# Lymphatus/caesium-clt

Measured on AMD Instinct MI355X. Metric: megapixels/sec JPEG q=80 1920x1080 batch, higher is better.
Workload: dtype int32

## Files before the change

### caesium-clt_amd/binding.py

```python
import ctypes as C
import os

_HERE = os.path.dirname(os.path.abspath(__file__))
NPHASES = 8
NKERNELS = 36
PHASE_NAMES = ["decode", "pixel", "masks_flags_runs", "stats_tables", "sizes_scan", "pack", "stuff_assemble", "reserved"]


class CCSParameters(C.Structure):
    _fields_ = [("keep_metadata", C.c_bool), ("jpeg_quality", C.c_uint32), ("jpeg_chroma_subsampling", C.c_uint32),
                ("jpeg_progressive", C.c_bool), ("jpeg_optimize", C.c_bool), ("jpeg_preserve_icc", C.c_bool),
                ("png_quality", C.c_uint32), ("png_optimization_level", C.c_uint32), ("png_force_zopfli", C.c_bool),
                ("png_optimize", C.c_bool), ("gif_quality", C.c_uint32), ("webp_quality", C.c_uint32), ("webp_lossless", C.c_bool),
                ("tiff_compression", C.c_uint32), ("tiff_deflate_level", C.c_uint32), ("width", C.c_uint32), ("height", C.c_uint32)]


class CCSResult(C.Structure):
    _fields_ = [("success", C.c_bool), ("code", C.c_uint32), ("error_message", C.c_char_p)]


class CByteArray(C.Structure):
    _fields_ = [("data", C.POINTER(C.c_uint8)), ("length", C.c_size_t)]


class Timing(C.Structure):
    _fields_ = [("total_ms", C.c_float), ("phase_ms", C.c_float * NPHASES), ("kernel_ms", C.c_float * NKERNELS), ("in_bytes", C.c_uint64), ("out_bytes", C.c_uint64),
                ("pixels", C.c_uint64), ("coef_bytes", C.c_uint64), ("n_images", C.c_uint32), ("n_failed", C.c_uint32), ("n_seq_decoded", C.c_uint32), ("n_par_fallback", C.c_uint32), ("n_par_short", C.c_uint32), ("n_prog_decoded", C.c_uint32), ("n_refine_chains", C.c_uint32), ("n_search_extra", C.c_uint32), ("n_fused_lists", C.c_uint32), ("n_list_refine", C.c_uint32), ("n_ac_in_lists", C.c_uint32), ("n_list_runs", C.c_uint32), ("n_ref_packed", C.c_uint32)]


class PngTiming(C.Structure):
    _fields_ = [("total_ms", C.c_float), ("kernel_ms", C.c_float * 16), ("in_bytes", C.c_uint64), ("out_bytes", C.c_uint64), ("pixels", C.c_uint64),
                ("raw_bytes", C.c_uint64), ("n_images", C.c_uint32), ("n_failed", C.c_uint32), ("n_trials", C.c_uint32)]


class GifTiming(C.Structure):
    _fields_ = [("total_ms", C.c_float), ("kernel_ms", C.c_float * 8), ("in_bytes", C.c_uint64), ("out_bytes", C.c_uint64), ("n_files", C.c_uint32), ("n_frames", C.c_uint32),
                ("n_failed", C.c_uint32), ("n_passed_palette", C.c_uint32), ("n_not_smaller", C.c_uint32), ("chunk_pixels", C.c_uint32), ("lossy_distance", C.c_uint32)]


class CaesiumError(RuntimeError):
    def __init__(self, code, message):
        super().__init__(f"[{code}] {message}")
        self.code = code


def library_path():
    return os.path.join(_HERE, "libcaesium_hip.so")


EXPORTS = ["cs_default_parameters", "cs_compress_in_memory", "cs_compress_to_size_in_memory", "cs_convert_in_memory",
           "cs_batch_compress", "cs_batch_extent", "cs_free_bytes", "cs_free_result", "csh_device_count", "csh_last_error", "csh_kernel_name", "csh_kernel_name_webp", "csh_release_cached_memory", "csh_warmup", "csh_batch_create",
           "csh_batch_run", "csh_batch_fetch", "csh_batch_destroy", "csh_batch_retain_dct", "csh_batch_set_quality", "csh_batch_rerun_encode", "cs_batch_compress_to_size", "csh_batch_geometry", "csh_batch_read_coefs",
           "csp_kernel_name", "csp_batch_create", "csp_batch_create_webp", "csp_batch_create_pixels", "csh_batch_create_pixels", "csh_batch_pixels", "csh_batch_create_from_pixels", "csp_png_to_jpeg", "csp_png_to_lossless_webp", "csp_batch_run", "csp_batch_fetch", "csp_batch_destroy", "csp_batch_geometry", "csp_batch_read_rows", "csp_batch_read_stream",
           "csp_batch_trials", "csp_batch_read_scores", "csp_batch_chunk_bits", "csh_batch_create_webp", "cs_batch_convert",
           "cswd_batch_create", "cswd_batch_run", "cswd_batch_pixels", "cswd_batch_read_pixels", "cswd_batch_alpha", "cswd_batch_read_rgba", "cswd_batch_destroy", "cswd_batch_frames", "cswd_batch_read_canvas", "cswd_batch_encode_anim", "cswd_rgba_join", "cswd_rgba_destroy", "csh_batch_create_webp_from_pixels", "csh_batch_create_from_pixels_rgb", "csl_encode_pixels", "csl_attach_alpha"]
GIF_EXPORTS = ["csg_kernel_name", "csg_batch_create", "csg_batch_run", "csg_batch_fetch", "csg_batch_destroy", "csg_batch_frames", "csg_batch_read_indices", "csg_batch_read_canvas", "csg_batch_create_lossy", "csg_batch_read_near"]


def _declare(L):
    P = C.POINTER
    L.cs_default_parameters.argtypes = [P(CCSParameters)]
    L.cs_default_parameters.restype = None
    L.cs_compress_in_memory.argtypes = [C.c_char_p, C.c_size_t, P(CCSParameters), P(CByteArray)]
    L.cs_compress_in_memory.restype = CCSResult
    L.cs_compress_to_size_in_memory.argtypes = [C.c_char_p, C.c_size_t, P(CCSParameters), C.c_size_t, C.c_bool, P(CByteArray)]
    L.cs_compress_to_size_in_memory.restype = CCSResult
    L.cs_convert_in_memory.argtypes = [C.c_char_p, C.c_size_t, P(CCSParameters), C.c_uint32, P(CByteArray)]
    L.cs_convert_in_memory.restype = CCSResult
    L.cs_batch_compress.argtypes = [P(CByteArray), C.c_size_t, P(CCSParameters), C.c_int, P(CByteArray), P(CCSResult)]
    L.cs_batch_extent.argtypes = [P(CByteArray), C.c_size_t]
    L.cs_batch_extent.restype = C.c_size_t
    L.cs_free_bytes.argtypes = [P(CByteArray)]
    L.cs_free_bytes.restype = None
    L.cs_free_result.argtypes = [P(CCSResult)]
    L.cs_free_result.restype = None
    L.csh_last_error.restype = C.c_char_p
    L.csh_kernel_name.argtypes = [C.c_int]
    L.csh_kernel_name.restype = C.c_char_p
    L.csh_kernel_name_webp.argtypes = [C.c_int]
    L.csh_kernel_name_webp.restype = C.c_char_p
    L.csh_batch_create.argtypes = [P(CByteArray), C.c_size_t, P(CCSParameters), C.c_int, P(C.c_void_p)]
    L.csh_batch_run.argtypes = [C.c_void_p, P(Timing)]
    L.csh_batch_fetch.argtypes = [C.c_void_p, P(CByteArray), P(CCSResult)]
    L.csh_batch_retain_dct.argtypes = [C.c_void_p, C.c_int]
    L.csh_batch_set_quality.argtypes = [C.c_void_p, P(C.c_uint32)]
    L.csh_batch_rerun_encode.argtypes = [C.c_void_p, P(Timing)]
    L.cs_batch_compress_to_size.argtypes = [P(CByteArray), C.c_size_t, P(CCSParameters), C.c_size_t, C.c_bool, C.c_int, P(CByteArray), P(CCSResult)]
    L.csh_batch_destroy.argtypes = [C.c_void_p]
    L.csh_batch_destroy.restype = None
    L.csh_batch_geometry.argtypes = [C.c_void_p, C.c_size_t, C.c_int, C.c_int, P(C.c_int), P(C.c_int), P(C.c_int), P(C.c_int)]
    L.csh_batch_read_coefs.argtypes = [C.c_void_p, C.c_size_t, C.c_int, C.c_int, C.c_void_p]
    L.csh_batch_create_webp.argtypes = [P(CByteArray), C.c_size_t, P(CCSParameters), C.c_int, P(C.c_void_p)]
    L.cs_batch_convert.argtypes = [P(CByteArray), C.c_size_t, P(CCSParameters), C.c_uint32, C.c_int, P(CByteArray), P(CCSResult)]
    L.csp_kernel_name.argtypes = [C.c_int]
    L.csp_kernel_name.restype = C.c_char_p
    L.csp_batch_create.argtypes = [P(CByteArray), C.c_size_t, P(CCSParameters), C.c_int, P(C.c_void_p)]
    L.csp_batch_run.argtypes = [C.c_void_p, P(PngTiming)]
    L.csp_batch_fetch.argtypes = [C.c_void_p, P(CByteArray), P(CCSResult)]
    L.csp_batch_destroy.argtypes = [C.c_void_p]
    L.csp_batch_destroy.restype = None
    L.csp_batch_geometry.argtypes = [C.c_void_p, C.c_size_t, P(C.c_uint32), P(C.c_uint32), P(C.c_uint32)]
    L.csp_batch_read_rows.argtypes = [C.c_void_p, C.c_size_t, C.c_void_p]
    L.csp_batch_read_stream.argtypes = [C.c_void_p, C.c_size_t, C.c_int, C.c_void_p]
    L.csp_batch_read_scores.argtypes = [C.c_void_p, C.c_size_t, C.c_void_p, P(C.c_int)]
    L.csp_batch_chunk_bits.argtypes = [C.c_void_p, C.c_size_t, C.c_int, P(C.c_uint64), C.c_size_t, P(C.c_size_t)]
    L.csp_batch_trials.argtypes = [C.c_void_p, C.c_size_t, P(C.c_int), P(C.c_uint64), P(C.c_int), P(C.c_int)]
    L.cswd_batch_create.argtypes = [P(CByteArray), C.c_size_t, C.c_int, P(C.c_void_p)]
    L.cswd_batch_run.argtypes = [C.c_void_p]
    L.cswd_batch_pixels.argtypes = [C.c_void_p, C.c_size_t, P(C.c_void_p), P(C.c_uint32), P(C.c_uint32), P(C.c_uint32), P(C.c_char_p)]
    L.cswd_batch_read_pixels.argtypes = [C.c_void_p, C.c_size_t, C.c_void_p]
    L.cswd_batch_alpha.argtypes = [C.c_void_p, C.c_size_t, P(C.c_void_p), P(C.c_void_p)]
    L.cswd_batch_read_rgba.argtypes = [C.c_void_p, C.c_size_t, C.c_void_p]
    L.cswd_batch_destroy.argtypes = [C.c_void_p]
    L.cswd_batch_destroy.restype = None
    L.cswd_batch_frames.argtypes = [C.c_void_p, C.c_size_t, P(C.c_uint32), P(C.c_uint32), P(C.c_uint32)]
    L.cswd_batch_read_canvas.argtypes = [C.c_void_p, C.c_size_t, C.c_uint32, C.c_void_p]
    L.cswd_batch_encode_anim.argtypes = [C.c_void_p, P(CByteArray), P(C.c_size_t), C.c_size_t, P(CCSParameters), C.c_int, P(CByteArray), P(CCSResult)]
    L.cswd_rgba_join.argtypes = [C.c_void_p, C.c_void_p, C.c_uint32, C.c_uint32, C.c_int, C.POINTER(C.c_void_p), C.POINTER(C.c_void_p)]
    L.cswd_rgba_join.restype = C.c_int
    L.cswd_rgba_destroy.argtypes = [C.c_void_p]
    L.cswd_rgba_destroy.restype = None
    L.csg_kernel_name.argtypes = [C.c_int]
    L.csg_kernel_name.restype = C.c_char_p
    L.csg_batch_create.argtypes = [P(CByteArray), C.c_size_t, P(CCSParameters), C.c_int, P(C.c_void_p)]
    L.csg_batch_run.argtypes = [C.c_void_p, P(GifTiming)]
    L.csg_batch_fetch.argtypes = [C.c_void_p, P(CByteArray), P(CCSResult)]
    L.csg_batch_destroy.argtypes = [C.c_void_p]
    L.csg_batch_destroy.restype = None
    L.csg_batch_frames.argtypes = [C.c_void_p, C.c_size_t, P(C.c_uint32), P(C.c_uint32), P(C.c_uint32)]
    L.csg_batch_read_indices.argtypes = [C.c_void_p, C.c_size_t, C.c_uint32, C.c_void_p]
    L.csg_batch_read_canvas.argtypes = [C.c_void_p, C.c_size_t, C.c_uint32, C.c_void_p]
    L.csg_batch_create_lossy.argtypes = [P(CByteArray), C.c_size_t, P(CCSParameters), C.c_int, P(C.c_void_p)]
    L.csg_batch_read_near.argtypes = [C.c_void_p, C.c_size_t, C.c_uint32, C.c_void_p, C.c_void_p]
    return L


def default_parameters(lib=None, **kw):
    p = CCSParameters()
    p.jpeg_quality = p.png_quality = p.webp_quality = p.gif_quality = 80
    p.jpeg_progressive = True
    p.jpeg_preserve_icc = True
    p.png_optimization_level = 3
    p.tiff_deflate_level = 6
    for k, v in kw.items():
        if not hasattr(p, k):
            raise AttributeError(k)
        setattr(p, k, v)
    return p


class Batch:

    def __init__(self, api, blobs, params, device=0, webp=False):
        self.api = api
        L = api.L
        self.n = len(blobs)
        self._keep = [C.create_string_buffer(b, len(b)) for b in blobs]
        self._in = (CByteArray * self.n)()
        for i, buf in enumerate(self._keep):
            self._in[i].data = C.cast(buf, C.POINTER(C.c_uint8))
            self._in[i].length = len(blobs[i])
        self.h = C.c_void_p()
        rc = (L.csh_batch_create_webp if webp else L.csh_batch_create)(self._in, self.n, C.byref(params), device, C.byref(self.h))
        if rc:
            raise CaesiumError(rc, L.csh_last_error().decode())

    def run(self):
        t = Timing()
        rc = self.api.L.csh_batch_run(self.h, C.byref(t))
        if rc:
            raise CaesiumError(rc, self.api.L.csh_last_error().decode())
        return t

    def retain_dct(self, on=True):
        if self.api.L.csh_batch_retain_dct(self.h, 1 if on else 0):
            raise CaesiumError(-1, self.api.L.csh_last_error().decode())

    def set_quality(self, qualities):
        arr = (C.c_uint32 * self.n)(*qualities)
        if self.api.L.csh_batch_set_quality(self.h, arr):
# ... 430 lines not shown
```

### caesium-clt_amd/csrc/batch.hpp

```cpp
#pragma once
#include <array>
#include <chrono>
#include <map>
#include <string>
#include <vector>

#include "../../include/caesium_hip.h"
#include "devmem.hpp"
#include "jpeg_host.hpp"
#include "kernels.h"
#include "webp_kernels.h"

namespace csh {

struct Item {
    int code = 0;
    std::string msg;
    JpegInfo in;
    JpegInfo out;
    int image = -1;
    size_t file_size = 0;
    std::vector<uint8_t> meta_out;
};

struct DecodePlan {
    PinnedBytes bits_pool;
    std::vector<DecScan> dscans;
    std::vector<DevHuffSet> hsets;
    std::vector<ParHuffSet> phsets;
    std::vector<char> phset_fits;
    std::vector<ParHuffSet4> phsets4;
    std::vector<std::array<int8_t, 8>> slot4;
    bool use4 = true;
    std::vector<ParScan> pscans;
    std::vector<uint32_t> need_seq_init;
    std::vector<ProgChain> chains;
    std::vector<int> chain_scans;
    std::vector<RefineUnit> refine_units;
    uint32_t refine_hist = 0, refine_pos = 0, refine_max_blocks = 0;
    uint32_t total_sub = 0, max_sub = 0, max_par_blocks = 0, dc_total = 0;

    DevBuf<uint8_t> d_bits, d_clean;
    DevBuf<ParScan> d_pscans;
    DevBuf<uint64_t> d_pstate, d_relax_list[2], d_unstuff_off, d_blk_off, d_dc_off;
    DevBuf<uint32_t> d_unstuff_cnt, d_nblk, d_need_seq, d_need_seq_init, d_relax_cnt, d_scan_pending, d_cut_block, d_claim;
    DevBuf<uint16_t> d_hyp;
    DevBuf<int32_t> d_dcdiff;
    DevBuf<DecScan> d_dscans;
    DevBuf<ProgChain> d_chains;
    DevBuf<int> d_chain_scans;
    DevBuf<uint64_t> d_refine_hist;
    DevBuf<uint32_t> d_refine_pos, d_refine_prog;
    DevBuf<RefineUnit> d_refine_units;
    DevBuf<DevHuffSet> d_hsets;
    DevBuf<ParHuffSet> d_phsets;
    DevBuf<ParHuffSet4> d_phsets4;
};

struct PixelPlan {
    std::vector<PlaneWork> pwork;
    std::vector<ResizeWork> rwork;
    std::vector<ResizeTap> rtaps;
    std::vector<float> rweights;
    uint64_t rgb_bytes = 0, tmp_floats = 0, max_tmp = 0, max_dst = 0;
    uint32_t max_row_in = 0, max_out_w = 0, max_nh = 0;
    uint32_t max_src_px = 0;
    uint64_t plane_bytes = 0, oplane_bytes = 0;
    uint32_t max_quads = 0;
    bool any_layout = false, any_layout_rgb = false;
    bool any_space_rgb = false;

    DevBuf<uint8_t> d_planes, d_oplanes, d_rgb;
    DevBuf<PlaneWork> d_pwork;
    DevBuf<ResizeWork> d_rwork;
    DevBuf<ResizeTap> d_rtaps;
    DevBuf<float> d_rweights, d_rtmp;
    DevBuf<int16_t> d_dct_raw;
};

struct Stage {
    uint32_t work0 = 0, nwork = 0, slot0 = 0, nslots = 0, ech0 = 0, nech = 0, table0 = 0, ntables = 0, plan0 = 0, nplans = 0, nzc0 = 0, nnzc = 0, ls0 = 0, nls = 0, ts0 = 0, nts = 0, rs0 = 0, nrs = 0, lr0 = 0, nlr = 0, rr0 = 0, nrr = 0;
    bool nz_build[2] = {true, true}, nz_filter[2] = {true, true};
};
struct SearchImg {
    int cand_work[64]; int ncand;
    int Al_luma = 0, Al_chroma = 0;
    uint64_t best_luma = 0, best_chroma = 0;
    int split_luma = 0, split_chroma = 0;
    bool luma_on = false, chroma_on = false;
    bool fixed = false;
};

struct EncodePlan {
    std::vector<EncScan> script;
    std::vector<ScanWork> swork;
    uint32_t nslots = 0, nlist_slots = 0, ntok_slots = 0;
    uint32_t nref_slots = 0;
    uint32_t last_run_refine = 0;
    uint32_t last_run_ref_packed = 0;
    bool ref_pack = true;
    uint32_t list_run = CSH_LIST_RUN;
    uint32_t nlist_runs = 0, nref_runs = 0;
    bool ac_runs_slot = false;
    uint32_t last_run_list_runs = 0;
    uint64_t total_corr = 0;
    uint64_t total_units = 0, total_words = 0;
    uint32_t max_units = 0;
    int ntables = 0;
    std::vector<TokPlan> plans;
    std::vector<int> plan_comp, plan_image;
    std::vector<EChunk> echunks;
    uint64_t tok_cap = 0;
    uint32_t tok_scale = 1;
    std::vector<TokRegion> regions;
    std::vector<uint32_t> region_est;
    uint32_t hist_rows = 0;
    std::vector<NzList> nzlists;
    std::vector<NzSet> nzsets;
    std::vector<int> nzset_of;
    std::vector<uint32_t> nzset_built;
    std::vector<int> nzset_comp, nzset_image;
    std::vector<NzChunk> nzchunks;
    std::vector<NzChunk> nzchunks_fused;
    uint32_t n_fused = 0;
    uint32_t last_run_fused = 0;
    uint32_t n_ac_lists = 0;
    uint32_t last_run_ac_lists = 0;
    std::vector<uint8_t> nzset_ac_lists;
    std::vector<uint32_t> nz_est, nz_worst;
    uint32_t nz_nrec = 0;
    uint64_t nz_cap = 0;
    bool search = false;
    enum { ST_1 = 0, ST_1B = 1, ST_2 = 2, ST_2B = 3, ST_2C = 4, ST_N = 5 };
    Stage stage[ST_N];
    void stage_begin(Stage &sg) {
        sg.work0 = uint32_t(swork.size()); sg.slot0 = nslots; sg.ech0 = uint32_t(echunks.size()); sg.table0 = uint32_t(ntables); sg.plan0 = uint32_t(plans.size());
        sg.nzc0 = uint32_t(nzchunks.size()); sg.ls0 = nlist_slots; sg.ts0 = ntok_slots; sg.rs0 = nref_slots; sg.lr0 = nlist_runs; sg.rr0 = nref_runs;
    }
    void stage_end(Stage &sg) {
        sg.nwork = uint32_t(swork.size()) - sg.work0; sg.nslots = nslots - sg.slot0; sg.nech = uint32_t(echunks.size()) - sg.ech0;
        sg.ntables = uint32_t(ntables) - sg.table0; sg.nplans = uint32_t(plans.size()) - sg.plan0;
        sg.nnzc = uint32_t(nzchunks.size()) - sg.nzc0; sg.nls = nlist_slots - sg.ls0; sg.nts = ntok_slots - sg.ts0; sg.nrs = nref_slots - sg.rs0; sg.nlr = nlist_runs - sg.lr0; sg.nrr = nref_runs - sg.rr0;
    }
    std::vector<SearchImg> simg;
    std::vector<uint8_t> work_active;
    uint32_t n_gated_runs = 0;
    std::vector<uint32_t> img_list, img_nlist, h_cost;
    std::map<std::array<int, 5>, int> cand_script;
    std::vector<uint8_t> hdr_pool;
    std::vector<uint32_t> hdr_off;

    DevBuf<uint8_t> d_hdr, d_tail, d_scan_tmp, d_work_active;
    DevBuf<EncScan> d_script;
    DevBuf<ScanWork> d_swork;
    DevBuf<uint32_t> d_slot_work;
    DevBuf<EChunk> d_echunks;
    DevBuf<SlotRec> d_slots;
    DevBuf<TokPlan> d_plans;
    DevBuf<uint64_t> d_corr, d_symbits, d_eobbits, d_tok_off, d_chunk_off, d_scan_raw_off;
    DevBuf<uint32_t> d_tok_cursor;
    DevBuf<TokRegion> d_regions;
    DevBuf<uint16_t> d_eobrun, d_slot_hist, d_lastn;
    DevBuf<uint32_t> d_img_list, d_img_nlist, d_scan_cost, d_slot_raw, d_slot_eobh, d_long_runs, d_long_cnt, d_tokens, d_chunk_ntok, d_chunk_bits, d_raw, d_scan_pad, d_chunk_ff, d_hdr_off;
    DevBuf<DevEncTable> d_tables;
    DevBuf<NzList> d_nzlists;
    DevBuf<NzSet> d_nzsets;
    DevBuf<NzChunk> d_nzchunks, d_nzchunks_fused;
    DevBuf<uint32_t> d_nz_pool, d_nz_cursor, d_nz_chunk_off, d_nz_chunk_cnt, d_list_slots, d_tok_slots, d_ref_slots, d_list_runs, d_ref_runs;
};

struct TrellisPlan {
    bool trellis = false, dering = false;
    Stage tstage;
    std::vector<TrellisWork> twork;
    std::vector<TrellisRun> truns;
    uint32_t t_units = 0, t_max_rows = 0;
    std::vector<uint32_t> trows;
    bool t_sort = false;
    bool nz_once = false;

    DevBuf<TrellisWork> d_twork;
    DevBuf<TrellisRun> d_truns;
    DevBuf<uint32_t> d_tqueue, d_trows, d_tperm, d_tspill;
    DevBuf<uint8_t> d_tblk_cnt;
    DevBuf<uint16_t> d_tblk_off;
    DevBuf<uint64_t> d_tlambda, d_tdcbt;
};

struct WebpTail {
    uint32_t webp_mb_bytes = 768;
    std::vector<csw::WebpImg> wimgs;
    uint64_t wwork_bytes = 0, wlevels = 0;
    uint32_t wmax_luma = 0, wmax_mbh = 0;

    DevBuf<csw::WebpImg> d_wimgs;
    DevBuf<uint8_t> d_wwork, d_wscratch, d_wprobs, d_wupdate;
    DevBuf<uint32_t> d_wpart, d_wstats;
    DevBuf<int16_t> d_wlevels;
};

struct Outputs {
    uint64_t raw_bytes_cap = 0, out_cap = 0;
    DevBuf<uint8_t> d_out;
    DevBuf<uint64_t> d_img_off;
    DevBuf<uint32_t> d_img_size, d_img_size_pad, d_status, d_overflow;
    std::vector<uint32_t> h_img_size;
    std::vector<uint64_t> h_img_off;
    std::vector<uint32_t> h_status;
    bool ran = false;
};

}

struct csh_batch {
    int device = 0;
    hipStream_t stream = 0;
    bool have_stream = false;
    CCSParameters params;
    std::vector<csh::Item> items;
    int nimg = 0;
    bool lossless = false;
    bool rgb_out = false;
    bool webp = false;
    int test_pool_shift = -1;
    bool progressive = true;
    bool retain_dct = false;
    bool have_dct = false;
    int q_base = 0;

    std::vector<csh::ImgDesc> imgs;
    std::vector<csh::DevQuant> quants;
    uint32_t ntiles = 0, ntiles_in = 0, ntiles_out = 0, max_tiles = 0, max_dummy = 0;
    csh::DevBuf<csh::ImgDesc> d_imgs;
    csh::DevBuf<csh::DevQuant> d_quants;
    csh::DevBuf<int16_t> d_coef;

    csh::DecodePlan dec;
    csh::PixelPlan pix;
    csh::EncodePlan enc;
    csh::TrellisPlan tr;
    csh::WebpTail wp;
    csh::Outputs out;

    ~csh_batch() { if (have_stream) { (void)hipStreamSynchronize(stream); (void)hipStreamDestroy(stream); } }
};

namespace csh {

enum KernelSlot {
    KS_MEMSET_COEF, KS_UNSTUFF, KS_DEC_SPEC, KS_DEC_RELAX0, KS_DEC_RELAX, KS_DEC_WRITE, KS_DC_SCATTER, KS_REFINE_CHAINS, KS_DECODE_PROG_SEQ,
    KS_IDCT_PLANE, KS_RESIZE, KS_XFORM_DIRECT, KS_RESAMPLE_FDCT, KS_FIX_DUMMY, KS_MEMSET_ENC, KS_TRELLIS_STATS, KS_TRELLIS_AC, KS_TRELLIS_DC,
    KS_NZLIST, KS_TOKENS, KS_LIST_STATS, KS_AC_RUNS, KS_GEN_TABLES, KS_CHUNK_SIZES, KS_SCAN_CHUNK_BITS, KS_SCAN_LAYOUT, KS_PACK, KS_LIST_PACK,
    KS_FF_COUNT, KS_SCAN_SEARCH, KS_LAYOUT, KS_SCAN_IMAGES, KS_EMIT, KS_SPARE0, KS_SPARE1, KS_SPARE2, KS_COUNT,
    KS_WEBP_YUV = KS_XFORM_DIRECT, KS_WEBP_ENCODE = KS_RESAMPLE_FDCT, KS_WEBP_ASSEMBLE = KS_FIX_DUMMY
};
struct KernelSlotRow { KernelSlot slot; const char *name; int phase; };
constexpr KernelSlotRow kKernelSlots[] = {
    {KS_MEMSET_COEF, "memset_coef", 0},        {KS_UNSTUFF, "unstuff", 0},                 {KS_DEC_SPEC, "k_dec_spec", 0},
    {KS_DEC_RELAX0, "k_dec_relax0", 0},        {KS_DEC_RELAX, "k_dec_relax1_4", 0},        {KS_DEC_WRITE, "k_dec_write", 0},
    {KS_DC_SCATTER, "k_dc_scatter", 0},        {KS_REFINE_CHAINS, "k_refine_chains", 0},   {KS_DECODE_PROG_SEQ, "k_decode_prog+seq", 0},
    {KS_IDCT_PLANE, "k_idct_plane", 1},        {KS_RESIZE, "resize", 1},                   {KS_XFORM_DIRECT, "k_xform_direct", 1},
    {KS_RESAMPLE_FDCT, "k_resample+k_plane_fdct", 1}, {KS_FIX_DUMMY, "k_fix_dummy", 1},    {KS_MEMSET_ENC, "memset_enc", 2},
    {KS_TRELLIS_STATS, "trellis_stats", 1},    {KS_TRELLIS_AC, "k_trellis_ac", 1},         {KS_TRELLIS_DC, "k_trellis_dc", 1},
    {KS_NZLIST, "k_nzlist", 2},                {KS_TOKENS, "k_tokens", 2},                 {KS_LIST_STATS, "k_list_stats", 2},
    {KS_AC_RUNS, "k_ac_runs", 2},              {KS_GEN_TABLES, "k_gen_tables", 3},         {KS_CHUNK_SIZES, "k_chunk_sizes", 4},
    {KS_SCAN_CHUNK_BITS, "scan_chunk_bits", 4}, {KS_SCAN_LAYOUT, "scan_layout", 4},        {KS_PACK, "k_pack", 5},
    {KS_LIST_PACK, "k_list_pack", 5},          {KS_FF_COUNT, "k_ff_count", 6},             {KS_SCAN_SEARCH, "scan_search_stage2", 7},
    {KS_LAYOUT, "k_layout", 6},                {KS_SCAN_IMAGES, "scan_images", 6},         {KS_EMIT, "k_emit", 6},
    {KS_SPARE0, "", 7},                        {KS_SPARE1, "", 7},                         {KS_SPARE2, "", 7}};
constexpr bool kernel_slots_in_order() {
    for (int i = 0; i < int(sizeof kKernelSlots / sizeof kKernelSlots[0]); i++) if (kKernelSlots[i].slot != i) return false;
    return true;
}
static_assert(sizeof kKernelSlots / sizeof kKernelSlots[0] == CSH_NKERNELS && int(KS_COUNT) == int(CSH_NKERNELS), "one row per csh_timing.kernel_ms slot");
static_assert(kernel_slots_in_order(), "row i of kKernelSlots describes slot i");

struct PlanSwitches {
    std::string profile;
    bool nz_once = true;
    bool tr_sort = true;
    int prog_par = -1;
    bool fused_420 = true;
    bool nz_fused = true;
    bool ref_list = true;
    bool ref_pack = true;
    uint32_t list_run = CSH_LIST_RUN;
    bool ac_runs_slot = false;
    bool ac_tiles = false;
    static PlanSwitches read();
};

struct Laps {
    const bool trace;
    std::chrono::steady_clock::time_point at = std::chrono::steady_clock::now();
    std::string text;
    Laps();
    void lap(const char *what);
};

struct BatchPlanner {
    csh_batch *const b;
    const CByteArray *const inputs;
    const size_t count;
    const CCSParameters *const p;
    const csp_pixels *const px;
    const PlanSwitches sw;
    const bool progressive;
    uint16_t qout_nat[64];
    int script_base3 = 0, script_base1 = 0;
    std::map<int, int> other_scripts;
    std::vector<std::pair<std::vector<uint8_t>, int>> hset_keys;
    std::map<std::vector<uint16_t>, int> quant_index;
    uint64_t plane_off = 64, oplane_off = 0;

    BatchPlanner(csh_batch *b, const CByteArray *inputs, size_t count, const CCSParameters *p, const csp_pixels *px);
    void begin();
    void parse();
    int reserve_pinned();
    int plan_image(size_t n);
    int plan_search_stages();
    int plan_trellis();
    void finish_descriptors();
    int upload(Laps &laps);

private:
    void image_geometry(Item &it, ImgDesc &im);
    int decode_scans(Item &it, ImgDesc &im, const uint8_t *d);
    int huff_set(const JScan &js);
    void place_blocks(ParScan &ps, const JpegInfo &in, const JScan &js, uint32_t units, bool dc_rows, bool subseqs);
    int sequential_split(const Item &it, const ImgDesc &im, const uint8_t *d, int img_index, bool &par_ok);
    bool progressive_plan(const Item &it, const ImgDesc &im, int img_index);
    void plane_work(ImgDesc &im, const JpegInfo &in, const JpegInfo &o, int img_index, bool resized);
    void resize_work(const JpegInfo &in, const JpegInfo &o, int img_index);
    void output_scans(Item &it, ImgDesc &im, int img_index, size_t in_len);
    void frame_header(Item &it);
    template <class Fill> int enc_scan(const std::array<int, 5> &key, Fill fill);
    int space_script(int ncomp, int space, int &ns);
    int cand_index(int comp, int Ss, int Se, int Ah, int Al, int cls = -1);
    int dc_scan_index(int ncomp);
    int seq1_index(int comp, int cls = -1);
    uint32_t nz_list(int img_index, int comp, int Al, const ImgDesc &im, size_t in_len);
    void add_works(Item &it, ImgDesc &im, int img_index, const std::vector<int> &list, size_t in_len, const JpegInfo &o, bool stats_only = false);
    template <class Make> void add_stage(int sid, Make make);
    template <class Add> void splits(const ImgDesc &im, Add &add, int i0, int i1, bool whole);
};

void layout_token_pool(csh_batch *b);

int run_once(csh_batch *b, csh_timing *t, bool requant_only);

int search_costs(csh_batch *b, AsmCtx &a, int stage);
uint32_t search_gate(csh_batch *b, int stage, int (*want)(const SearchImg &));
int search_decide(csh_batch *b, int stage);
int search_lists(csh_batch *b);

}
```

### caesium-clt_amd/csrc/batch_plan.cpp

```cpp
#include <algorithm>
#include <atomic>
#include <cmath>
#include <thread>

#include "batch.hpp"
#include "resize_host.h"
#include "result.h"

namespace csh {

static void build_dev_huff(const HuffSpec &h, DevHuff &d) {
    memset(&d, 0, sizeof d);
    for (int l = 0; l < 18; l++) d.maxcode[l] = -1;
    if (!h.present) return;
    int code = 0, p = 0;
    for (int l = 1; l <= 16; l++) {
        if (h.bits[l]) {
            d.valptr[l] = p - code;
            for (int i = 0; i < h.bits[l]; i++, p++, code++)
                if (l <= 9) {
                    int base = code << (9 - l);
                    for (int k = 0; k < (1 << (9 - l)); k++) d.look[(base + k) & 511] = uint16_t((l << 8) | h.vals[p]);
                }
            d.maxcode[l] = code - 1;
// ... 50 lines not shown
            while ((2 << lg) <= q.div[k]) lg++;
            const int P = std::max(25, lg + 18);
            q.mul[k] = uint32_t((1ull << P) / uint64_t(q.div[k])) + 1u;
            q.sh[k] = uint32_t(32 - P);
        }
    }
}

static void fill_geom(const JComp &c, CompGeom &g, uint32_t &ntiles) {
    g.h = c.h; g.v = c.v; g.comp_w = c.comp_w; g.comp_h = c.comp_h;
    g.real_bw = c.real_bw; g.real_bh = c.real_bh; g.bw = c.bw; g.bh = c.bh;
    g.ntiles = (c.bw * c.bh + 63) / 64;
    g.tile_base = ntiles;
    ntiles += g.ntiles;
}

static void add_script(std::vector<EncScan> &v, int ncomp, bool progressive, int space) {
    for (const OutScan &o : output_script(ncomp, progressive, space == CSH_CS_YCC)) {
        EncScan e;
        memset(&e, 0, sizeof e);
        e.ncomp = o.ncomp; e.Ss = o.Ss; e.Se = o.Se; e.Ah = o.Ah; e.Al = o.Al;
        for (int k = 0; k < o.ncomp; k++) e.comp[k] = o.comp[k];
        if (!progressive) {
            e.sequential = 1;
            for (int k = 0; k < o.ncomp; k++) {
                int id = table_class(space, o.comp[k]);
                int di = -1, ai = -1;
                for (int t = 0; t < e.ntables; t++) { if (e.dht_id[t] == id) di = t; if (e.dht_id[t] == (0x10 | id)) ai = t; }
                if (di < 0) { di = e.ntables; e.dht_id[e.ntables++] = id; }
                if (ai < 0) { ai = e.ntables; e.dht_id[e.ntables++] = 0x10 | id; }
                e.dc_tbl[k] = di; e.ac_tbl[k] = ai;
                e.sos_tdta[k] = (id << 4) | id;
            }
        } else if (o.Ss == 0) {
            if (o.Ah == 0) {
                e.ntables = 0;
                for (int k = 0; k < o.ncomp; k++) {
                    int id = table_class(space, o.comp[k]);
                    int idx = -1;
                    for (int t = 0; t < e.ntables; t++) if (e.dht_id[t] == id) idx = t;
                    if (idx < 0) { idx = e.ntables; e.dht_id[e.ntables++] = id; }
                    e.dc_tbl[k] = idx;
                    e.sos_tdta[k] = id << 4;
                }
            }
        } else {
            int id = table_class(space, o.comp[0]);
            e.ntables = 1; e.dht_id[0] = 0x10 | id; e.sos_tdta[0] = id;
        }
        v.push_back(e);
    }
}

static UpDesc up_desc(int hx, int vx, int cw) {
    UpDesc u; u.hx = uint8_t(hx); u.vx = uint8_t(vx); u.pad = 0;
    if (hx == 1 && vx == 1) u.cls = CSH_UP_COPY;
    else if (hx == 2 && vx == 1 && cw > 2) u.cls = CSH_UP_H2V1;
    else if (hx == 1 && vx == 2) u.cls = CSH_UP_H1V2;
    else if (hx == 2 && vx == 2 && cw > 2) u.cls = CSH_UP_H2V2;
    else u.cls = CSH_UP_REP;
    return u;
}
static int dn_kind(int hx, int vx) { return hx == 1 ? CSH_DN_FULL : (hx == 4 ? CSH_DN_H4V1 : (vx == 2 ? CSH_DN_H2V2 : CSH_DN_H2V1)); }

static int plan_item(Item &it, const CCSParameters &p, bool lossless, bool to_rgb) {
    const JpegInfo &in = it.in;
    if (in.ncomp != 1 && in.ncomp != 3 && in.ncomp != 4) { it.msg = "unsupported component count"; return CS_ERR_JPEG_FEATURE; }
    if (uint64_t(in.width) * uint64_t(in.height) > (1ull << 28)) { it.msg = "image dimensions too large for the device path"; return CS_ERR_JPEG_FEATURE; }
    const bool other_space = in.space != CSH_CS_GREY && in.space != CSH_CS_YCC;
    const bool converted = other_space && to_rgb;
    it.out = JpegInfo();
    JpegInfo &o = it.out;
    o.width = in.width; o.height = in.height; o.ncomp = converted ? 3 : in.ncomp;
    o.space = converted ? CSH_CS_YCC : in.space;
    if (other_space && !converted) { o.write_jfif = false; o.write_adobe = in.adobe_transform; }
    if (p.width || p.height) {
        if (lossless) { it.msg = "resize + lossless transcode not on the device path"; return CS_ERR_UNSUPPORTED; }
        csh_compute_dimensions(in.width, in.height, int(p.width), int(p.height), o.width, o.height);
        if (o.width > 65500 || o.height > 65500 || uint64_t(o.width) * uint64_t(o.height) > (1ull << 28)) { it.msg = "resize target too large for JPEG"; return CS_ERR_JPEG_FEATURE; }
    }
    if (in.ncomp >= 3 && (!lossless || in.ncomp == 4)) {
        int blocks = 0;
        for (int c = 0; c < in.ncomp; c++) {
            const JComp &k = in.comp[c];
            blocks += k.h * k.v;
            if (in.hmax % k.h || in.vmax % k.v) { it.msg = "fractional chroma sampling ratio (component factors do not divide the largest ones)"; return CS_ERR_JPEG_FEATURE; }
            if (in.hmax / k.h > 4 || in.vmax / k.v > 4) { it.msg = "chroma sampling ratio above 4"; return CS_ERR_JPEG_FEATURE; }
        }
        if (blocks > 10) { it.msg = "more than 10 blocks per MCU"; return CS_ERR_JPEG_FEATURE; }
    }
    if (lossless) {
        for (int c = 0; c < in.ncomp; c++)
            if (memcmp(in.comp[c].qt, in.qt[in.comp[c].tq], sizeof in.comp[c].qt)) { it.msg = "a component was decoded with a quantisation table that its slot no longer holds"; return CS_ERR_JPEG_FEATURE; }
        for (int c = 0; c < in.ncomp; c++) o.comp[c] = in.comp[c];
        jpeg_geometry(o);
        return 0;
    }
    int ss = int(p.jpeg_chroma_subsampling);
    if (ss == 0) ss = 420;
    static const char kRgbIds[] = "RGB", kCmykIds[] = "CMYK";
    for (int c = 0; c < o.ncomp; c++) {
        o.comp[c].id = o.space == CSH_CS_RGB ? kRgbIds[c] : (o.space == CSH_CS_CMYK ? kCmykIds[c] : c + 1);
        o.comp[c].h = o.comp[c].v = 1; o.comp[c].tq = table_class(o.space, c);
    }
    if (o.space == CSH_CS_YCC || o.space == CSH_CS_YCCK) {
        int h = 1, v = 1;
        if (ss == 420) { h = 2; v = 2; }
        else if (ss == 422) { h = 2; v = 1; }
        else if (ss == 411) { h = 4; v = 1; }
        else if (ss != 444) { it.msg = "unknown output chroma subsampling"; return CS_ERR_JPEG_FEATURE; }
        o.comp[0].h = h; o.comp[0].v = v;
        if (o.space == CSH_CS_YCCK) { o.comp[3].h = h; o.comp[3].v = v; }
    }
    jpeg_geometry(o);
    return 0;
}

void layout_token_pool(csh_batch *b) {
    b->enc.regions.resize(b->enc.region_est.size());
    if (b->test_pool_shift < 0) b->test_pool_shift = getenv("CSH_TEST_POOL_SHIFT") ? std::min(16, std::max(0, atoi(getenv("CSH_TEST_POOL_SHIFT")))) : 0;
    const int shift = b->test_pool_shift;
    uint64_t at = 0;
    for (size_t i = 0; i < b->enc.regions.size(); i++) {
        const uint64_t cap = std::min<uint64_t>(std::max<uint64_t>((uint64_t(b->enc.region_est[i]) * b->enc.tok_scale) >> shift, 64), 0xFFFFFFF0ull);
        b->enc.regions[i].base = at; b->enc.regions[i].cap = uint32_t(cap); b->enc.regions[i].pad = 0;
        at += (cap + 3) & ~uint64_t(3);
    }
    b->enc.tok_cap = at + 64;
    at = 0;
    for (size_t i = 0; i < b->enc.nzlists.size(); i++) {
        const uint64_t cap = std::min<uint64_t>(std::max<uint64_t>((uint64_t(b->enc.nz_est[i]) * b->enc.tok_scale) >> shift, 64), b->enc.nz_worst[i]);
        b->enc.nzlists[i].base = at; b->enc.nzlists[i].cap = uint32_t(cap);
        at += (cap + 3) & ~uint64_t(3);
    }
    b->enc.nz_cap = at + 64;
}

PlanSwitches PlanSwitches::read() {
    auto is = [](const char *name, const char *v) { const char *e = getenv(name); return e && !strcmp(e, v); };
    PlanSwitches s;
    const char *penv = getenv("CSH_PROFILE");
    s.profile = penv && *penv ? penv : "mozjpeg";
    s.nz_once = !is("CSH_NZ_ONCE", "0");
    s.tr_sort = !is("CSH_TR_SORT", "0");
    s.nz_fused = !is("CSH_NZ_FUSED", "0");
    s.ac_tiles = is("CSH_AC_TILES", "1");
    s.ref_list = is("CSH_REF_LIST", "1") || (s.ref_list && !is("CSH_REF_LIST", "0"));
    s.ref_pack = s.ref_list && (is("CSH_REF_PACK", "1") || (s.ref_pack && !is("CSH_REF_PACK", "0")));
    const char *pp = getenv("CSH_PROG_PAR");
    s.prog_par = pp && !strcmp(pp, "0") ? 0 : (pp && !strcmp(pp, "1") ? 1 : -1);
    s.fused_420 = !getenv("CSH_NO_FUSED_420");
    if (const char *lr = getenv("CSH_LIST_RUN")) { if (*lr) s.list_run = uint32_t(std::min(32, std::max(1, atoi(lr)))); }
    s.ac_runs_slot = is("CSH_AC_RUNS", "slot");
    return s;
}

Laps::Laps() : trace(getenv("CSH_TRACE") != nullptr) {}
void Laps::lap(const char *what) {
    if (!trace) return;
    const auto now = std::chrono::steady_clock::now();
    char buf[64];
    snprintf(buf, sizeof buf, " %s %.1f", what, std::chrono::duration<double, std::milli>(now - at).count());
    text += buf; at = now;
}

BatchPlanner::BatchPlanner(csh_batch *b_, const CByteArray *inputs_, size_t count_, const CCSParameters *p_, const csp_pixels *px_)
    : b(b_), inputs(inputs_), count(count_), p(p_), px(px_), sw(PlanSwitches::read()), progressive(p_->jpeg_progressive) {}

void BatchPlanner::begin() {
    b->items.resize(count);
    quality_table(int(p->jpeg_quality), qout_nat);
    DevQuant qo; make_quant(qout_nat, qo);
    b->quants.push_back(qo);
    b->q_base = int(b->quants.size()) - 1;
    for (int q = 1; q <= 100; q++) { uint16_t tq[64]; quality_table(q, tq); DevQuant dq; make_quant(tq, dq); b->quants.push_back(dq); }
    b->progressive = progressive;
    b->enc.list_run = sw.list_run;
    b->enc.ac_runs_slot = sw.ac_runs_slot;
    b->enc.ref_pack = sw.ref_pack;

    add_script(b->enc.script, 3, true, CSH_CS_YCC);
    add_script(b->enc.script, 1, true, CSH_CS_GREY);
    add_script(b->enc.script, 3, false, CSH_CS_YCC);
    add_script(b->enc.script, 1, false, CSH_CS_GREY);
    script_base3 = progressive ? 0 : 16; script_base1 = progressive ? 10 : 17;
    const bool webp = b->webp, rgb_out = b->rgb_out;
    const std::string &profile = sw.profile;
    b->enc.search = progressive && !webp && !rgb_out && profile != "plain";
    const bool lossy_jpeg = !b->lossless && !webp && !rgb_out;
    b->tr.trellis = lossy_jpeg && (profile == "mozjpeg" || profile == "mozjpeg-trellis");
    b->tr.dering = lossy_jpeg && (profile == "mozjpeg" || profile == "mozjpeg-dering");
    b->tr.nz_once = b->tr.trellis && progressive && sw.nz_once && sw.tr_sort;
}

template <class Fill>
int BatchPlanner::enc_scan(const std::array<int, 5> &key, Fill fill) {
    auto f = b->enc.cand_script.find(key);
    if (f != b->enc.cand_script.end()) return f->second;
    EncScan e;
    memset(&e, 0, sizeof e);
    fill(e);
    b->enc.script.push_back(e);
    return b->enc.cand_script[key] = int(b->enc.script.size()) - 1;
}
int BatchPlanner::space_script(int ncomp, int space, int &ns) {
    ns = progressive ? (space == CSH_CS_YCC ? 10 : 2 + 4 * ncomp) : 1;
    if (space == CSH_CS_YCC) return script_base3;
    if (space == CSH_CS_GREY) return script_base1;
    auto f = other_scripts.find(space);
    if (f == other_scripts.end()) {
        f = other_scripts.emplace(space, int(b->enc.script.size())).first;
        add_script(b->enc.script, ncomp, progressive, space);
    }
    return f->second;
}
int BatchPlanner::cand_index(int comp, int Ss, int Se, int Ah, int Al, int cls) {
    const int ycc = comp ? 1 : 0;
    if (cls < 0) cls = ycc;
    return enc_scan({cls == ycc ? comp : comp + 16 * (1 + cls), Ss, Se, Ah, Al}, [&](EncScan &e) {
        const int id = cls;
        e.ncomp = 1; e.comp[0] = comp; e.Ss = Ss; e.Se = Se; e.Ah = Ah; e.Al = Al;
        e.ntables = 1; e.dht_id[0] = 0x10 | id; e.sos_tdta[0] = id;
    });
}
int BatchPlanner::dc_scan_index(int ncomp) {
    return enc_scan({-ncomp, 0, 0, 0, 0}, [&](EncScan &e) {
        e.ncomp = ncomp;
        for (int k = 0; k < ncomp; k++) {
            e.comp[k] = k;
            const int id = k ? 1 : 0;
            int idx = -1;
            for (int t = 0; t < e.ntables; t++) if (e.dht_id[t] == id) idx = t;
            if (idx < 0) { idx = e.ntables; e.dht_id[e.ntables++] = id; }
            e.dc_tbl[k] = idx; e.sos_tdta[k] = id << 4;
        }
    });
}
int BatchPlanner::seq1_index(int comp, int cls) {
    const int ycc = comp ? 1 : 0;
    if (cls < 0) cls = ycc;
    return enc_scan({cls == ycc ? comp : comp + 16 * (1 + cls), 0, 63, -1, -1}, [&](EncScan &e) {
        const int id = cls;
        e.ncomp = 1; e.comp[0] = comp; e.Ss = 0; e.Se = 63; e.sequential = 1;
        e.ntables = 2; e.dht_id[0] = id; e.dht_id[1] = 0x10 | id; e.dc_tbl[0] = 0; e.ac_tbl[0] = 1; e.sos_tdta[0] = (id << 4) | id;
    });
}

static uint64_t blocks_of(const ImgDesc &im) {
    uint64_t n = 0;
    for (int k = 0; k < im.ncomp; k++) n += uint64_t(im.out[k].real_bw) * im.out[k].real_bh;
    return n;
}

uint32_t BatchPlanner::nz_list(int img_index, int comp, int Al, const ImgDesc &im, size_t in_len) {
    if (b->enc.nzset_of.size() < size_t(img_index + 1) * CSH_MAX_COMPS) b->enc.nzset_of.resize(size_t(img_index + 1) * CSH_MAX_COMPS, -1);
    int &si = b->enc.nzset_of[size_t(img_index) * CSH_MAX_COMPS + size_t(comp)];
    const uint32_t nu = uint32_t(im.out[comp].real_bw * im.out[comp].real_bh);
    if (si < 0) {
        NzSet S;
        memset(&S, 0, sizeof S);
        for (int L = 0; L < CSH_NZ_LEVELS; L++) S.list[L] = 0xFFFFFFFFu;
        S.cnt_base = 0xFFFFFFFFu;
        S.nunits = nu; S.real_bw = im.out[comp].real_bw; S.bw = im.out[comp].bw; S.tile_base = im.out[comp].tile_base;
        si = int(b->enc.nzsets.size());
        b->enc.nzsets.push_back(S); b->enc.nzset_built.push_back(0u); b->enc.nzset_comp.push_back(comp); b->enc.nzset_image.push_back(img_index);
    }
    const uint64_t blocks_all = blocks_of(im);
    static const uint32_t kShare[CSH_NZ_LEVELS] = {20, 16, 12, 9};
    for (int L : {0, Al}) {
        if (b->enc.nzsets[size_t(si)].list[L] != 0xFFFFFFFFu) continue;
        const uint32_t nch = (nu + 255) / 256;
        NzList R;
        memset(&R, 0, sizeof R);
        R.chunk0 = b->enc.nz_nrec; b->enc.nz_nrec += nch;
        b->enc.nzsets[size_t(si)].list[L] = uint32_t(b->enc.nzlists.size());
        b->enc.nzlists.push_back(R);
        const uint64_t est = uint64_t(in_len) * kShare[L] / 8 * nu / std::max<uint64_t>(1, blocks_all) + nu + 4ull * nch + 256;
        const uint64_t worst = uint64_t(nu) * 64 + 4ull * nch;
        b->enc.nz_est.push_back(uint32_t(std::min<uint64_t>(est, worst)));
        b->enc.nz_worst.push_back(uint32_t(std::min<uint64_t>(worst, 0xFFFFFFF0ull)));
    }
    return b->enc.nzsets[size_t(si)].list[Al];
}

void BatchPlanner::add_works(Item &it, ImgDesc &im, int img_index, const std::vector<int> &list, size_t in_len, const JpegInfo &o, bool stats_only) {
    const int w_first = int(b->enc.swork.size());
    uint32_t nz_need[CSH_MAX_COMPS] = {0, 0, 0}, nz_gate[CSH_MAX_COMPS] = {0, 0, 0};
    for (int sidx : list) {
        const EncScan &e = b->enc.script[sidx];
        ScanWork w;
        memset(&w, 0, sizeof w);
        w.image = img_index; w.scan = sidx;
        w.out_off = 0xFFFFFFFFu;
        const bool from_list = e.Ss > 0 && !e.sequential && e.Ah == 0;
        const bool ref_list = sw.ref_list && e.Ss > 0 && !e.sequential && e.Ah != 0;
        w.list = 0xFFFFFFFFu; w.rs_base = 0xFFFFFFFFu; w.lr_base = 0xFFFFFFFFu; w.rr_base = 0xFFFFFFFFu;
        if (from_list || ref_list) {
            if (e.Al >= CSH_NZ_LEVELS) { it.code = CS_ERR_JPEG_FEATURE; it.msg = "internal: output scan script outside what the list coder carries"; }
            else {
                w.list = nz_list(img_index, e.comp[0], e.Al, im, in_len);
                if (!nz_need[e.comp[0]]) nz_gate[e.comp[0]] = uint32_t(b->enc.swork.size());
                nz_need[e.comp[0]] |= 1u << e.Al;
            }
        }
        if (e.Ss == 0 && e.ncomp > 1) w.nunits = uint32_t(im.omcus_x * im.omcus_y);
        else w.nunits = uint32_t(im.out[e.comp[0]].real_bw * im.out[e.comp[0]].real_bh);
// ... 585 lines not shown
    }
}
int BatchPlanner::plan_search_stages() {
    b->enc.hdr_off.push_back(uint32_t(b->enc.hdr_pool.size()));
    b->nimg = int(b->imgs.size());
    b->enc.stage_end(b->enc.stage[0]);
    if (!b->enc.search) return 0;
    add_stage(EncodePlan::ST_1B, [&](const ImgDesc &, auto &add) { add(9, cand_index(0, 1, 63, 3, 2)); add(10, cand_index(0, 1, 8, 0, 3)); add(11, cand_index(0, 9, 63, 0, 3)); });
    add_stage(EncodePlan::ST_2, [&](const ImgDesc &im, auto &add) { splits(im, add, 0, 2, true); });
    add_stage(EncodePlan::ST_2B, [&](const ImgDesc &im, auto &add) { splits(im, add, 3, 3, false); });
    add_stage(EncodePlan::ST_2C, [&](const ImgDesc &im, auto &add) { splits(im, add, 4, 4, false); });
    for (int c = 0; c < 3; c++) for (int i = -1; i < 5; i++) for (int Al = 1; Al <= (c ? 2 : 3); Al++) {
        if (i < 0) cand_index(c, 1, 63, 0, Al); else { cand_index(c, 1, kSplit[i], 0, Al); cand_index(c, kSplit[i] + 1, 63, 0, Al); }
    }
    b->enc.work_active.assign(b->enc.swork.size(), 0);
    if (b->enc.total_units > 0xFFFFFFF0ull) { csh_set_error("csh_batch_create: batch too large for the scan search's candidate lists (fewer files per batch)"); return CS_ERR_POOL_OVERFLOW; }
    return 0;
}

int BatchPlanner::plan_trellis() {
    if (!b->tr.trellis) return 0;
    b->enc.nslots++;
    Stage &tg = b->tr.tstage;
    b->enc.stage_begin(tg);
    for (size_t n = 0; n < count; n++) {
        Item &it = b->items[n];
        if (it.image < 0) continue;
        ImgDesc &im = b->imgs[size_t(it.image)];
        std::vector<int> list;
        const int space = it.out.space;
        for (int c = 0; c < im.ncomp; c++) list.push_back(progressive ? cand_index(c, 1, 63, 0, 0, table_class(space, c)) : seq1_index(c, table_class(space, c)));
        const size_t first = b->enc.swork.size();
        add_works(it, im, it.image, list, inputs[n].length, it.out, true);
        for (int c = 0; c < im.ncomp; c++) {
            const ScanWork &w = b->enc.swork[first + size_t(c)];
            TrellisWork tw;
            memset(&tw, 0, sizeof tw);
            tw.image = it.image; tw.comp = c; tw.dc_cls = uint32_t(table_class(space, c));
            tw.table_ac = w.table_base + (progressive ? 0u : 1u);
            tw.table_dc = progressive ? -1 : int32_t(w.table_base);
            tw.nunits = w.nunits; tw.unit_base = b->tr.t_units;
            b->tr.t_units += w.nunits;
            b->tr.t_max_rows = std::max<uint32_t>(b->tr.t_max_rows, uint32_t((im.out[c].real_bh + im.out[c].v - 1) / im.out[c].v));
            tw.nzset = 0xFFFFFFFFu;
            if (progressive) {
                const int si = b->enc.nzset_of[size_t(it.image) * CSH_MAX_COMPS + size_t(c)];
                b->enc.nzsets[size_t(si)].cnt_base = tw.unit_base;
                if (b->tr.nz_once) tw.nzset = uint32_t(si);
            }
            b->tr.twork.push_back(tw);
        }
    }
    b->enc.stage_end(tg);
    {
        std::vector<uint32_t> nch(b->tr.twork.size());
        uint32_t most = 0;
        for (size_t wi = 0; wi < b->tr.twork.size(); wi++) { nch[wi] = (b->tr.twork[wi].nunits + CSH_TR_WG - 1) / CSH_TR_WG; most = std::max(most, nch[wi]); }
        for (uint32_t j = 0; j < most; j += CSH_TR_RUN)
            for (size_t wi = 0; wi < b->tr.twork.size(); wi++)
                if (j < nch[wi]) b->tr.truns.push_back(TrellisRun{uint32_t(wi), j, std::min<uint32_t>(CSH_TR_RUN, nch[wi] - j)});
    }
    {
        b->tr.t_sort = progressive && sw.tr_sort;
        std::vector<std::pair<uint32_t, uint32_t>> rows;
        for (size_t wi = 0; wi < b->tr.twork.size(); wi++) {
            const CompGeom &g = b->imgs[size_t(b->tr.twork[wi].image)].out[b->tr.twork[wi].comp];
            for (int r = 0; r < (g.real_bh + g.v - 1) / g.v; r++) rows.push_back({uint32_t(g.real_bw * g.v), uint32_t(wi << 16) | uint32_t(r)});
        }
        std::stable_sort(rows.begin(), rows.end(), [](const auto &a, const auto &b2) { return a.first > b2.first; });
        for (const auto &r : rows) b->tr.trows.push_back(r.second);
    }
    if (b->enc.total_units > 0xFFFFFFF0ull) { csh_set_error("csh_batch_create: batch too large (fewer files per batch)"); return CS_ERR_POOL_OVERFLOW; }
    return 0;
}

void BatchPlanner::finish_descriptors() {
    if (!b->lossless)
        for (ImgDesc &im : b->imgs) for (int c = 0; c < im.ncomp; c++) im.out[c].tile_base += b->ntiles_in;
    for (size_t i = 0; i < b->enc.plans.size(); i++) b->enc.plans[i].tile_base = b->imgs[size_t(b->enc.plan_image[i])].out[b->enc.plan_comp[i]].tile_base;
    for (size_t i = 0; i < b->enc.nzsets.size(); i++) b->enc.nzsets[i].tile_base = b->imgs[size_t(b->enc.nzset_image[i])].out[b->enc.nzset_comp[i]].tile_base;
    {
        b->enc.nzchunks_fused = b->enc.nzchunks;
        const bool allowed = sw.nz_fused && !b->lossless && !b->webp && !b->rgb_out && !(b->tr.trellis && progressive && !b->tr.nz_once);
        std::vector<uint8_t> fused(b->enc.nzsets.size(), 0);
        const bool lists_only = progressive && !sw.ac_tiles && sw.ref_list && sw.nz_once && sw.tr_sort && (!b->tr.trellis || (b->tr.t_sort && b->tr.nz_once));
        std::vector<uint8_t> planned(b->enc.nzsets.size(), 0);
        for (size_t i = 0; i < b->enc.plans.size(); i++) {
            const size_t at = size_t(b->enc.plan_image[i]) * CSH_MAX_COMPS + size_t(b->enc.plan_comp[i]);
            if (at < b->enc.nzset_of.size() && b->enc.nzset_of[at] >= 0) planned[size_t(b->enc.nzset_of[at])] = 1;
        }
        b->enc.nzset_ac_lists.assign(b->enc.nzsets.size(), 0);
        for (PlaneWork &w : b->pix.pwork) {
            w.ac_lists = 0u;
            const size_t at = size_t(w.image) * CSH_MAX_COMPS + size_t(w.comp);
            const int si = allowed && at < b->enc.nzset_of.size() ? b->enc.nzset_of[at] : -1;
            if (si < 0) continue;
            const NzSet &S = b->enc.nzsets[size_t(si)];
            if (S.real_bw != S.bw || S.list[0] == 0xFFFFFFFFu) continue;
            w.nzset = uint32_t(si); fused[size_t(si)] = 1; b->enc.n_fused++;
            if (lists_only && !planned[size_t(si)]) { w.ac_lists = 1u; b->enc.nzset_ac_lists[size_t(si)] = 1; b->enc.n_ac_lists++; }
        }
        for (TrellisWork &tw : b->tr.twork) tw.ac_lists = (tw.nzset != 0xFFFFFFFFu && b->enc.nzset_ac_lists[tw.nzset]) ? 1u : 0u;
        for (NzChunk &ch : b->enc.nzchunks_fused) if (fused[ch.set]) ch.levels &= ~1u;
        auto flags = [&](Stage &sg) {
            for (int f = 0; f < 2; f++) {
                const std::vector<NzChunk> &v = f ? b->enc.nzchunks_fused : b->enc.nzchunks;
                sg.nz_build[f] = sg.nz_filter[f] = false;
                for (uint32_t i = sg.nzc0; i < sg.nzc0 + sg.nnzc; i++) { sg.nz_build[f] |= (v[i].levels & 1u) != 0u; sg.nz_filter[f] |= (v[i].levels & ~1u) != 0u; }
            }
        };
        for (Stage &sg : b->enc.stage) flags(sg);
        flags(b->tr.tstage);
    }
    for (ParScan &ps : b->dec.pscans)
        for (int m = 0; m < ps.nb_mcu && m < 10; m++) {
            int dcs = ps.dct[m] & 3, acs = 4 + (ps.act[m] & 3);
            if (b->dec.use4) { dcs = std::max<int>(0, b->dec.slot4[ps.huff_set][dcs]); acs = std::max<int>(0, b->dec.slot4[ps.huff_set][acs]); }
            ps.sel |= uint64_t(dcs | (acs << 3)) << (6 * m);
        }
    {
        std::vector<int> last(b->dec.chains.size(), -1);
        for (int s = 0;; s++) {
            bool any = false;
            for (size_t c = 0; c < b->dec.chains.size(); c++)
                if (b->dec.chains[c].refine && b->dec.chains[c].count > s) {
                    RefineUnit u; u.chain = int(c); u.s = s; u.prev = last[c];
                    last[c] = int(b->dec.refine_units.size());
                    b->dec.refine_units.push_back(u);
                    any = true;
                }
            if (!any) break;
        }
    }
    b->ntiles = b->ntiles_in + b->ntiles_out;
    b->pix.plane_bytes = plane_off;
    b->pix.oplane_bytes = oplane_off;
    b->out.out_cap = b->out.raw_bytes_cap;
    layout_token_pool(b);
}

int BatchPlanner::upload(Laps &laps) {
    hipStream_t st = b->stream;
    if (!b->nimg) return 0;
    b->dec.bits_pool.flush_copies();
    laps.lap("copy_in");
    if (b->dec.d_bits.alloc(b->dec.bits_pool.size()) || (b->dec.bits_pool.size() && hipMemcpyAsync(b->dec.d_bits.p, b->dec.bits_pool.p, b->dec.bits_pool.size(), hipMemcpyHostToDevice, st) != hipSuccess) ||
        b->d_imgs.upload(b->imgs, st) || b->dec.d_dscans.upload(b->dec.dscans, st) || b->dec.d_chains.upload(b->dec.chains, st) || b->dec.d_chain_scans.upload(b->dec.chain_scans, st) ||
        b->dec.d_hsets.upload(b->dec.hsets, st) || b->dec.d_phsets.upload(b->dec.phsets, st) || (b->dec.use4 && b->dec.d_phsets4.upload(b->dec.phsets4, st)) || b->d_quants.upload(b->quants, st) || b->pix.d_pwork.upload(b->pix.pwork, st) ||
        b->enc.d_script.upload(b->enc.script, st) || b->enc.d_swork.upload(b->enc.swork, st) || b->enc.d_slot_work.alloc(size_t(b->enc.nslots) + 1) || b->enc.d_slots.alloc(size_t(b->enc.nslots) + 1) || b->enc.d_plans.upload(b->enc.plans, st) || b->enc.d_echunks.upload(b->enc.echunks, st) || b->enc.d_hdr.upload(b->enc.hdr_pool, st) ||
        b->enc.d_hdr_off.upload(b->enc.hdr_off, st) || b->dec.d_pscans.upload(b->dec.pscans, st) || b->pix.d_rwork.upload(b->pix.rwork, st) || b->pix.d_rtaps.upload(b->pix.rtaps, st) ||
        b->pix.d_rweights.upload(b->pix.rweights, st) || b->pix.d_rgb.alloc(b->pix.rgb_bytes + 64) || b->pix.d_rtmp.alloc((resize_is_fused(b->pix.max_row_in) ? 0 : b->pix.tmp_floats) + 16) || b->dec.d_need_seq_init.upload(b->dec.need_seq_init, st))
        return CS_ERR_NO_DEVICE;
    size_t nchunks = b->dec.bits_pool.size() / 64 + 1, nst = size_t(b->dec.total_sub) + b->dec.pscans.size() + 1;
    if (b->dec.d_clean.alloc(b->dec.bits_pool.size() + 64) || b->dec.d_unstuff_cnt.alloc(nchunks + 1) || b->dec.d_unstuff_off.alloc(nchunks + 2) ||
        b->dec.d_pstate.alloc(nst) || b->dec.d_relax_list[0].alloc(nst) || b->dec.d_relax_list[1].alloc(nst) || b->dec.d_relax_cnt.alloc(512) || b->dec.d_scan_pending.alloc(b->dec.pscans.size() + 1) || b->dec.d_cut_block.alloc(b->dec.pscans.size() + 1) || b->dec.d_claim.alloc(size_t(b->dec.total_sub) + 1) || b->dec.d_hyp.alloc((size_t(b->dec.total_sub) + 1) * 10) ||
        b->dec.d_nblk.alloc(size_t(b->dec.total_sub) + 1) || b->dec.d_blk_off.alloc(size_t(b->dec.total_sub) + 2) || b->dec.d_need_seq.alloc(b->nimg + 1) ||
        b->dec.d_dcdiff.alloc(size_t(b->dec.dc_total) + 1) || b->dec.d_dc_off.alloc(size_t(b->dec.dc_total) + 2) ||
        b->dec.d_refine_hist.alloc(size_t(b->dec.refine_hist) + 1) || b->dec.d_refine_pos.alloc(size_t(b->dec.refine_pos) + 1) || b->dec.d_refine_units.upload(b->dec.refine_units, st) ||
        b->dec.d_refine_prog.alloc(b->dec.refine_units.size() + 1))
        return CS_ERR_NO_DEVICE;
    if (b->d_coef.alloc(size_t(b->ntiles) * CSH_TILE_I16) || b->pix.d_planes.alloc(b->pix.plane_bytes + 64) || b->pix.d_oplanes.alloc(b->pix.oplane_bytes + 64) ||
        b->enc.d_symbits.alloc(b->enc.total_words + 1) || b->enc.d_eobbits.alloc(b->enc.total_words + 1) ||
        b->enc.d_long_runs.alloc(2 * (b->enc.total_units / 512 + b->enc.swork.size() + 16)) || b->enc.d_long_cnt.alloc(4) || b->enc.d_tail.alloc(b->enc.total_units + 1) || b->enc.d_eobrun.alloc(b->enc.total_units + 1) || b->enc.d_corr.alloc(b->enc.total_corr + 1) || b->enc.d_lastn.alloc((b->enc.ref_pack ? b->enc.total_corr : 0) + 1) ||
        b->enc.d_tok_off.alloc(4 * size_t(b->enc.nslots) + 4) || b->enc.d_chunk_ntok.alloc(4 * size_t(b->enc.nslots) + 4) || b->enc.d_slot_hist.alloc(size_t(b->enc.hist_rows) * 256 + 256) ||
        b->enc.d_slot_raw.alloc(size_t(b->enc.nslots) + 1) || b->enc.d_img_list.upload(b->enc.img_list, st) || b->enc.d_img_nlist.upload(b->enc.img_nlist, st) || b->enc.d_scan_cost.alloc(b->enc.swork.size() + 1) || b->enc.d_slot_eobh.alloc(16 * size_t(b->enc.nslots) + 16) || b->enc.d_chunk_bits.alloc(size_t(b->enc.nslots) + 1) || b->enc.d_chunk_off.alloc(size_t(b->enc.nslots) + 2) || b->enc.d_tok_cursor.alloc(b->enc.region_est.size() + 1) || b->enc.d_regions.upload(b->enc.regions, st) ||
        b->enc.d_tables.alloc(b->enc.ntables) || b->enc.d_scan_pad.alloc(b->enc.swork.size() + 1) ||
        b->enc.d_nzlists.upload(b->enc.nzlists, st) || b->enc.d_nzsets.upload(b->enc.nzsets, st) || b->enc.d_nzchunks.upload(b->enc.nzchunks, st) || (b->enc.n_fused && b->enc.d_nzchunks_fused.upload(b->enc.nzchunks_fused, st)) || b->enc.d_list_slots.alloc(size_t(b->enc.nlist_slots) + 1) || b->enc.d_tok_slots.alloc(size_t(b->enc.ntok_slots) + 1) || b->enc.d_ref_slots.alloc(size_t(b->enc.nref_slots) + 1) || b->enc.d_list_runs.alloc(size_t(b->enc.nlist_runs) + 1) || b->enc.d_ref_runs.alloc(size_t(b->enc.nref_runs) + 1) ||
        b->enc.d_nz_cursor.alloc(b->enc.nzlists.size() + 1) || b->enc.d_nz_chunk_off.alloc(size_t(b->enc.nz_nrec) + 1) || b->enc.d_nz_chunk_cnt.alloc(size_t(b->enc.nz_nrec) + 1) ||
        b->enc.d_scan_raw_off.alloc(b->enc.swork.size() + 2) || b->out.d_img_size.alloc(b->nimg + 1) || b->out.d_img_size_pad.alloc(b->nimg + 1) ||
        b->out.d_img_off.alloc(b->nimg + 2) || b->out.d_status.alloc(b->nimg) || b->out.d_overflow.alloc(4))
        return CS_ERR_NO_DEVICE;
    if (hipMemsetAsync(b->enc.d_slots.p, 0, (size_t(b->enc.nslots) + 1) * sizeof(SlotRec), st) != hipSuccess ||
        hipMemsetAsync(b->enc.d_slot_work.p, 0, (size_t(b->enc.nslots) + 1) * sizeof(uint32_t), st) != hipSuccess) { csh_set_error("hipMemsetAsync failed"); return CS_ERR_NO_DEVICE; }
    launch_make_slots(st, b->enc.d_swork.p, uint32_t(b->enc.swork.size()), b->enc.d_script.p, b->enc.d_nzlists.p, b->enc.d_slots.p, b->enc.d_slot_work.p, b->enc.d_list_slots.p, b->enc.d_tok_slots.p, b->enc.d_ref_slots.p, b->enc.d_list_runs.p, b->enc.d_ref_runs.p, b->enc.list_run);
    if (b->tr.trellis && (b->tr.d_trows.upload(b->tr.trows, st) || (b->tr.t_sort && (b->tr.d_tperm.alloc(size_t(b->tr.t_units) + 1) || b->tr.d_tblk_cnt.alloc(size_t(b->tr.t_units) + 1) || (b->tr.nz_once && b->tr.d_tblk_off.alloc(size_t(b->tr.t_units) + 1)))))) return CS_ERR_NO_DEVICE;
    if (b->tr.trellis && (b->tr.d_twork.upload(b->tr.twork, st) || b->tr.d_truns.upload(b->tr.truns, st) || b->tr.d_tqueue.alloc(1) || b->tr.d_tlambda.alloc(size_t(b->tr.t_units) + 1) || b->tr.d_tdcbt.alloc(size_t(b->tr.t_units) + 1) ||
                       b->tr.d_tspill.alloc(trellis_spill_words(trellis_ac_slots())) || b->pix.d_dct_raw.alloc(size_t(b->ntiles_out) * CSH_TILE_I16)))
        return CS_ERR_NO_DEVICE;
    for (size_t n = 0; px && n < count; n++) {
        const Item &it = b->items[n];
        if (it.image < 0) continue;
        const ResizeWork &rw = b->pix.rwork[size_t(it.image)];
        if (rw.image != it.image) { csh_set_error("internal: resize work out of order"); return CS_ERR_NO_DEVICE; }
        if (hipMemcpyAsync(b->pix.d_rgb.p + rw.rgb_src_off, px[n].device_pixels, size_t(px[n].width) * px[n].height * px[n].channels, hipMemcpyDeviceToDevice, st) != hipSuccess) { csh_set_error("pixel copy failed"); return CS_ERR_NO_DEVICE; }
    }
    laps.lap("alloc+enqueue");
    if (hipStreamSynchronize(st) != hipSuccess) { csh_set_error("upload failed"); return CS_ERR_NO_DEVICE; }
    laps.lap("upload_wait");
    return 0;
}

}
```

### caesium-clt_amd/csrc/batch_run.cpp

```cpp
#include <algorithm>

#include "batch.hpp"

namespace csh {
namespace {

class KernelMarks {
    hipEvent_t ev[CSH_NKERNELS + 1];
    int created = 0, next = 0;
    const hipStream_t st;

public:
    explicit KernelMarks(hipStream_t s) : st(s) {}
    KernelMarks(const KernelMarks &) = delete;
    KernelMarks &operator=(const KernelMarks &) = delete;
    ~KernelMarks() { for (int i = 0; i < created; i++) (void)hipEventDestroy(ev[i]); }
    int start() {
        for (; created <= CSH_NKERNELS; created++) CSH_CHECK(hipEventCreate(&ev[created]));
        CSH_CHECK(hipEventRecord(ev[0], st));
        return 0;
    }
    int claim(KernelSlot slot, hipEvent_t *e) {
        if (int(slot) != next || next >= CSH_NKERNELS) {
            csh_set_error("internal: timing mark '%s' out of order (slot %d is next)", slot < KS_COUNT ? kKernelSlots[slot].name : "?", next);
            return -1;
        }
        *e = ev[++next];
        return 0;
    }
    int mark(KernelSlot slot) {
        hipEvent_t e;
        if (claim(slot, &e)) return -1;
        CSH_CHECK(hipEventRecord(e, st));
        return 0;
    }
    int skip_to(KernelSlot slot) {
        while (next < int(slot)) if (mark(KernelSlot(next))) return -1;
        return int(slot) == next ? 0 : mark(slot);
    }
    int read(csh_timing *t, bool phases) const {
        if (phases) {
            for (int i = 0; i < CSH_NPHASES; i++) t->phase_ms[i] = 0;
            for (int i = 0; i < CSH_NKERNELS; i++) t->kernel_ms[i] = 0;
        }
        for (int i = 0; i < next; i++) {
            CSH_CHECK(hipEventElapsedTime(&t->kernel_ms[i], ev[i], ev[i + 1]));
            if (phases) t->phase_ms[kKernelSlots[i].phase] += t->kernel_ms[i];
        }
        CSH_CHECK(hipEventElapsedTime(&t->total_ms, ev[0], ev[next]));
        return 0;
    }
};
#define MARK(slot) do { if (marks.mark(slot)) return -1; } while (0)

struct Run {
    csh_batch *const b;
    csh_timing *const t;
    const hipStream_t st;
    const int nimg;
    KernelMarks marks;
    uint64_t raw_chunks = 0;
    bool eobrun_cleared = false;
    bool fused = false;
    EncCtx c;
    AsmCtx a;

    Run(csh_batch *b_, csh_timing *t_) : b(b_), t(t_), st(b_->stream), nimg(b_->nimg), marks(b_->stream) {}

    int pools() {
        raw_chunks = (b->out.raw_bytes_cap + 63) / 64;
        if (b->enc.d_raw.n != raw_chunks * 16) {
            if (b->enc.d_raw.alloc(raw_chunks * 16) || b->enc.d_chunk_ff.alloc(raw_chunks + 1) || b->out.d_out.alloc(b->out.out_cap + 64))
                return -1;
            const uint64_t longest = std::max({uint64_t(size_t(b->enc.nslots)), uint64_t(b->enc.swork.size()), uint64_t(b->dec.dc_total), uint64_t(b->dec.total_sub), uint64_t(b->dec.bits_pool.size() / 64), uint64_t(nimg)});
            size_t tmp = exclusive_scan_tmp_bytes(longest + 1);
            if (b->enc.d_scan_tmp.alloc(tmp)) return -1;
        }
        if (b->enc.d_tokens.n < b->enc.tok_cap && b->enc.d_tokens.alloc(b->enc.tok_cap)) return -1;
        if (b->enc.d_nz_pool.n < b->enc.nz_cap && b->enc.d_nz_pool.alloc(b->enc.nz_cap)) return -1;
        return 0;
    }

    int requant() {
        if (b->out.d_status.zero(st) || b->out.d_overflow.zero(st)) return -1;
        launch_requant(st, b->d_imgs.p, b->pix.d_pwork.p, int(b->pix.pwork.size()), b->max_tiles, b->d_quants.p, b->pix.d_dct_raw.p, b->ntiles_in, b->d_coef.p);
        launch_fix_dummy(st, b->d_imgs.p, nimg, b->max_dummy, b->d_coef.p);
        return marks.skip_to(KS_MEMSET_ENC);
    }
    int skip_decode() {
        if (b->out.d_status.zero(st) || b->out.d_overflow.zero(st)) return -1;
        return marks.skip_to(KS_IDCT_PLANE);
    }

    int decode() {
        const bool zero_in_spec = !b->dec.pscans.empty() && b->dec.max_sub != 0;
        if (!zero_in_spec) CSH_CHECK(hipMemsetAsync(b->d_coef.p, 0, size_t(b->ntiles_in) * CSH_TILE_I16 * sizeof(int16_t), st));
        if (b->out.d_status.zero(st) || b->out.d_overflow.zero(st)) return -1;
        CSH_CHECK(hipMemcpyAsync(b->dec.d_need_seq.p, b->dec.d_need_seq_init.p, size_t(nimg) * sizeof(uint32_t), hipMemcpyDeviceToDevice, st));
        MARK(KS_MEMSET_COEF);
        {
            int nps = int(b->dec.pscans.size());
            uint32_t nchunks = uint32_t(b->dec.bits_pool.size() / 64);
            if (nps) {
                launch_unstuff_count(st, b->dec.d_bits.p, b->dec.d_pscans.p, nps, nchunks, b->dec.d_unstuff_cnt.p);
                launch_exclusive_scan(st, b->dec.d_unstuff_cnt.p, b->dec.d_unstuff_off.p, nchunks, b->enc.d_scan_tmp.p, b->enc.d_scan_tmp.n);
                launch_unstuff_copy(st, b->dec.d_bits.p, b->dec.d_clean.p, b->dec.d_pscans.p, nps, nchunks, b->dec.d_unstuff_off.p);
            }
            MARK(KS_UNSTUFF);
            DenseArgs da;
            memset(&da, 0, sizeof da);
            da.clean = b->dec.d_clean.p; da.pss = b->dec.d_pscans.p; da.huffs = b->dec.use4 ? static_cast<const void *>(b->dec.d_phsets4.p) : static_cast<const void *>(b->dec.d_phsets.p); da.compact = b->dec.use4 ? 1 : 0; da.state = b->dec.d_pstate.p; da.nblk = b->dec.d_nblk.p;
            da.list_out = b->dec.d_relax_list[0].p; da.cnt_out = b->dec.d_relax_cnt.p; da.blk_off = b->dec.d_blk_off.p; da.imgs = b->d_imgs.p;
            da.coef = b->d_coef.p; da.dcdiff = b->dec.d_dcdiff.p; da.need_seq = b->dec.d_need_seq.p; da.cut_block = b->dec.d_cut_block.p;
            CSH_CHECK(hipMemsetAsync(b->dec.d_cut_block.p, 0xFF, b->dec.d_cut_block.n * sizeof(uint32_t), st));
            const uint64_t zero_all = uint64_t(b->ntiles_in) * CSH_TILE_I16 * sizeof(int16_t), zero_half = (zero_all / 2) & ~uint64_t(15);
            const uint64_t eob_all = (uint64_t(b->enc.d_eobrun.n) * sizeof(uint16_t)) & ~uint64_t(15), eob_half = (eob_all / 2) & ~uint64_t(15);
            if (zero_in_spec) { da.zero_ptr = reinterpret_cast<uint8_t *>(b->d_coef.p); da.zero_bytes = zero_half; da.zero2_ptr = reinterpret_cast<uint8_t *>(b->enc.d_eobrun.p); da.zero2_bytes = eob_half; }
            launch_dec_dense(st, 0, nps, b->dec.max_sub, da);
            da.zero_bytes = 0; da.zero2_bytes = 0;
            MARK(KS_DEC_SPEC);
            if (nps) CSH_CHECK(hipMemsetAsync(b->dec.d_relax_cnt.p, 0, b->dec.d_relax_cnt.n * sizeof(uint32_t), st));
            if (nps && b->dec.d_claim.zero(st)) return -1;
            if (zero_in_spec) {
                da.zero_ptr = reinterpret_cast<uint8_t *>(b->d_coef.p) + zero_half; da.zero_bytes = zero_all - zero_half;
                da.zero2_ptr = reinterpret_cast<uint8_t *>(b->enc.d_eobrun.p) + eob_half; da.zero2_bytes = eob_all - eob_half;
                if (uint64_t(b->enc.d_eobrun.n) * sizeof(uint16_t) > eob_all) CSH_CHECK(hipMemsetAsync(reinterpret_cast<uint8_t *>(b->enc.d_eobrun.p) + eob_all, 0, uint64_t(b->enc.d_eobrun.n) * sizeof(uint16_t) - eob_all, st));
                eobrun_cleared = b->enc.d_eobrun.n != 0;
            }
            launch_dec_dense(st, 1, nps, b->dec.max_sub, da);
            da.zero_bytes = 0; da.zero2_bytes = 0;
            MARK(KS_DEC_RELAX0);
            const int kMaxRounds = int(b->dec.d_relax_cnt.n) - 2;
            int R = 0;
            for (int group = 12; nps && R < kMaxRounds; group = 8) {
                for (int g = 0; g < group && R < kMaxRounds; g++, R++)
                    launch_dec_relax_list(st, b->dec.d_clean.p, b->dec.d_pscans.p, b->dec.total_sub, da.huffs, da.compact, b->dec.d_pstate.p, b->dec.d_nblk.p, b->dec.d_relax_list[R & 1].p,
                                          b->dec.d_relax_cnt.p + R, b->dec.d_relax_list[(R & 1) ^ 1].p, b->dec.d_relax_cnt.p + R + 1, b->dec.d_pstate.n, b->dec.d_claim.p, uint32_t(R + 1));
                uint32_t left = 0;
                CSH_CHECK(hipMemcpyAsync(&left, b->dec.d_relax_cnt.p + R, sizeof left, hipMemcpyDeviceToHost, st));
                CSH_CHECK(hipStreamSynchronize(st));
                if (!left) break;
            }
            if (nps) {
                if (b->dec.d_scan_pending.zero(st)) return -1;
                launch_dec_mark_pending(st, b->dec.d_pscans.p, b->dec.total_sub, b->dec.d_relax_list[R & 1].p, b->dec.d_relax_cnt.p + R, b->dec.d_scan_pending.p);
                da.hyp = b->dec.d_hyp.p; da.scan_pending = b->dec.d_scan_pending.p;
                launch_dec_dense(st, 3, nps, b->dec.max_sub, da);
                launch_dec_chain(st, b->dec.d_pscans.p, nps, b->dec.d_pstate.p, b->dec.d_nblk.p, b->dec.d_hyp.p, b->dec.d_scan_pending.p, b->dec.d_need_seq.p);
            }
            MARK(KS_DEC_RELAX);
            if (nps) launch_exclusive_scan(st, b->dec.d_nblk.p, b->dec.d_blk_off.p, b->dec.total_sub, b->enc.d_scan_tmp.p, b->enc.d_scan_tmp.n);
            launch_dec_dense(st, 2, nps, b->dec.max_sub, da);
            MARK(KS_DEC_WRITE);
            if (nps) launch_exclusive_scan(st, reinterpret_cast<uint32_t *>(b->dec.d_dcdiff.p), b->dec.d_dc_off.p, b->dec.dc_total, b->enc.d_scan_tmp.p, b->enc.d_scan_tmp.n);
            launch_dc_scatter(st, b->dec.d_pscans.p, nps, b->dec.max_par_blocks, b->d_imgs.p, b->dec.d_dc_off.p, b->d_coef.p, b->dec.d_need_seq.p, b->dec.d_cut_block.p);
            launch_dc_refine(st, b->dec.d_clean.p, b->dec.d_pscans.p, nps, b->dec.max_par_blocks, b->d_imgs.p, b->d_coef.p, b->dec.d_need_seq.p);
            MARK(KS_DC_SCATTER);
        }
        launch_refine_chains(st, b->dec.d_clean.p, b->dec.d_pscans.p, b->dec.d_phsets.p, b->dec.d_dscans.p, b->dec.d_chains.p, b->dec.d_chain_scans.p, int(b->dec.chains.size()), b->dec.d_refine_units.p,
                             int(b->dec.refine_units.size()), b->dec.refine_max_blocks, b->d_imgs.p, b->d_coef.p, b->dec.d_need_seq.p, b->dec.d_refine_hist.p, b->dec.d_refine_pos.p, b->dec.d_refine_prog.p);
        MARK(KS_REFINE_CHAINS);
        launch_decode_prog(st, b->dec.d_clean.p, b->dec.d_pscans.p, b->dec.d_phsets.p, b->dec.d_dscans.p, b->dec.d_chains.p, b->dec.d_chain_scans.p, int(b->dec.chains.size()), b->d_imgs.p,
                           b->d_coef.p, b->dec.d_need_seq.p);
        launch_decode_seq(st, b->dec.d_bits.p, b->d_imgs.p, b->dec.d_dscans.p, b->dec.d_hsets.p, b->d_coef.p, nimg, b->dec.d_need_seq.p);
        MARK(KS_DECODE_PROG_SEQ);
        return 0;
    }

    int planes() {
        int nw = b->lossless ? 0 : int(b->pix.pwork.size());
        launch_idct_plane(st, b->d_imgs.p, b->pix.d_pwork.p, nw, b->max_tiles, b->d_quants.p, b->d_coef.p, b->pix.d_planes.p);
        MARK(KS_IDCT_PLANE);
        launch_resize(st, b->d_imgs.p, b->pix.d_rwork.p, int(b->pix.rwork.size()), b->pix.d_rtaps.p, b->pix.d_rweights.p, b->pix.d_planes.p, b->pix.d_rgb.p, b->pix.d_rtmp.p,
                      b->pix.max_src_px, b->pix.max_tmp, b->pix.max_dst, b->pix.max_row_in, b->pix.max_out_w, b->pix.max_nh, !(b->webp || b->rgb_out), b->pix.any_layout_rgb, b->pix.any_space_rgb);
        MARK(KS_RESIZE);
        return 0;
    }
    int pixels() {
        const int nw = b->lossless ? 0 : int(b->pix.pwork.size());
        int16_t *rawp = ((b->retain_dct || b->tr.trellis) && !b->lossless) ? b->pix.d_dct_raw.p : nullptr;
        NzFuse nzf;
        memset(&nzf, 0, sizeof nzf);
        fused = nw && b->enc.n_fused;
        if (fused) {
            if (b->enc.d_nz_cursor.zero(st) || b->enc.d_nz_chunk_cnt.zero(st)) return -1;
            nzf.nzsets = b->enc.d_nzsets.p; nzf.nzlists = b->enc.d_nzlists.p; nzf.nz_pool = b->enc.d_nz_pool.p; nzf.nz_cursor = b->enc.d_nz_cursor.p;
            nzf.nz_chunk_off = b->enc.d_nz_chunk_off.p; nzf.nz_chunk_cnt = b->enc.d_nz_chunk_cnt.p; nzf.overflow = b->out.d_overflow.p;
            nzf.blk_cnt = (b->tr.trellis && b->tr.t_sort) ? b->tr.d_tblk_cnt.p : nullptr;
            nzf.blk_off = (nzf.blk_cnt && b->tr.nz_once) ? b->tr.d_tblk_off.p : nullptr;
        }
        if (nw && getenv("CSH_DEBUG") && (uint32_t(atoi(getenv("CSH_DEBUG"))) & 32768u))
            CSH_CHECK(hipMemsetAsync(b->d_coef.p + size_t(b->ntiles_in) * CSH_TILE_I16, 0x5A, size_t(b->ntiles - b->ntiles_in) * CSH_TILE_I16 * sizeof(int16_t), st));
        launch_xform_direct(st, b->d_imgs.p, b->pix.d_pwork.p, nw, b->max_tiles, b->d_quants.p, b->d_coef.p, b->d_coef.p, rawp, b->ntiles_in, b->tr.dering, nzf);
        MARK(KS_XFORM_DIRECT);
        launch_resample_plane(st, b->d_imgs.p, b->pix.d_pwork.p, nw, b->pix.max_quads, b->pix.d_planes.p, b->pix.d_oplanes.p);
        if (b->pix.any_layout) launch_resample_any(st, b->d_imgs.p, b->pix.d_pwork.p, nw, b->pix.max_quads, b->pix.d_planes.p, b->pix.d_oplanes.p);
        launch_plane_fdct(st, b->d_imgs.p, b->pix.d_pwork.p, nw, b->max_tiles, b->d_quants.p, b->pix.d_oplanes.p, b->d_coef.p, rawp, b->ntiles_in, b->tr.dering, nzf);
        launch_resample_fdct_420(st, b->d_imgs.p, b->pix.d_pwork.p, nw, b->max_tiles, b->d_quants.p, b->pix.d_planes.p, b->d_coef.p, rawp, b->ntiles_in, b->tr.dering, nzf);
        MARK(KS_RESAMPLE_FDCT);
        if (!b->lossless) launch_fix_dummy(st, b->d_imgs.p, nimg, b->max_dummy, b->d_coef.p);
        MARK(KS_FIX_DUMMY);
        return 0;
    }

    void fill_enc_ctx() {
        memset(&c, 0, sizeof c);
        c.imgs = b->d_imgs.p; c.script = b->enc.d_script.p; c.work = b->enc.d_swork.p; c.nwork = int(b->enc.swork.size());
        c.echunks = b->enc.d_echunks.p; c.plans = b->enc.d_plans.p; c.nechunks = uint32_t(b->enc.echunks.size()); c.slot_work = b->enc.d_slot_work.p; c.slots = b->enc.d_slots.p; c.nslots = b->enc.nslots;
        c.coef = b->d_coef.p; c.sym_bits = b->enc.d_symbits.p; c.eob_bits = b->enc.d_eobbits.p; c.tail = b->enc.d_tail.p;
        c.eobrun = b->enc.d_eobrun.p; c.long_runs = b->enc.d_long_runs.p; c.long_cnt = b->enc.d_long_cnt.p; c.corr = b->enc.d_corr.p; c.lastn = b->enc.d_lastn.p; c.ref_pack = b->enc.ref_pack ? 1u : 0u;
        c.tokens = b->enc.d_tokens.p; c.regions = b->enc.d_regions.p; c.tok_cursor = b->enc.d_tok_cursor.p; c.tok_off = b->enc.d_tok_off.p; c.chunk_ntok = b->enc.d_chunk_ntok.p; c.slot_hist = b->enc.d_slot_hist.p; c.slot_raw = b->enc.d_slot_raw.p; c.slot_eobh = b->enc.d_slot_eobh.p;
        c.chunk_bits = b->enc.d_chunk_bits.p; c.chunk_off = b->enc.d_chunk_off.p; c.tables = b->enc.d_tables.p;
        c.raw = b->enc.d_raw.p; c.raw_words = raw_chunks * 16; c.status = b->out.d_status.p; c.overflow = b->out.d_overflow.p;
        c.nzlists = b->enc.d_nzlists.p; c.nzsets = b->enc.d_nzsets.p; c.nz_pool = b->enc.d_nz_pool.p; c.nz_cursor = b->enc.d_nz_cursor.p; c.nz_chunk_off = b->enc.d_nz_chunk_off.p; c.nz_chunk_cnt = b->enc.d_nz_chunk_cnt.p;
        c.debug = getenv("CSH_DEBUG") ? uint32_t(atoi(getenv("CSH_DEBUG"))) : 0u;
    }
    void fill_asm_ctx() {
        memset(&a, 0, sizeof a);
        a.imgs = b->d_imgs.p; a.script = b->enc.d_script.p; a.work = b->enc.d_swork.p; a.nimg = nimg;
        a.nwork = b->tr.trellis ? int(b->tr.tstage.work0) : c.nwork;
        a.tables = b->enc.d_tables.p; a.chunk_off = b->enc.d_chunk_off.p; a.scan_pad_bytes = b->enc.d_scan_pad.p; a.scan_raw_off = b->enc.d_scan_raw_off.p;
        a.raw = b->enc.d_raw.p; a.raw_chunks = raw_chunks; a.chunk_ff = b->enc.d_chunk_ff.p;
        a.hdr_pool = b->enc.d_hdr.p; a.hdr_off = b->enc.d_hdr_off.p; a.img_size = b->out.d_img_size.p; a.img_size_pad = b->out.d_img_size_pad.p;
        a.img_off = b->out.d_img_off.p; a.out = b->out.d_out.p; a.out_cap = b->out.out_cap; a.status = b->out.d_status.p; a.overflow = b->out.d_overflow.p;
        a.img_list = b->enc.d_img_list.p; a.img_nlist = b->enc.d_img_nlist.p; a.scan_cost = b->enc.d_scan_cost.p;
    }
    void fill_trellis_ctx(TrellisCtx &tc) {
        memset(&tc, 0, sizeof tc);
        tc.imgs = b->d_imgs.p; tc.quant = b->d_quants.p; tc.work = b->tr.d_twork.p; tc.nwork = int(b->tr.twork.size()); tc.runs = b->tr.d_truns.p; tc.nruns = uint32_t(b->tr.truns.size());
        tc.tables = b->enc.d_tables.p; tc.raw = b->pix.d_dct_raw.p; tc.raw_tile0 = b->ntiles_in; tc.coef = b->d_coef.p; tc.dcrec = b->tr.d_tlambda.p; tc.dcbt = b->tr.d_tdcbt.p;
        tc.spill = b->tr.d_tspill.p; tc.nslots = uint32_t(b->tr.d_tspill.n / trellis_spill_words(1)); tc.max_rows = b->tr.t_max_rows;
        tc.queue = b->tr.d_tqueue.p;
        tc.rows = b->tr.d_trows.p; tc.nrows = uint32_t(b->tr.trows.size());
        if (b->tr.t_sort) { tc.blk_cnt = b->tr.d_tblk_cnt.p; tc.perm = b->tr.d_tperm.p; }
        if (b->tr.t_sort && b->tr.nz_once) {
            tc.nz_pool = b->enc.d_nz_pool.p; tc.nzlists = b->enc.d_nzlists.p; tc.nzsets = b->enc.d_nzsets.p; tc.nz_chunk_off = b->enc.d_nz_chunk_off.p; tc.nz_chunk_cnt = b->enc.d_nz_chunk_cnt.p;
            tc.blk_off = b->tr.d_tblk_off.p;
        }
        tc.ac_lists = fused ? 1u : 0u;
        tc.debug = getenv("CSH_TR_DEBUG") ? uint32_t(atoi(getenv("CSH_TR_DEBUG"))) : 0u;
    }

    int encode_begin() {
        fill_enc_ctx();
        launch_reset_works(st, b->enc.d_swork.p, c.nwork);
        if (!fused && (b->enc.d_nz_cursor.zero(st) || b->enc.d_nz_chunk_cnt.zero(st))) return -1;
        if (b->enc.d_symbits.zero(st) || b->enc.d_eobbits.zero(st) || (!eobrun_cleared && b->enc.d_eobrun.zero(st)) || b->enc.d_tables.zero(st) || b->enc.d_tok_cursor.zero(st) || b->enc.d_slot_eobh.zero(st) || b->enc.d_scan_pad.zero(st)) return -1;
#ifdef CSH_EMUL
        if (b->enc.d_raw.zero(st)) return -1;
#else
        if ((c.debug & 8192u) && b->enc.d_raw.zero(st)) return -1;
#endif
        MARK(KS_MEMSET_ENC);
        return 0;
    }

    void count_list_runs(const Stage &sg, bool gate) {
        for (uint32_t wi = sg.work0; (sg.nlr || sg.nrr) && wi < sg.work0 + sg.nwork; wi++) {
            const ScanWork &w = b->enc.swork[wi];
            if ((w.lr_base != 0xFFFFFFFFu || w.rr_base != 0xFFFFFFFFu) && (!gate || b->enc.work_active[wi])) b->enc.last_run_list_runs += ((w.nunits + 255u) / 256u + b->enc.list_run - 1u) / b->enc.list_run;
        }
    }

    void set_stage(const Stage &sg) {
        c.echunks = b->enc.d_echunks.p + sg.ech0; c.nechunks = sg.nech; c.slot0 = sg.slot0; c.nslots = sg.nslots;
        c.nzchunks = (fused ? b->enc.d_nzchunks_fused.p : b->enc.d_nzchunks.p) + sg.nzc0; c.nnzchunks = sg.nnzc;
        c.nz_build = sg.nz_build[fused ? 1 : 0]; c.nz_filter = sg.nz_filter[fused ? 1 : 0];
        c.list_slots = b->enc.d_list_slots.p + sg.ls0; c.nlist_slots = sg.nls; c.tok_slots = b->enc.d_tok_slots.p + sg.ts0; c.ntok_slots = sg.nts;
        c.ref_slots = b->enc.d_ref_slots.p + sg.rs0; c.nref_slots = sg.nrs;
        c.list_runs = b->enc.d_list_runs.p + sg.lr0; c.nlist_runs = sg.nlr; c.ref_runs = b->enc.d_ref_runs.p + sg.rr0; c.nref_runs = sg.nrr; c.list_run = b->enc.list_run;
        c.ac_runs_slot = b->enc.ac_runs_slot ? 1u : 0u;
    }

    int trellis() {
        const Stage &tg = b->tr.tstage;
        set_stage(tg);
        c.stats_only = 1;
        if (b->enc.d_long_cnt.zero(st)) return -1;
        c.nz_blk_cnt = b->tr.t_sort ? b->tr.d_tblk_cnt.p : nullptr;
        c.nz_blk_off = (b->tr.t_sort && b->tr.nz_once) ? b->tr.d_tblk_off.p : nullptr;
        launch_nzlist(st, c);
        c.nz_blk_cnt = nullptr; c.nz_blk_off = nullptr;
        if (b->tr.t_sort) {
            TrellisCtx ts;
            memset(&ts, 0, sizeof ts);
            ts.work = b->tr.d_twork.p; ts.nwork = int(b->tr.twork.size()); ts.blk_cnt = b->tr.d_tblk_cnt.p; ts.perm = b->tr.d_tperm.p;
            launch_trellis_sort(st, ts);
        }
        launch_tokens(st, c);
        launch_list_stats(st, c);
        count_list_runs(tg, false);
        launch_ac_runs(st, c);
        launch_gen_tables(st, b->enc.d_tables.p + tg.table0, int(tg.ntables));
        c.stats_only = 0;
        if (b->enc.d_nz_cursor.zero(st)) return -1;
        MARK(KS_TRELLIS_STATS);
        TrellisCtx tc;
        fill_trellis_ctx(tc);
        if (b->tr.d_tqueue.zero(st)) return -1;
        launch_trellis_ac(st, tc);
        MARK(KS_TRELLIS_AC);
        launch_trellis_dc(st, tc);
        launch_fix_dummy(st, b->d_imgs.p, nimg, b->max_dummy, b->d_coef.p);
        MARK(KS_TRELLIS_DC);
        return 0;
    }

    int stage(const Stage &sg, bool mark, bool gate) {
#define SMARK(slot) do { if (mark) MARK(slot); } while (0)
        set_stage(sg);
        c.work_active = gate ? b->enc.d_work_active.p : nullptr;
        a.work0 = int(sg.work0); a.nwork_run = int(sg.nwork);
        if (b->enc.d_long_cnt.zero(st)) return -1;
        launch_nzlist(st, c);
        SMARK(KS_NZLIST);
        launch_list_refine(st, c);
        for (uint32_t wi = sg.work0; sg.nrs && wi < sg.work0 + sg.nwork; wi++)
            if (b->enc.swork[wi].rs_base != 0xFFFFFFFFu && (!gate || b->enc.work_active[wi])) { b->enc.last_run_refine++; if (b->enc.ref_pack) b->enc.last_run_ref_packed++; }
        count_list_runs(sg, gate);
        launch_tokens(st, c);
        SMARK(KS_TOKENS);
        launch_list_stats(st, c);
        SMARK(KS_LIST_STATS);
        launch_ac_runs(st, c);
        SMARK(KS_AC_RUNS);
        launch_gen_tables(st, b->enc.d_tables.p + sg.table0, int(sg.ntables));
        SMARK(KS_GEN_TABLES);
        launch_chunk_sizes(st, c);
        SMARK(KS_CHUNK_SIZES);
        launch_exclusive_scan(st, b->enc.d_chunk_bits.p + sg.slot0, b->enc.d_chunk_off.p + sg.slot0, sg.nslots, b->enc.d_scan_tmp.p, b->enc.d_scan_tmp.n);
        SMARK(KS_SCAN_CHUNK_BITS);
        launch_scan_sizes(st, a);
        launch_exclusive_scan(st, b->enc.d_scan_pad.p, b->enc.d_scan_raw_off.p, uint64_t(a.nwork), b->enc.d_scan_tmp.p, b->enc.d_scan_tmp.n);
        launch_scan_place(st, a);
        launch_zero_edges(st, c);
        SMARK(KS_SCAN_LAYOUT);
        launch_pack(st, c);
        launch_list_refine_pack(st, c);
        SMARK(KS_PACK);
        launch_list_pack(st, c);
        SMARK(KS_LIST_PACK);
        launch_ff_count(st, a);
        SMARK(KS_FF_COUNT);
#undef SMARK
        return 0;
    }

    int gated_stage(int sid, int (*want)(const SearchImg &)) {
        if (!search_gate(b, sid, want)) return 0;
        b->enc.n_gated_runs++;
        if (b->enc.d_work_active.upload(b->enc.work_active, st)) return -1;
        if (stage(b->enc.stage[sid], false, true) || search_costs(b, a, sid)) return -1;
        return search_decide(b, sid);
    }
    int search() {
        b->enc.n_gated_runs = 0;
        if (search_costs(b, a, EncodePlan::ST_1) || search_decide(b, EncodePlan::ST_1)) return -1;
        if (gated_stage(EncodePlan::ST_1B, [](const SearchImg &si) { return si.luma_on ? 1 : 0; })) return -1;
        if (stage(b->enc.stage[EncodePlan::ST_2], false, false)) return -1;
        if (search_costs(b, a, EncodePlan::ST_2) || search_decide(b, EncodePlan::ST_2)) return -1;
        for (int sid : {int(EncodePlan::ST_2B), int(EncodePlan::ST_2C)})
            if (gated_stage(sid, [](const SearchImg &si) { return (si.luma_on ? 1 : 0) | (si.chroma_on ? 2 : 0); })) return -1;
        if (search_lists(b)) return -1;
        return 0;
    }

    int emit() {
        MARK(KS_SCAN_SEARCH);
        launch_layout(st, a);
        MARK(KS_LAYOUT);
        launch_exclusive_scan(st, b->out.d_img_size_pad.p, b->out.d_img_off.p, uint64_t(nimg), b->enc.d_scan_tmp.p, b->enc.d_scan_tmp.n);
        MARK(KS_SCAN_IMAGES);
        launch_emit(st, a);
        MARK(KS_EMIT);
        return 0;
    }

    int finish(bool phases) {
        CSH_CHECK(hipStreamSynchronize(st));
        CSH_CHECK(hipGetLastError());
        if (t && marks.read(t, phases)) return -1;
        if (t && !phases) t->n_images = uint32_t(nimg);
        return 0;
    }

    int webp() {
        const int nwimg = int(b->wp.wimgs.size());
        uint64_t out_bytes = 0;
        std::vector<uint64_t> off(size_t(b->nimg) + 1, 0);
        for (auto &wi : b->wp.wimgs) {
            const uint64_t cap = 4096 + uint64_t(wi.mbw) * wi.mbh * (b->wp.webp_mb_bytes + 2);
            wi.out_cap = uint32_t(std::min<uint64_t>(cap, 0xFFFFFF00u)); wi.out_off = out_bytes;
            off[wi.image] = out_bytes;
            out_bytes += (wi.out_cap + 63) & ~uint64_t(63);
            const int q = int(b->params.webp_quality);
            wi.quality = q < 0 ? 0 : q > 100 ? 100 : q;
        }
        off[b->nimg] = out_bytes;
        if (b->out.d_out.n < out_bytes + 64 && b->out.d_out.alloc(out_bytes + 64)) return -1;
        if ((b->wp.d_wscratch.n < out_bytes + 64 && b->wp.d_wscratch.alloc(out_bytes + 64)) || (b->wp.d_wpart.n < size_t(b->nimg) * 9 + 9 && b->wp.d_wpart.alloc(size_t(b->nimg) * 9 + 9)) ||
            (b->wp.d_wstats.n < size_t(b->nimg) * 2112 + 8 && (b->wp.d_wstats.alloc(size_t(b->nimg) * 2112 + 8) || b->wp.d_wprobs.alloc(size_t(b->nimg) * 1056 + 8) || b->wp.d_wupdate.alloc(size_t(b->nimg) * 1056 + 8))))
            return -1;
        if (b->wp.d_wstats.zero(st)) return -1;
        if (b->wp.d_wimgs.upload(b->wp.wimgs, st) || (b->wp.d_wwork.n < b->wp.wwork_bytes + 64 && b->wp.d_wwork.alloc(b->wp.wwork_bytes + 64)) ||
            (b->wp.d_wlevels.n < b->wp.wlevels + 64 && b->wp.d_wlevels.alloc(b->wp.wlevels + 64)))
            return -1;
        CSH_CHECK(hipMemcpyAsync(b->out.d_img_off.p, off.data(), off.size() * sizeof(uint64_t), hipMemcpyHostToDevice, st));
        if (b->out.d_img_size.zero(st)) return -1;
        csw::launch_webp_yuv(st, b->wp.d_wimgs.p, nwimg, b->wp.wmax_luma, b->pix.d_rgb.p, b->wp.d_wwork.p);
        MARK(KS_WEBP_YUV);
        hipEvent_t mid;
        if (marks.claim(KS_WEBP_ENCODE, &mid)) return -1;
        if (csw::launch_webp_encode(st, b->wp.wimgs.data(), nwimg, b->wp.d_wimgs.p, b->wp.d_wwork.p, b->wp.d_wlevels.p, b->wp.d_wscratch.p, b->wp.d_wpart.p, b->out.d_out.p, b->out.d_img_size.p, b->out.d_status.p, mid)) return -1;
        MARK(KS_WEBP_ASSEMBLE);
        return finish(false);
    }
};

}

int run_once(csh_batch *b, csh_timing *t, bool requant_only) {
    Run r(b, t);
    b->enc.last_run_list_runs = 0;
    b->enc.last_run_fused = 0; b->enc.last_run_refine = 0; b->enc.last_run_ref_packed = 0; b->enc.last_run_ac_lists = 0;
    if (r.pools() || r.marks.start()) return -1;
    const bool from_pixels = requant_only && b->tr.dering;
    if (requant_only && !from_pixels) {
        if (r.requant()) return -1;
    } else {
        if (from_pixels ? r.skip_decode() : r.decode()) return -1;
        if (r.planes()) return -1;
        if (b->webp) return r.webp();
        if (b->rgb_out) return (r.marks.mark(KS_XFORM_DIRECT) || r.finish(false)) ? -1 : 0;
        if (r.pixels()) return -1;
    }
    if (r.encode_begin()) return -1;
    b->enc.last_run_fused = r.fused ? b->enc.n_fused : 0u;
    b->enc.last_run_ac_lists = r.fused ? b->enc.n_ac_lists : 0u;
    if (b->tr.trellis ? r.trellis() : r.marks.skip_to(KS_NZLIST)) return -1;
    r.fill_asm_ctx();
    if (r.stage(b->enc.stage[0], true, false)) return -1;
    if (b->enc.search && r.search()) return -1;
    return (r.emit() || r.finish(true)) ? -1 : 0;
}

}
```

### caesium-clt_amd/csrc/k_decode_par.hip

```cpp
#include "kernels.h"

namespace csh {

__device__ static int scan_of_byte(const ParScan *ps, int nps, uint32_t byte) {
    int lo = 0, hi = nps;
    while (hi - lo > 1) { int mid = (lo + hi) >> 1; if (ps[mid].bits_off <= byte) lo = mid; else hi = mid; }
    return lo;
}

#define CSH_US_STRIDE 17
__device__ __forceinline__ static uint32_t zero_bytes(uint32_t w) { return ~(((w & 0x7F7F7F7Fu) + 0x7F7F7F7Fu) | w | 0x7F7F7F7Fu); }
__device__ __forceinline__ static void unstuff_stage(const uint8_t *raw, uint32_t c0, uint32_t nchunks, uint32_t *lw, uint32_t tid) {
    const uint32_t *g = reinterpret_cast<const uint32_t *>(raw);
    for (uint32_t i = 0; i < 16; i++) {
        uint32_t d = i * 256 + tid, chunk = c0 + d / 16;
        lw[(d / 16) * CSH_US_STRIDE + d % 16] = chunk < nchunks ? g[size_t(c0) * 16 + d] : 0u;
    }
    if (tid == 0) lw[256 * CSH_US_STRIDE] = c0 ? g[size_t(c0) * 16 - 1] : 0u;
}
__device__ __forceinline__ static uint32_t unstuff_masks(const uint32_t *lw, uint32_t tid, uint32_t b0, uint32_t lo, uint32_t end, uint32_t del[16]) {
    uint32_t prev = tid ? lw[(tid - 1) * CSH_US_STRIDE + 15] : lw[256 * CSH_US_STRIDE];
    uint32_t carry = (b0 > lo) ? (zero_bytes(~prev) >> 24) : 0u;
    uint32_t n = 0;
    for (int j = 0; j < 16; j++) {
// ... 115 lines not shown
};
#define CSH_LROW_WORDS 35
#define CSH_LROW_STRIDE 35
struct RowReader {
    const uint32_t *row;
    __device__ __forceinline__ uint32_t word(uint32_t r) const {
#ifdef CSH_EMUL
        if (r >= CSH_LROW_WORDS) { fprintf(stderr, "decode_span: stream window exceeded (%u)\n", r); abort(); }
#endif
        return row[r];
    }
};
#define CSH_SWZ_WORDS (257 * 32)
struct SwzReader {
    const uint32_t *lds;
    uint32_t tl;
    __device__ __forceinline__ static uint32_t index(uint32_t row, uint32_t r) { return (row << 5) + ((r + row) & 31u); }
    __device__ __forceinline__ uint32_t word(uint32_t r) const {
#ifdef CSH_EMUL
        if (r >= CSH_LROW_WORDS) { fprintf(stderr, "decode_span: stream window exceeded (%u)\n", r); abort(); }
#endif
        return lds[index(tl + (r >> 5), r & 31u)];
    }
};

__device__ __forceinline__ static int extend_p(int r, int n) { return r < (1 << (n - 1)) ? r - (1 << n) + 1 : r; }

struct ParCtx {
    uint64_t sel;
    int nb_mcu;
    uint32_t total_blocks;
    int mcus_x;
    uint32_t first_mcu;
    uint32_t real_bits;
    int Ss, Se, Al;
};
__device__ __forceinline__ static ParCtx make_ctx(const ParScan &ps, const ImgDesc *im) {
    ParCtx c; c.sel = ps.sel; c.nb_mcu = ps.nb_mcu; c.total_blocks = ps.total_blocks;
    c.mcus_x = im ? (ps.ncomp > 1 ? im->mcus_x : im->in[ps.comp_of[0]].real_bw) : 1;
    c.first_mcu = ps.first_mcu;
    c.real_bits = ps.clean_len * 8u;
    c.Ss = ps.Ss; c.Se = ps.Se; c.Al = ps.Al;
    return c;
}
__device__ __forceinline__ static void make_block_info(const ParScan &ps, const ImgDesc &im, int m, ParBlockInfo &o) {
    const CompGeom &g = im.in[ps.comp_of[m]];
    o.tile_base = g.tile_base;
    if (ps.ncomp > 1) { o.row_step = g.v * g.bw; o.col_step = g.h; o.first = ps.by_of[m] * g.bw + ps.bx_of[m]; }
    else { o.row_step = g.bw; o.col_step = 1; o.first = 0; }
    o.dc_first = ps.dc_base[m] + ps.dc_idx[m]; o.dc_per_mcu = ps.dc_per_mcu[m];
}

template <bool WRITE, int KIND, class R>
__device__ __forceinline__ static uint32_t decode_span(const R &rd, uint32_t w0, const uint8_t *hb, uint32_t sub_off, const ParCtx &cx, PState &st, uint32_t stop_bit,
                                                        uint32_t ordinal, const ParBlockInfo *bi, int16_t *coef, int32_t *dcdiff, uint32_t *hand_over = nullptr) {
    uint32_t nblk = 0;
    int16_t *blk = nullptr;
    int32_t *dcp = nullptr;
    const uint16_t *sub = reinterpret_cast<const uint16_t *>(hb + sub_off);
    uint32_t mcu = 0; int mx = 0, my = 0;
    bool in_range = false;
    auto word = [&](uint32_t wi) -> uint32_t { const uint32_t r = wi - w0; return (WRITE && r >= CSH_LROW_WORDS) ? 0u : rd.word(r); };
    uint32_t cut_mcu = 0xFFFFFFFFu;
    const bool dead = WRITE && st.pos > cx.real_bits;
    auto locate = [&](int m) {
        in_range = __umul24(mcu, uint32_t(cx.nb_mcu)) + uint32_t(m) < cx.total_blocks && mcu <= cut_mcu && !dead;
        const ParBlockInfo g = bi[m];
        blk = coef + coef_index(g.tile_base, __mul24(my, g.row_step) + __mul24(mx, g.col_step) + g.first, 0);
        dcp = dcdiff + (__umul24(mcu, g.dc_per_mcu) + g.dc_first);
    };
    uint32_t pos = st.pos, wi = (pos >> 5) + 2;
    int k = st.k, m = st.m;
    const int k_first = KIND == CSH_PS_AC_FIRST ? cx.Ss : 0;
    int cur_oct = -1, shared_oct = k > 0 ? (k >> 3) : -1;
    uint64_t olo = 0, ohi = 0;
    auto flush = [&](bool piecewise) {
        int16_t *dst = blk + cur_oct * CSH_OCT_STRIDE;
        if (!piecewise) *reinterpret_cast<uint4 *>(dst) = uint4{uint32_t(olo), uint32_t(olo >> 32), uint32_t(ohi), uint32_t(ohi >> 32)};
        else {
            CSH_UNROLL
            for (int i = 0; i < 8; i++) { const uint32_t c = uint32_t(((i & 4) ? ohi : olo) >> (16 * (i & 3))) & 0xFFFFu; if (c) dst[i] = int16_t(c); }
        }
        cur_oct = -1; olo = 0; ohi = 0;
    };
    if (WRITE) {
        mcu = ordinal / uint32_t(cx.nb_mcu);
        my = int(mcu + cx.first_mcu) / cx.mcus_x; mx = int(mcu + cx.first_mcu) - my * cx.mcus_x;
        locate(m);
    }
    uint32_t dco, aco;
    auto tables = [&](int mm) { uint32_t x = uint32_t(cx.sel >> __umul24(uint32_t(mm), 6u)); dco = (x & 7u) << 10; aco = (x & 56u) << 7; };
    tables(m);
    uint64_t acc = ((uint64_t(word(wi - 2)) << 32) | word(wi - 1)) << (pos & 31);
    int nb = 64 - int(pos & 31);
    uint32_t nxt = word(wi);
    auto step = [&]() {
        const uint32_t w = uint32_t(acc >> 32), top16 = w >> 16;
        const bool isdc = KIND == CSH_PS_DC_FIRST ? true : (KIND == CSH_PS_AC_FIRST ? false : k == 0);
        uint32_t e = *reinterpret_cast<const uint16_t *>(hb + (isdc ? dco : aco) + ((top16 >> 7) << 1));
        if (e & 0x8000u) e = sub[(e & 0xFFFu) + ((top16 & 127u) >> (7u - ((e >> 12) & 7u)))];
        const int len = e ? int(e >> 8) : 16;
        const int sym = int(e & 255u);
        const int n = sym & 15, r = isdc ? 0 : (sym >> 4);
        const int kn = k + r;
        const bool val = n != 0 && kn <= 63;
        const bool eobrun = KIND == CSH_PS_AC_FIRST && n == 0 && r != 15;
        const int nx = eobrun ? r : n;
        int v = int((w << len) >> ((32 - nx) & 31));
        uint32_t run = 1;
        if (eobrun) { run = (1u << r) + (r ? uint32_t(v) : 0u); v = 0; }
        else { v = v < int(1u << ((n - 1) & 31)) ? v - (1 << n) + 1 : v; v = val ? v : 0; }
        if (WRITE && in_range) {
            if (KIND == CSH_PS_AC_FIRST) {
                if (val) blk[coef_off(kn)] = int16_t(v * (1 << cx.Al));
                if (val && kn > cx.Se) *hand_over = 2u;
            }
            else if (isdc) *dcp = v;
            else if (val) {
                const int oct = kn >> 3;
                if (oct != cur_oct) { if (cur_oct >= 0) flush(cur_oct == shared_oct); cur_oct = oct; }
                const uint64_t piece = uint64_t(uint32_t(v) & 0xFFFFu) << (16 * (kn & 3));
                if (kn & 4) ohi |= piece; else olo |= piece;
            }
        }
        const int used = len + (eobrun ? r : (val ? n : 0));
        const bool eob = KIND == CSH_PS_AC_FIRST ? eobrun : (!isdc && n == 0 && r != 15);
        const int kc = kn > 63 ? 63 : kn;
        if (KIND == CSH_PS_DC_FIRST) k = 64;
        else if (KIND == CSH_PS_AC_FIRST) k = (eob || kn > 63 || kc + 1 > cx.Se) ? 64 : kc + 1;
        else k = eob ? 64 : kc + 1;
        pos += uint32_t(used);
        acc <<= used;
        nb -= used;
        if (nb < 32) { acc |= uint64_t(nxt) << (32 - nb); nb += 32; wi++; nxt = word(wi); }
        if (k >= 64) {
            if (WRITE && KIND == CSH_PS_SEQ) { if (cur_oct >= 0) flush(cur_oct == shared_oct); shared_oct = -1; }
            k = k_first;
            nblk += run;
            if (WRITE) cut_mcu = (pos > cx.real_bits && mcu < cut_mcu) ? mcu : cut_mcu;
            const bool wrap = m + 1 == cx.nb_mcu;
            m = wrap ? 0 : m + 1;
            tables(m);
            if (WRITE) {
                if (KIND == CSH_PS_AC_FIRST) {
                    mcu += run;
                    if (run == 1) { if (++mx == cx.mcus_x) { mx = 0; my++; } }
                    else { my = int(mcu + cx.first_mcu) / cx.mcus_x; mx = int(mcu + cx.first_mcu) - my * cx.mcus_x; }
                } else if (wrap) { mcu++; if (++mx == cx.mcus_x) { mx = 0; my++; } }
                locate(m);
            }
        }
    };
    while (pos < stop_bit) step();
    if (WRITE && !dead)
        while (pos > cx.real_bits && (k != k_first || m != 0) && __umul24(mcu, uint32_t(cx.nb_mcu)) < cx.total_blocks) step();
    if (WRITE && KIND == CSH_PS_SEQ && cur_oct >= 0) flush(true);
    st.pos = pos; st.k = k; st.m = m;
    return WRITE ? ((cut_mcu == 0xFFFFFFFFu || dead) ? 0xFFFFFFFFu : (cut_mcu + 1u) * uint32_t(cx.nb_mcu)) : nblk;
}

#define CSH_SPAN(WR, KINDV, ...)                                                                        \
    ((KINDV) == CSH_PS_AC_FIRST ? decode_span<WR, CSH_PS_AC_FIRST>(__VA_ARGS__)                          \
                                : (KINDV) == CSH_PS_DC_FIRST ? decode_span<WR, CSH_PS_DC_FIRST>(__VA_ARGS__) : decode_span<WR, CSH_PS_SEQ>(__VA_ARGS__))
__device__ __forceinline__ static bool par_decoded(int kind) { return kind == CSH_PS_SEQ || kind == CSH_PS_DC_FIRST || kind == CSH_PS_AC_FIRST; }

#define CSH_LIST_LANES 512
#define CSH_LIST_WALK 8
template <class SET>
__global__ void __launch_bounds__(CSH_LIST_LANES) k_dec_relax_list(const uint8_t *clean, const ParScan *pss, const SET *huffs, uint64_t *state, const uint64_t *state_rd,
                                                         uint32_t *nblk, const uint64_t *list_in, const uint32_t *cnt_in, uint64_t *list_out, uint32_t *cnt_out,
                                                         uint32_t *claim, uint32_t epoch, uint32_t walk_below) {
    CSH_SHARED uint32_t lbits[CSH_LIST_LANES * CSH_LROW_STRIDE];
    CSH_SHARED SET lhs;
    CSH_SHARED uint32_t d_scan[CSH_LIST_LANES], d_t[CSH_LIST_LANES];
    const uint32_t tid = threadIdx.x, j = blockIdx.x * blockDim.x + tid, count = *cnt_in;
    const uint32_t j0 = blockIdx.x * blockDim.x;
    CSH_PHASE_LOOP(3) {
        if (j0 >= count) continue;
        if (phase == 0) {
            uint32_t si = 0xFFFFFFFFu, t = 0;
            if (j < count) {
                uint64_t e = list_in[j]; si = uint32_t(e >> 32); t = uint32_t(e);
                if (atomicExch(&claim[pss[si].sub_base + t], epoch) == epoch) si = 0xFFFFFFFFu;
            }
            d_scan[tid] = si; d_t[tid] = t;
            const uint32_t *src = reinterpret_cast<const uint32_t *>(&huffs[pss[uint32_t(list_in[j0] >> 32)].huff_set]);
            uint32_t *dst = reinterpret_cast<uint32_t *>(&lhs);
            for (uint32_t i = tid; i < sizeof(SET) / 4; i += CSH_LIST_LANES) dst[i] = src[i];
            continue;
        }
        if (phase == 1) {
            const uint32_t wave0 = tid & ~63u, lane = tid & 63u;
            for (uint32_t r = 0; r < 64; r++) {
                uint32_t si = d_scan[wave0 + r];
                if (si == 0xFFFFFFFFu || lane >= CSH_LROW_WORDS) continue;
                const ParScan &ps = pss[si];
                PReader g; g.base = clean + ps.bits_off; g.len = ps.clean_len;
                lbits[(wave0 + r) * CSH_LROW_STRIDE + lane] = g.word(d_t[wave0 + r] * (CSH_SUBSEQ_BYTES / 4) + lane);
            }
            continue;
        }
        if (j >= count || d_scan[tid] == 0xFFFFFFFFu) continue;
        const ParScan &ps = pss[d_scan[tid]];
        uint32_t t = d_t[tid];
        const size_t base = ps.sub_base + ps.par_index;
        PState st = unpack_state(state_rd[base + t]);
        uint32_t *row = lbits + tid * CSH_LROW_STRIDE;
        RowReader rd; rd.row = row;
        const ParCtx cx = make_ctx(ps, nullptr);
        const int staged_set = pss[uint32_t(list_in[j0] >> 32)].huff_set;
        const uint8_t *hb = ps.huff_set == staged_set ? reinterpret_cast<const uint8_t *>(&lhs) : reinterpret_cast<const uint8_t *>(&huffs[ps.huff_set]);
        PReader g; g.base = clean + ps.bits_off; g.len = ps.clean_len;
        for (int step = 0;; step++) {
            const uint32_t w0 = t * (CSH_SUBSEQ_BYTES / 4), stop = (t + 1) * CSH_SUBSEQ_BYTES * 8;
            const uint32_t n = CSH_SPAN(false, ps.kind, rd, w0, hb, uint32_t(sizeof(SET::root)), cx, st, stop, 0, nullptr, nullptr, nullptr);
            nblk[ps.sub_base + t] = n;
            const uint64_t e = pack_state(st);
            if (e == state[base + t + 1]) break;
            state[base + t + 1] = e;
            if ((t + 1) * CSH_SUBSEQ_BYTES >= ps.clean_len) break;
            if (count < walk_below && step + 1 < CSH_LIST_WALK && atomicExch(&claim[ps.sub_base + t + 1], epoch) != epoch) {
                t++;
                for (uint32_t i = 0; i < CSH_LROW_WORDS; i++) row[i] = g.word(t * (CSH_SUBSEQ_BYTES / 4) + i);
                continue;
            }
            list_out[atomicAdd(cnt_out, 1u)] = (uint64_t(ps.par_index) << 32) | (t + 1);
            break;
        }
    }
}

__global__ void __launch_bounds__(256) k_dec_mark_pending(const ParScan *pss, const uint64_t *list_in, const uint32_t *cnt_in, uint32_t *scan_pending) {
    uint32_t j = blockIdx.x * blockDim.x + threadIdx.x;
    if (j >= *cnt_in) return;
    scan_pending[uint32_t(list_in[j] >> 32)] = 1;
}
__global__ void k_dec_chain(const ParScan *pss, int nps, uint64_t *state, uint32_t *nblk, const uint16_t *hyp, const uint32_t *scan_pending, uint32_t *need_seq) {
    int si = blockIdx.x * blockDim.x + threadIdx.x;
    if (si >= nps || !scan_pending[si] || !par_decoded(pss[si].kind)) return;
    const ParScan &ps = pss[si];
    if (ps.kind == CSH_PS_AC_FIRST) { need_seq[ps.image] = 2; return; }
    uint32_t nsub = (ps.bits_len + CSH_SUBSEQ_BYTES - 1) / CSH_SUBSEQ_BYTES;
    size_t base = ps.sub_base + ps.par_index;
    int m = 0;
    for (uint32_t t = 0; t < nsub && t * CSH_SUBSEQ_BYTES < ps.clean_len; t++) {
        PState st = unpack_state(state[base + t]);
        st.m = m;
        state[base + t] = pack_state(st);
        uint16_t h = hyp[(size_t(ps.sub_base) + t) * 10 + m];
        if (h == 0xFFFF) { need_seq[ps.image] = 2; return; }
        nblk[ps.sub_base + t] = h & 4095u;
        m = h >> 12;
    }
}

template <int MODE, class SET>
__global__ void __launch_bounds__(256) k_dec_dense(DenseArgs a) {
    CSH_SHARED uint32_t lbits[CSH_SWZ_WORDS];
    CSH_SHARED SET lhs;
    CSH_SHARED ParBlockInfo lbi[10];
    auto clear_region = [&](uint8_t *ptr, uint64_t bytes) __attribute__((always_inline)) {
        if (!bytes) return;
        const uint64_t nwg = uint64_t(gridDim.x) * gridDim.y, wg = uint64_t(blockIdx.y) * gridDim.x + blockIdx.x;
        const uint64_t share = ((bytes / 16 + nwg - 1) / nwg) * 16, z0 = wg * share, z1 = z0 + share < bytes ? z0 + share : bytes;
        for (uint64_t off = z0 + uint64_t(threadIdx.x) * 16; off < z1; off += 256 * 16) {
#ifdef CSH_EMUL
            memset(ptr + off, 0, 16);
#else
            __builtin_nontemporal_store(0ull, reinterpret_cast<unsigned long long *>(ptr + off));
            __builtin_nontemporal_store(0ull, reinterpret_cast<unsigned long long *>(ptr + off + 8));
#endif
        }
    };
    auto clear_share = [&]() __attribute__((always_inline)) {
        if (MODE != 0 && MODE != 1) return;
        clear_region(a.zero_ptr, a.zero_bytes);
        clear_region(a.zero2_ptr, a.zero2_bytes);
    };
    const ParScan &ps = a.pss[blockIdx.y];
    if (!par_decoded(ps.kind)) { clear_share(); return; }
    const uint32_t nsub = (ps.bits_len + CSH_SUBSEQ_BYTES - 1) / CSH_SUBSEQ_BYTES;
    const uint32_t t0 = blockIdx.x * 256, tid = threadIdx.x, t = t0 + tid;
    const bool wg_live = t0 < nsub && t0 * CSH_SUBSEQ_BYTES < ps.clean_len && !(MODE == 2 && a.need_seq[ps.image] == 1) &&
                         !(MODE == 3 && a.scan_pending[ps.par_index] == 0);
    PReader g; g.base = a.clean + ps.bits_off; g.len = ps.clean_len;
    CSH_PHASE_LOOP(2) {
        if (phase == 0) {
            if (MODE == 1 && t < nsub && t * CSH_SUBSEQ_BYTES >= ps.clean_len) a.nblk[ps.sub_base + t] = 0;
            if (!wg_live) continue;
            const uint32_t *src = reinterpret_cast<const uint32_t *>(&static_cast<const SET *>(a.huffs)[ps.huff_set]);
            uint32_t *dst = reinterpret_cast<uint32_t *>(&lhs);
            for (uint32_t i = tid; i < sizeof(SET) / 4; i += 256) dst[i] = src[i];
            if (MODE == 2 && int(tid) < ps.nb_mcu && tid < 10) make_block_info(ps, a.imgs[ps.image], int(tid), lbi[tid]);
            const uint32_t w_first = t0 * (CSH_SUBSEQ_BYTES / 4);
            for (uint32_t i = 0; i < CSH_SUBSEQ_BYTES / 4 + 1; i++) {
                uint32_t d = i * 256 + tid;
                if (d >= 256 * (CSH_SUBSEQ_BYTES / 4) + (CSH_LROW_WORDS - CSH_SUBSEQ_BYTES / 4)) break;
                lbits[SwzReader::index(d >> 5, d & 31u)] = g.word(w_first + d);
            }
            continue;
        }
        if (!wg_live || t >= nsub) continue;
        size_t base = ps.sub_base + ps.par_index;
        const bool live = t * CSH_SUBSEQ_BYTES < ps.clean_len;
        SwzReader rd; rd.lds = lbits; rd.tl = tid;
        const uint32_t w0 = t * (CSH_SUBSEQ_BYTES / 4), stop = (t + 1) * CSH_SUBSEQ_BYTES * 8;
        const uint8_t *hb = reinterpret_cast<const uint8_t *>(&lhs);
        const uint32_t sub_off = uint32_t(sizeof(SET::root));
        const ParCtx cx = make_ctx(ps, MODE == 2 ? &a.imgs[ps.image] : nullptr);
        if (MODE == 0) {
            PState st; st.pos = t * CSH_SUBSEQ_BYTES * 8; st.m = 0; st.k = ps.kind == CSH_PS_AC_FIRST ? ps.Ss : 0;
            if (t == 0) a.state[base] = pack_state(st);
            if (!live) { a.state[base + t + 1] = 0; continue; }
            CSH_SPAN(false, ps.kind, rd, w0, hb, sub_off, cx, st, stop, 0, nullptr, nullptr, nullptr);
            a.state[base + t + 1] = pack_state(st);
        } else if (MODE == 1) {
            if (!live) continue;
            PState st = unpack_state(a.state[base + t]);
            uint32_t n = CSH_SPAN(false, ps.kind, rd, w0, hb, sub_off, cx, st, stop, 0, nullptr, nullptr, nullptr);
            a.nblk[ps.sub_base + t] = n;
            uint64_t e = pack_state(st);
            if (e != a.state[base + t + 1]) {
                a.state[base + t + 1] = e;
                if ((t + 1) * CSH_SUBSEQ_BYTES < ps.clean_len) a.list_out[atomicAdd(a.cnt_out, 1u)] = (uint64_t(ps.par_index) << 32) | (t + 1);
            }
        } else if (MODE == 3) {
            if (!live) continue;
            const PState s0 = unpack_state(a.state[base + t]);
            const PState nx = unpack_state(a.state[base + t + 1]);
            const bool last = (t + 1) * CSH_SUBSEQ_BYTES >= ps.clean_len;
            for (int m0 = 0; m0 < ps.nb_mcu && m0 < 10; m0++) {
                PState st = s0; st.m = m0;
                uint32_t n = CSH_SPAN(false, ps.kind, rd, w0, hb, sub_off, cx, st, stop, 0, nullptr, nullptr, nullptr);
                const bool same = last || (st.pos == nx.pos && st.k == nx.k);
                a.hyp[(size_t(ps.sub_base) + t) * 10 + m0] = same ? uint16_t((st.m << 12) | (n > 4095 ? 4095 : n)) : uint16_t(0xFFFF);
            }
        } else {
            { const uint32_t ns = a.need_seq[ps.image]; if (ns && ns != 4u) continue; }
            uint32_t ordinal = uint32_t(a.blk_off[ps.sub_base + t] - a.blk_off[ps.sub_base]);
            if (!live || ordinal >= ps.total_blocks) continue;
            PState st = unpack_state(a.state[base + t]);
            const uint32_t cut = CSH_SPAN(true, ps.kind, rd, w0, hb, sub_off, cx, st, stop, ordinal, lbi, a.coef, a.dcdiff, a.need_seq + ps.image);
            if (cut != 0xFFFFFFFFu) atomicMin(&a.cut_block[ps.par_index], cut);
        }
    }
    clear_share();
}

__global__ void __launch_bounds__(256) k_dc_scatter(const ParScan *pss, const ImgDesc *imgs, const uint64_t *dc_off, int16_t *coef, const uint32_t *need_seq,
                                                     const uint32_t *cut_block) {
    const ParScan &ps = pss[blockIdx.y];
    if (ps.kind != CSH_PS_SEQ && ps.kind != CSH_PS_DC_FIRST) return;
    { const uint32_t ns = need_seq[ps.image]; if (ns && ns != 4u) return; }
    uint32_t j = blockIdx.x * blockDim.x + threadIdx.x;
    if (j >= ps.total_blocks) return;
    const ImgDesc &im = imgs[ps.image];
    uint32_t mcu = j / uint32_t(ps.nb_mcu);
    int m = int(j - mcu * uint32_t(ps.nb_mcu));
    const CompGeom &g = im.in[ps.comp_of[m]];
    int by, bx;
    const int amcu = int(mcu + ps.first_mcu);
    if (ps.ncomp > 1) { int my = amcu / im.mcus_x, mx = amcu - my * im.mcus_x; by = my * g.v + ps.by_of[m]; bx = mx * g.h + ps.bx_of[m]; }
    else { by = amcu / g.real_bw; bx = amcu - by * g.real_bw; }
    uint32_t idx = ps.dc_base[m] + mcu * ps.dc_per_mcu[m] + ps.dc_idx[m];
    uint32_t v = uint32_t(dc_off[idx + 1] - dc_off[ps.dc_base[m]]);
    if (j >= cut_block[blockIdx.y]) v = 0;
    coef[coef_index(g.tile_base, by * g.bw + bx, 0)] = int16_t(int32_t(v) * (1 << (ps.kind == CSH_PS_DC_FIRST ? ps.Al : 0)));
}
__global__ void __launch_bounds__(256) k_dc_refine(const uint8_t *clean, const ParScan *pss, const ImgDesc *imgs, int16_t *coef, const uint32_t *need_seq) {
    const ParScan &ps = pss[blockIdx.y];
    if (ps.kind != CSH_PS_DC_REFINE || need_seq[ps.image] != 4u) return;
    const uint32_t j = blockIdx.x * blockDim.x + threadIdx.x;
    if (j >= ps.total_blocks || (j >> 3) >= ps.clean_len) return;
    if (!((clean[ps.bits_off + (j >> 3)] >> (7u - (j & 7u))) & 1u)) return;
    const ImgDesc &im = imgs[ps.image];
    const uint32_t mcu = j / uint32_t(ps.nb_mcu);
    const int m = int(j - mcu * uint32_t(ps.nb_mcu));
    const CompGeom &g = im.in[ps.comp_of[m]];
    int by, bx;
    if (ps.ncomp > 1) { const int my = int(mcu) / im.mcus_x, mx = int(mcu) - my * im.mcus_x; by = my * g.v + ps.by_of[m]; bx = mx * g.h + ps.bx_of[m]; }
    else { by = int(mcu) / g.real_bw; bx = int(mcu) - by * g.real_bw; }
    int16_t *p = coef + coef_index(g.tile_base, by * g.bw + bx, 0);
    const uintptr_t a = reinterpret_cast<uintptr_t>(p);
    atomicOr(reinterpret_cast<uint32_t *>(a & ~uintptr_t(3)), (1u << ps.Al) << ((a & 2u) ? 16 : 0));
}

void launch_unstuff_count(hipStream_t st, const uint8_t *raw, const ParScan *ps, int nps, uint32_t nchunks, uint32_t *cnt) {
    if (nchunks) CSH_LAUNCH_PHASED(k_unstuff_count, 2, dim3((nchunks + 255) / 256), dim3(256), st, raw, ps, nps, nchunks, cnt);
}
void launch_unstuff_copy(hipStream_t st, const uint8_t *raw, uint8_t *clean, ParScan *ps, int nps, uint32_t nchunks, const uint64_t *off) {
    if (nchunks) CSH_LAUNCH_PHASED(k_unstuff_copy, 2, dim3((nchunks + 255) / 256), dim3(256), st, raw, clean, ps, nps, nchunks, off);
}
void launch_dec_dense(hipStream_t st, int mode, int nps, uint32_t max_sub, const DenseArgs &a) {
    if (!nps || !max_sub) return;
    dim3 grid((max_sub + 255) / 256, nps);
#define CSH_DENSE(M) do { if (a.compact) CSH_LAUNCH_PHASED((k_dec_dense<M, ParHuffSet4>), 2, grid, dim3(256), st, a); \
                          else CSH_LAUNCH_PHASED((k_dec_dense<M, ParHuffSet>), 2, grid, dim3(256), st, a); } while (0)
    if (mode == 0) CSH_DENSE(0);
    else if (mode == 1) CSH_DENSE(1);
    else if (mode == 2) CSH_DENSE(2);
    else CSH_DENSE(3);
#undef CSH_DENSE
}
#ifdef CSH_EMUL
int csh_emul_jacobi = 0;
#endif
void launch_dec_relax_list(hipStream_t st, const uint8_t *clean, const ParScan *ps, uint32_t total_sub, const void *huffs, int compact, uint64_t *state, uint32_t *nblk,
                           const uint64_t *list_in, const uint32_t *cnt_in, uint64_t *list_out, uint32_t *cnt_out, size_t nstate, uint32_t *claim, uint32_t epoch) {
    const uint32_t walk_below = epoch > 10 ? 0xFFFFFFFFu : total_sub / 1024 + 1;
    if (!total_sub) return;
    const uint64_t *state_rd = state;
#ifdef CSH_EMUL
    uint64_t *snap = nullptr;
    if (csh_emul_jacobi) { snap = (uint64_t *)malloc(nstate * 8); memcpy(snap, state, nstate * 8); state_rd = snap; }
#else
    (void)nstate;
#endif
    if (compact) CSH_LAUNCH_PHASED(k_dec_relax_list<ParHuffSet4>, 3, dim3((total_sub + CSH_LIST_LANES - 1) / CSH_LIST_LANES), dim3(CSH_LIST_LANES), st, clean, ps, static_cast<const ParHuffSet4 *>(huffs), state, state_rd, nblk, list_in, cnt_in, list_out, cnt_out, claim, epoch, walk_below);
    else CSH_LAUNCH_PHASED(k_dec_relax_list<ParHuffSet>, 3, dim3((total_sub + CSH_LIST_LANES - 1) / CSH_LIST_LANES), dim3(CSH_LIST_LANES), st, clean, ps, static_cast<const ParHuffSet *>(huffs), state, state_rd, nblk, list_in, cnt_in, list_out, cnt_out, claim, epoch, walk_below);
#ifdef CSH_EMUL
    free(snap);
#endif
}
void launch_dec_mark_pending(hipStream_t st, const ParScan *ps, uint32_t total_sub, const uint64_t *list_in, const uint32_t *cnt_in, uint32_t *scan_pending) {
    if (total_sub) CSH_LAUNCH(k_dec_mark_pending, dim3((total_sub + 255) / 256), dim3(256), st, ps, list_in, cnt_in, scan_pending);
}
void launch_dec_chain(hipStream_t st, const ParScan *ps, int nps, uint64_t *state, uint32_t *nblk, const uint16_t *hyp, const uint32_t *scan_pending, uint32_t *need_seq) {
    if (nps) CSH_LAUNCH(k_dec_chain, dim3((nps + 63) / 64), dim3(64), st, ps, nps, state, nblk, hyp, scan_pending, need_seq);
}
void launch_dc_refine(hipStream_t st, const uint8_t *clean, const ParScan *ps, int nps, uint32_t max_blocks, const ImgDesc *imgs, int16_t *coef, const uint32_t *need_seq) {
    if (nps && max_blocks) CSH_LAUNCH(k_dc_refine, dim3((max_blocks + 255) / 256, nps), dim3(256), st, clean, ps, imgs, coef, need_seq);
}
void launch_dc_scatter(hipStream_t st, const ParScan *ps, int nps, uint32_t max_blocks, const ImgDesc *imgs, const uint64_t *dc_off, int16_t *coef,
                       const uint32_t *need_seq, const uint32_t *cut_block) {
    if (nps && max_blocks) CSH_LAUNCH(k_dc_scatter, dim3((max_blocks + 255) / 256, nps), dim3(256), st, ps, imgs, dc_off, coef, need_seq, cut_block);
}

}
```

### caesium-clt_amd/csrc/kernels.h

```cpp
#pragma once
#include "gpu_rt.h"
#include "types.h"

namespace csh {

__host__ __device__ static inline int coef_off(int k) { return (k >> 3) * CSH_OCT_STRIDE + (k & 7); }
__host__ __device__ static inline size_t coef_index(uint32_t tile_base, int b, int k) {
    return (size_t(tile_base) + size_t(b >> 6)) * CSH_TILE_I16 + size_t((b & 63) * CSH_BLK_STRIDE) + size_t(coef_off(k));
}

#define CSH_RAW_OCT 8
__host__ __device__ static inline size_t raw_index(uint32_t tile_base, int b) { return size_t(tile_base) * CSH_TILE_I16 + size_t(b) * 64; }

__device__ __forceinline__ static int csh_plane_at(const uint8_t *p, int pitch, int cw, int ch, int y, int x) {
    y = y < 0 ? 0 : (y > ch - 1 ? ch - 1 : y);
    x = x < 0 ? 0 : (x > cw - 1 ? cw - 1 : x);
    return p[size_t(y) * pitch + x];
}
__device__ __forceinline__ static int csh_upsample_at(const uint8_t *p, int pitch, int cw, int ch, UpDesc u, int r, int xx) {
    switch (u.cls) {
    case CSH_UP_COPY: return csh_plane_at(p, pitch, cw, ch, r, xx);
    case CSH_UP_H2V1: {
        const int cx = xx >> 1, nb = (xx & 1) ? cx + 1 : cx - 1;
        return (3 * csh_plane_at(p, pitch, cw, ch, r, cx) + csh_plane_at(p, pitch, cw, ch, r, nb) + ((xx & 1) ? 2 : 1)) >> 2;
    }
    case CSH_UP_H1V2: {
        const int cy = r >> 1, fy = (r & 1) ? cy + 1 : cy - 1;
        return (3 * csh_plane_at(p, pitch, cw, ch, cy, xx) + csh_plane_at(p, pitch, cw, ch, fy, xx) + ((r & 1) ? 2 : 1)) >> 2;
    }
    case CSH_UP_H2V2: {
        const int cy = r >> 1, cx = xx >> 1, fy = (r & 1) ? cy + 1 : cy - 1, nb = (xx & 1) ? cx + 1 : cx - 1;
        const int cs = 3 * csh_plane_at(p, pitch, cw, ch, cy, cx) + csh_plane_at(p, pitch, cw, ch, fy, cx);
        const int cn = 3 * csh_plane_at(p, pitch, cw, ch, cy, nb) + csh_plane_at(p, pitch, cw, ch, fy, nb);
        return (3 * cs + cn + ((xx & 1) ? 7 : 8)) >> 4;
    }
    default: return csh_plane_at(p, pitch, cw, ch, r / int(u.vx), xx / int(u.hx));
    }
}

void launch_decode_seq(hipStream_t st, const uint8_t *bits, ImgDesc *imgs, const DecScan *scans, const DevHuffSet *huffs,
                       int16_t *coef, int nimg, const uint32_t *need_seq);

void launch_unstuff_count(hipStream_t st, const uint8_t *raw, const ParScan *ps, int nps, uint32_t nchunks, uint32_t *cnt);
void launch_unstuff_copy(hipStream_t st, const uint8_t *raw, uint8_t *clean, ParScan *ps, int nps, uint32_t nchunks, const uint64_t *off);
struct DenseArgs {
    const uint8_t *clean; const ParScan *pss; const void *huffs; int compact;
    uint64_t *state; uint32_t *nblk; uint64_t *list_out; uint32_t *cnt_out;
    uint16_t *hyp; const uint32_t *scan_pending;
    const uint64_t *blk_off; const ImgDesc *imgs; int16_t *coef; int32_t *dcdiff; uint32_t *need_seq;
    uint32_t *cut_block;
    uint8_t *zero_ptr; uint64_t zero_bytes;
    uint8_t *zero2_ptr; uint64_t zero2_bytes;
};
void launch_dec_dense(hipStream_t st, int mode , int nps, uint32_t max_sub, const DenseArgs &a);
void launch_dec_relax_list(hipStream_t st, const uint8_t *clean, const ParScan *ps, uint32_t total_sub, const void *huffs, int compact, uint64_t *state, uint32_t *nblk,
                           const uint64_t *list_in, const uint32_t *cnt_in, uint64_t *list_out, uint32_t *cnt_out, size_t nstate, uint32_t *claim, uint32_t epoch);
void launch_refine_chains(hipStream_t st, const uint8_t *clean, const ParScan *pss, const ParHuffSet *huffs, const DecScan *scans, const ProgChain *chains,
                          const int *chain_scans, int nchains, const RefineUnit *units, int nunits, uint32_t max_blocks, const ImgDesc *imgs, int16_t *coef,
                          uint32_t *need_seq, uint64_t *hist, uint32_t *posv, uint32_t *prog);
void launch_rebind_slots(hipStream_t st, const ScanWork *works, uint32_t nworks, const NzList *nzlists, SlotRec *slots);
void launch_make_slots(hipStream_t st, const ScanWork *works, uint32_t nworks, const EncScan *script, const NzList *nzlists, SlotRec *slots, uint32_t *slot_work, uint32_t *list_slots,
                       uint32_t *tok_slots, uint32_t *ref_slots, uint32_t *list_runs, uint32_t *ref_runs, uint32_t list_run);
void launch_decode_prog(hipStream_t st, const uint8_t *clean, const ParScan *pss, const ParHuffSet *huffs, const DecScan *scans, const ProgChain *chains,
                        const int *chain_scans, int nchains, const ImgDesc *imgs, int16_t *coef, uint32_t *need_seq);
void launch_dec_mark_pending(hipStream_t st, const ParScan *ps, uint32_t total_sub, const uint64_t *list_in, const uint32_t *cnt_in, uint32_t *scan_pending);
void launch_dec_chain(hipStream_t st, const ParScan *ps, int nps, uint64_t *state, uint32_t *nblk, const uint16_t *hyp, const uint32_t *scan_pending, uint32_t *need_seq);
void launch_dc_refine(hipStream_t st, const uint8_t *clean, const ParScan *ps, int nps, uint32_t max_blocks, const ImgDesc *imgs, int16_t *coef, const uint32_t *need_seq);
void launch_dc_scatter(hipStream_t st, const ParScan *ps, int nps, uint32_t max_blocks, const ImgDesc *imgs, const uint64_t *dc_off, int16_t *coef,
                       const uint32_t *need_seq, const uint32_t *cut_block);

struct NzFuse {
    const NzSet *nzsets; const NzList *nzlists;
    uint32_t *nz_pool, *nz_cursor, *nz_chunk_off, *nz_chunk_cnt;
    uint8_t *blk_cnt; uint16_t *blk_off;
    uint32_t *overflow;
};
void launch_xform_direct(hipStream_t st, const ImgDesc *imgs, const PlaneWork *work, int nwork, int max_tiles, const DevQuant *quant,
                         const int16_t *coef_in, int16_t *coef_out, int16_t *dct_raw, uint32_t raw_tile0, bool dering, const NzFuse &nzf);
void launch_requant(hipStream_t st, const ImgDesc *imgs, const PlaneWork *work, int nwork, int max_tiles, const DevQuant *quant, const int16_t *dct_raw,
                    uint32_t raw_tile0, int16_t *coef_out);
void launch_idct_plane(hipStream_t st, const ImgDesc *imgs, const PlaneWork *work, int nwork, int max_tiles, const DevQuant *quant,
                       const int16_t *coef_in, uint8_t *planes);
void launch_resample_plane(hipStream_t st, const ImgDesc *imgs, const PlaneWork *work, int nwork, uint32_t max_quads, const uint8_t *planes, uint8_t *oplanes);
void launch_plane_fdct(hipStream_t st, const ImgDesc *imgs, const PlaneWork *work, int nwork, int max_tiles, const DevQuant *quant,
                       const uint8_t *oplanes, int16_t *coef_out, int16_t *dct_raw, uint32_t raw_tile0, bool dering, const NzFuse &nzf);
void launch_resample_fdct_420(hipStream_t st, const ImgDesc *imgs, const PlaneWork *work, int nwork, int max_tiles, const DevQuant *quant,
                              const uint8_t *planes, int16_t *coef_out, int16_t *dct_raw, uint32_t raw_tile0, bool dering, const NzFuse &nzf);
void launch_resample_any(hipStream_t st, const ImgDesc *imgs, const PlaneWork *work, int nwork, uint32_t max_quads, const uint8_t *planes, uint8_t *oplanes);
void launch_fix_dummy(hipStream_t st, const ImgDesc *imgs, int nimg, int max_blocks, int16_t *coef_out);

bool resize_is_fused(uint32_t max_row_in);
void launch_resize(hipStream_t st, const ImgDesc *imgs, const ResizeWork *work, int nwork, const ResizeTap *taps, const float *weights,
                   uint8_t *planes, uint8_t *rgb, float *tmp, uint32_t max_src_px, uint64_t max_tmp, uint64_t max_dst, uint32_t max_row_in, uint32_t max_out_w, uint32_t max_nh, bool to_planes,
                   bool any_layout = false, bool any_space = false);

struct EncCtx {
    const ImgDesc *imgs;
    const EncScan *script;
    const ScanWork *work;
    int nwork;
    const EChunk *echunks;
    uint32_t nechunks;
    const TokPlan *plans;
    const uint32_t *slot_work;
    const SlotRec *slots;
    uint32_t slot0, nslots;
    const int16_t *coef;
    uint64_t *sym_bits;
    uint64_t *eob_bits;
    uint8_t *tail;
    uint16_t *eobrun;
    uint32_t *long_runs, *long_cnt;
    uint64_t *corr;
    uint32_t *tokens;
    const TokRegion *regions;
    uint32_t *tok_cursor;
    uint64_t *tok_off;
    uint32_t *chunk_ntok;
    uint16_t *slot_hist;
    uint32_t *slot_raw;
    uint32_t *slot_eobh;
    uint32_t *chunk_bits;
    const uint64_t *chunk_off;
    DevEncTable *tables;
    uint32_t *raw;
    uint64_t raw_words;
    uint32_t *status;
    uint32_t *overflow;
    uint32_t debug;
    uint32_t stats_only;
    const uint8_t *work_active;
    const NzList *nzlists;
    const NzSet *nzsets;
    const NzChunk *nzchunks;
    uint32_t nnzchunks;
    uint32_t *nz_pool;
    uint32_t *nz_cursor;
    uint32_t *nz_chunk_off;
    uint32_t *nz_chunk_cnt;
    uint8_t *nz_blk_cnt;
    uint16_t *nz_blk_off;
    const uint32_t *list_slots;
    uint32_t nlist_slots;
    const uint32_t *tok_slots;
    uint32_t ntok_slots;
    const uint32_t *ref_slots;
    uint32_t nref_slots;
    const uint32_t *list_runs;
    uint32_t nlist_runs;
    const uint32_t *ref_runs;
    uint32_t nref_runs;
    uint32_t list_run;
    uint16_t *lastn;
    uint32_t ref_pack;
    uint32_t ac_runs_slot;
    uint32_t nz_build, nz_filter;
};
enum : uint32_t { TK_SYM = 0u, TK_RAW = 1u, TK_ACF = 2u, TK_REF = 3u, TK_EOB = 4u };
void launch_tokens(hipStream_t st, const EncCtx &c);
void launch_ac_runs(hipStream_t st, const EncCtx &c);
void launch_gen_tables(hipStream_t st, DevEncTable *tables, int ntables);
void launch_chunk_sizes(hipStream_t st, const EncCtx &c);
void launch_zero_edges(hipStream_t st, const EncCtx &c);
void launch_pack(hipStream_t st, const EncCtx &c);
void launch_nzlist(hipStream_t st, const EncCtx &c);
void launch_list_stats(hipStream_t st, const EncCtx &c);
void launch_list_refine(hipStream_t st, const EncCtx &c);
void launch_list_pack(hipStream_t st, const EncCtx &c);
void launch_list_refine_pack(hipStream_t st, const EncCtx &c);
void launch_nz_to_tiles(hipStream_t st, const NzSet *nzsets, const NzList *nzlists, const uint32_t *nz_pool, const uint32_t *nz_chunk_off, const uint32_t *nz_chunk_cnt,
                        uint32_t set, uint32_t nchunks, int16_t *coef);
void launch_reset_works(hipStream_t st, ScanWork *work, int nwork);

#ifndef CSH_LIST_RUN
#define CSH_LIST_RUN 8
#endif
#ifndef CSH_TR_WG
#define CSH_TR_WG 256
#endif
#ifndef CSH_TR_RUN
#define CSH_TR_RUN 8
#endif
struct TrellisCtx {
    const ImgDesc *imgs;
    const DevQuant *quant;
    const TrellisWork *work;
    int nwork;
    const TrellisRun *runs;
    uint32_t nruns;
    uint32_t *queue;
    uint32_t nslots;
    const DevEncTable *tables;
    const int16_t *raw;
    uint32_t raw_tile0;
    int16_t *coef;
    uint64_t *dcrec;
    uint64_t *dcbt;
    uint32_t *spill;
    uint32_t max_rows;
    const uint8_t *blk_cnt;
    uint32_t *perm;
    const uint32_t *rows;
    uint32_t nrows;
    uint32_t debug;
    uint32_t *nz_pool;
    const NzList *nzlists;
    const NzSet *nzsets;
    const uint32_t *nz_chunk_off, *nz_chunk_cnt;
    const uint16_t *blk_off;
// ... 46 lines not shown
```

### caesium-clt_amd/csrc/pipeline.cpp

```cpp
#include <algorithm>
#include <atomic>
#include <cmath>
#include <cstdarg>
#include <memory>
#include <thread>

#include "batch.hpp"
#include "../../include/vp8_tables.h"
#include "resize_host.h"

static thread_local char g_err[512];
void csh_set_error(const char *fmt, ...) {
    va_list ap;
    va_start(ap, fmt);
    vsnprintf(g_err, sizeof g_err, fmt, ap);
    va_end(ap);
}
extern "C" const char *csh_last_error(void) { return g_err; }

#ifdef CSH_EMUL
thread_local dim3 threadIdx, blockIdx, blockDim, gridDim;
int csh_emul_reverse = 0;
thread_local int csh_emul_phase = 0;
extern "C" void csh_emul_set_reverse(int r) { csh_emul_reverse = r; }
// ... 76 lines not shown
    plan.begin();
    plan.parse();
    laps.lap("stream+parse");
    if (int rc = plan.reserve_pinned()) return rc;
    laps.lap("pinned");
    for (size_t n = 0; n < count; n++)
        if (int rc = plan.plan_image(n)) return rc;
    if (int rc = plan.plan_search_stages()) return rc;
    if (int rc = plan.plan_trellis()) return rc;
    plan.finish_descriptors();
    laps.lap("descriptors");
    if (int rc = plan.upload(laps)) return rc;
    if (laps.trace) fprintf(stderr, "[csh] create %zu files:%s\n", count, laps.text.c_str());
    *out = b.release();
    return 0;
}
extern "C" int csh_batch_create(const CByteArray *inputs, size_t count, const CCSParameters *p, int device, csh_batch **out) { return batch_create(inputs, count, p, device, false, out); }
extern "C" int csh_batch_create_pixels(const CByteArray *inputs, size_t count, const CCSParameters *p, int device, csh_batch **out) { return batch_create(inputs, count, p, device, false, out, true); }
extern "C" int csh_batch_create_webp(const CByteArray *inputs, size_t count, const CCSParameters *p, int device, csh_batch **out) { return batch_create(inputs, count, p, device, true, out); }

static std::vector<uint8_t> standin_jpeg(uint32_t w, uint32_t h, uint32_t nc) {
    std::vector<uint8_t> f = {0xFF, 0xD8, 0xFF, 0xDB, 0x00, 0x43, 0x00};
    f.insert(f.end(), 64, 1);
    const uint8_t sof[] = {0xFF, 0xC0, 0x00, uint8_t(8 + 3 * nc), 8, uint8_t(h >> 8), uint8_t(h), uint8_t(w >> 8), uint8_t(w), uint8_t(nc)};
    f.insert(f.end(), sof, sof + sizeof sof);
    for (uint32_t c = 0; c < nc; c++) { f.push_back(uint8_t(c + 1)); f.push_back(0x11); f.push_back(0); }
    for (int cls = 0; cls < 2; cls++) {
        const uint8_t dht[] = {0xFF, 0xC4, 0x00, 0x14, uint8_t(cls << 4), 1, 0, 0, 0, 0, 0, 0, 0, 0, 0, 0, 0, 0, 0, 0, 0, 0x00};
        f.insert(f.end(), dht, dht + sizeof dht);
    }
    const uint8_t sos[] = {0xFF, 0xDA, 0x00, uint8_t(6 + 2 * nc), uint8_t(nc)};
    f.insert(f.end(), sos, sos + sizeof sos);
    for (uint32_t c = 0; c < nc; c++) { f.push_back(uint8_t(c + 1)); f.push_back(0x00); }
    f.push_back(0); f.push_back(63); f.push_back(0);
    const uint64_t bits = uint64_t((w + 7) / 8) * ((h + 7) / 8) * nc * 2;
    f.insert(f.end(), size_t(bits / 8), 0x00);
    if (bits % 8) f.push_back(uint8_t(0xFF >> (bits % 8)));
    f.push_back(0xFF); f.push_back(0xD9);
    return f;
}
static int create_from_pixels(const csp_pixels *sources, size_t count, const CCSParameters *p, int device, csh_batch **out, bool webp, bool rgb_out) {
    *out = nullptr;
    const uint32_t max_side = webp ? 16383 : 65535;
    std::vector<std::vector<uint8_t>> files(count);
    std::vector<CByteArray> in(count);
    for (size_t i = 0; i < count; i++) {
        const csp_pixels &s = sources[i];
        if (!s.device_pixels || !s.width || !s.height || s.width > max_side || s.height > max_side || (s.channels != 1 && s.channels != 3)) files[i] = {'?'};
        else files[i] = standin_jpeg(s.width, s.height, s.channels);
        in[i].data = files[i].data(); in[i].length = files[i].size();
    }
    return batch_create(in.data(), count, p, device, webp, out, rgb_out, sources);
}
extern "C" int csh_batch_create_from_pixels(const csp_pixels *sources, size_t count, const CCSParameters *p, int device, csh_batch **out) { return create_from_pixels(sources, count, p, device, out, false, false); }
extern "C" int csh_batch_create_from_pixels_rgb(const csp_pixels *sources, size_t count, const CCSParameters *p, int device, csh_batch **out) { return create_from_pixels(sources, count, p, device, out, false, true); }
extern "C" int csh_batch_create_webp_from_pixels(const csp_pixels *sources, size_t count, const CCSParameters *p, int device, csh_batch **out) { return create_from_pixels(sources, count, p, device, out, true, false); }

extern "C" void csh_batch_destroy(csh_batch *b) { delete b; }

extern "C" const char *csh_kernel_name(int i) { return (i >= 0 && i < CSH_NKERNELS) ? kKernelSlots[i].name : ""; }
extern "C" const char *csh_kernel_name_webp(int i) {
    return i == KS_WEBP_YUV ? "k_webp_yuv" : i == KS_WEBP_ENCODE ? "k_vp8_analyse+segments+loop" : i == KS_WEBP_ASSEMBLE ? "k_webp_hdr+decisions+bool+assemble" : csh_kernel_name(i);
}

static int batch_run(csh_batch *b, csh_timing *t, bool requant_only);
extern "C" int csh_batch_run(csh_batch *b, csh_timing *t) { return batch_run(b, t, false); }

extern "C" int csh_batch_retain_dct(csh_batch *b, int on) {
    if (b->lossless) { csh_set_error("retain_dct: a coefficient transcode has no quality to re-target"); return -1; }
    b->retain_dct = on != 0;
    if (b->retain_dct && b->nimg && b->pix.d_dct_raw.n == 0 && b->pix.d_dct_raw.alloc(size_t(b->ntiles_out) * CSH_TILE_I16)) return -1;
    return 0;
}
extern "C" int csh_batch_set_quality(csh_batch *b, const uint32_t *quality) {
    if (b->lossless) { csh_set_error("set_quality on a lossless batch"); return -1; }
    b->enc.hdr_pool.clear(); b->enc.hdr_off.clear();
    for (size_t n = 0; n < b->items.size(); n++) {
        Item &it = b->items[n];
        if (it.image < 0) continue;
        ImgDesc &im = b->imgs[it.image];
        if (quality[n]) {
            int q = int(quality[n]) < 1 ? 1 : (quality[n] > 100 ? 100 : int(quality[n]));
            for (int c = 0; c < im.ncomp; c++) im.qt_out[c] = b->q_base + q;
        }
        JpegInfo hdr = it.out;
        int qidx = im.qt_out[0];
        uint16_t nat[64];
        for (int k = 0; k < 64; k++) nat[kZigZag[k]] = b->quants[qidx].q[k];
        memcpy(hdr.qt[0], nat, 128); memcpy(hdr.qt[1], nat, 128);
        std::vector<uint8_t> fh = build_frame_header(hdr, b->progressive, it.meta_out.empty() ? nullptr : &it.meta_out);
        b->enc.hdr_off.push_back(uint32_t(b->enc.hdr_pool.size()));
        b->enc.hdr_pool.insert(b->enc.hdr_pool.end(), fh.begin(), fh.end());
    }
    b->enc.hdr_off.push_back(uint32_t(b->enc.hdr_pool.size()));
    if (!b->nimg) return 0;
    if (hipSetDevice(b->device) != hipSuccess) return -1;
    if (b->d_imgs.upload(b->imgs, b->stream) || b->enc.d_hdr.upload(b->enc.hdr_pool, b->stream) || b->enc.d_hdr_off.upload(b->enc.hdr_off, b->stream)) return -1;
    CSH_CHECK(hipStreamSynchronize(b->stream));
    return 0;
}
extern "C" int csh_batch_rerun_encode(csh_batch *b, csh_timing *t) {
    if (!b->have_dct) { csh_set_error("rerun_encode needs a completed csh_batch_run after csh_batch_retain_dct(1)"); return -1; }
    return batch_run(b, t, true);
}

static int batch_run(csh_batch *b, csh_timing *t, bool requant_only) {
    if (t) memset(t, 0, sizeof *t);
    if (!b->nimg) { b->out.ran = true; return 0; }
    if (hipSetDevice(b->device) != hipSuccess) { csh_set_error("hipSetDevice failed"); return CS_ERR_NO_DEVICE; }
    for (int attempt = 0; attempt < 4; attempt++) {
        if (run_once(b, t, requant_only)) return CS_ERR_NO_DEVICE;
        uint32_t ovf[4] = {0, 0, 0, 0};
        if (csh_copy_wait(ovf, b->out.d_overflow.p, sizeof ovf, hipMemcpyDeviceToHost, b->stream) != hipSuccess) { csh_set_error("D2H failed"); return CS_ERR_NO_DEVICE; }
        b->out.h_status.resize(b->nimg);
        if (csh_copy_wait(b->out.h_status.data(), b->out.d_status.p, b->nimg * sizeof(uint32_t), hipMemcpyDeviceToHost, b->stream) != hipSuccess) return CS_ERR_NO_DEVICE;
        bool pool = ovf[0] != 0;
        if (ovf[1]) {
            pool = true; b->enc.tok_scale *= 4;
            layout_token_pool(b);
            if (b->enc.d_regions.upload(b->enc.regions, b->stream) || b->enc.d_nzlists.upload(b->enc.nzlists, b->stream) || hipStreamSynchronize(b->stream) != hipSuccess) return CS_ERR_NO_DEVICE;
        }
        for (uint32_t s : b->out.h_status) if (s == CS_ERR_POOL_OVERFLOW) pool = true;
        if (!pool) break;
        if (attempt == 3) { csh_set_error("device pools overflowed after 3 retries"); return CS_ERR_POOL_OVERFLOW; }
        b->out.raw_bytes_cap *= 4; b->out.out_cap = b->out.raw_bytes_cap;
        b->wp.webp_mb_bytes *= 4;
    }
    b->out.h_img_size.resize(b->nimg);
    b->out.h_img_off.resize(b->nimg + 1);
    if (csh_copy_wait(b->out.h_img_size.data(), b->out.d_img_size.p, b->nimg * sizeof(uint32_t), hipMemcpyDeviceToHost, b->stream) != hipSuccess ||
        csh_copy_wait(b->out.h_img_off.data(), b->out.d_img_off.p, (b->nimg + 1) * sizeof(uint64_t), hipMemcpyDeviceToHost, b->stream) != hipSuccess) {
        csh_set_error("D2H of sizes failed"); return CS_ERR_NO_DEVICE;
    }
    if (t) {
        std::vector<uint32_t> ns(b->nimg);
        if (csh_copy_wait(ns.data(), b->dec.d_need_seq.p, b->nimg * sizeof(uint32_t), hipMemcpyDeviceToHost, b->stream) != hipSuccess) return CS_ERR_NO_DEVICE;
        if (getenv("CSH_TRACE") && b->dec.d_relax_cnt.n) {
            std::vector<uint32_t> rc(b->dec.d_relax_cnt.n);
            if (csh_copy_wait(rc.data(), b->dec.d_relax_cnt.p, rc.size() * sizeof(uint32_t), hipMemcpyDeviceToHost, b->stream) == hipSuccess) {
                fprintf(stderr, "[csh] relax list sizes (of %u sub-sequences):", b->dec.total_sub);
                for (size_t i = 0; i < rc.size() && (i < 16 || rc[i]); i++) fprintf(stderr, " %u", rc[i]);
                fprintf(stderr, "\n");
            }
        }
        for (const ProgChain &pc : b->dec.chains) if (pc.refine && ns[size_t(pc.image)] == 4) t->n_refine_chains++;
        for (uint32_t v : ns) { if (v == 4) { t->n_prog_decoded++; continue; } if (v) t->n_seq_decoded++; if (v == 2 || v == 3) t->n_par_fallback++; if (v == 3) t->n_par_short++; }
        t->n_images = uint32_t(b->nimg);
        t->n_search_extra = b->enc.search ? b->enc.n_gated_runs : 0u;
        t->n_fused_lists = b->enc.last_run_fused;
        t->n_list_refine = b->enc.last_run_refine;
        t->n_ac_in_lists = b->enc.last_run_ac_lists;
        t->n_list_runs = b->enc.last_run_list_runs;
        t->n_ref_packed = b->enc.last_run_ref_packed;
        for (const Item &it : b->items) if (it.image < 0) t->n_failed++;
        for (int i = 0; i < b->nimg; i++) { t->out_bytes += b->out.h_img_size[i]; t->pixels += uint64_t(b->imgs[i].width) * b->imgs[i].height; }
        t->in_bytes = b->dec.bits_pool.size();
        uint64_t in_tiles = 0;
        for (const ImgDesc &im : b->imgs) for (int c = 0; c < im.ncomp_in; c++) in_tiles += im.in[c].ntiles;
        t->coef_bytes = in_tiles * CSH_TILE_I16 * 2;
    }
    b->out.ran = true;
    if (!requant_only) b->have_dct = (b->retain_dct || b->tr.trellis) && !b->lossless;
    return 0;
}

static void set_result(CCSResult *r, int code, const std::string &msg) {
    r->success = code == 0;
    r->code = uint32_t(code);
    r->error_message = nullptr;
    if (code) { char *m = (char *)malloc(msg.size() + 1); memcpy(m, msg.c_str(), msg.size() + 1); r->error_message = m; }
}

extern "C" int csh_batch_pixels(csh_batch *b, size_t image, const uint8_t **device_pixels, uint32_t *width, uint32_t *height, uint32_t *channels, const char **message) {
    *device_pixels = nullptr; *width = *height = *channels = 0;
    if (message) *message = "";
    if (!b || !b->out.ran || !b->rgb_out || image >= b->items.size()) { csh_set_error("csh_batch_pixels: not a pixel batch that has run"); if (message) *message = "not a pixel batch that has run"; return CS_ERR_NO_DEVICE; }
    const Item &it = b->items[image];
    if (it.code) { if (message) *message = it.msg.c_str(); return it.code; }
    if (b->out.h_status[it.image]) { if (message) *message = "device reported a malformed stream"; return int(b->out.h_status[it.image]); }
    if (size_t(it.image) < b->pix.rwork.size() && b->pix.rwork[size_t(it.image)].image == it.image) {
        const ResizeWork &rw = b->pix.rwork[size_t(it.image)];
        *device_pixels = b->pix.d_rgb.p + rw.rgb_dst_off; *width = uint32_t(rw.nw); *height = uint32_t(rw.nh); *channels = uint32_t(b->imgs[it.image].ncomp);
        return 0;
    }
    if (message) *message = "image has no pixel output";
    return CS_ERR_NO_DEVICE;
}

extern "C" int csh_batch_fetch(csh_batch *b, CByteArray *outputs, CCSResult *results) {
    if (!b->out.ran) { csh_set_error("csh_batch_fetch before csh_batch_run"); return -1; }
    if (b->rgb_out) { csh_set_error("csh_batch_fetch: a pixel batch has no files (csh_batch_pixels)"); return -1; }
    struct PinnedOut { uint8_t *p = nullptr; size_t cap = 0; ~PinnedOut() { if (p) pinned_cache().put(p, cap); } uint8_t *data() const { return p; } } host;
    if (b->nimg && b->out.h_img_off[b->nimg]) {
        host.p = static_cast<uint8_t *>(pinned_cache().get(b->out.h_img_off[b->nimg], host.cap));
        if (!host.p) { csh_set_error("out of pinned host memory"); return -1; }
        if (csh_copy_wait(host.p, b->out.d_out.p, b->out.h_img_off[b->nimg], hipMemcpyDeviceToHost, b->stream) != hipSuccess) { csh_set_error("D2H of output failed"); return -1; }
    }
    std::atomic<int> failed{0};
    std::atomic<size_t> next{0};
    auto worker = [&]() {
        for (size_t n; (n = next++) < b->items.size();) {
            Item &it = b->items[n];
            outputs[n].data = nullptr; outputs[n].length = 0;
            int code = it.code;
            std::string msg = it.msg;
            if (!code && it.image >= 0 && b->out.h_status[it.image]) { code = int(b->out.h_status[it.image]); msg = "device reported a malformed stream"; }
            if (!code) {
                size_t len = b->out.h_img_size[it.image];
                outputs[n].data = (uint8_t *)malloc(len ? len : 1);
                memcpy(outputs[n].data, host.data() + b->out.h_img_off[it.image], len);
                outputs[n].length = len;
            } else failed++;
            if (results) set_result(&results[n], code, msg);
        }
    };
    size_t nthreads = std::min<size_t>(std::min<size_t>(8, std::max(1u, std::thread::hardware_concurrency())), b->items.size() / 64 + 1);
    std::vector<std::thread> pool;
    for (size_t t = 1; t < nthreads; t++) pool.emplace_back(worker);
    worker();
    for (auto &t : pool) t.join();
    return failed.load();
}

extern "C" int csh_batch_geometry(csh_batch *b, size_t image, int comp, int which, int *bw, int *bh, int *real_bw, int *real_bh) {
    if (image >= b->items.size() || b->items[image].image < 0) { csh_set_error("image not on the device"); return -1; }
    const ImgDesc &im = b->imgs[b->items[image].image];
    if (comp < 0 || comp >= (which ? im.ncomp : im.ncomp_in)) { csh_set_error("bad component"); return -1; }
    const CompGeom &g = which ? im.out[comp] : im.in[comp];
    *bw = g.bw; *bh = g.bh; *real_bw = g.real_bw; *real_bh = g.real_bh;
    return 0;
}

extern "C" int csh_batch_read_coefs(csh_batch *b, size_t image, int comp, int which, int16_t *dst) {
    int bw, bh, rbw, rbh;
    if (csh_batch_geometry(b, image, comp, which, &bw, &bh, &rbw, &rbh)) return -1;
    const ImgDesc &im = b->imgs[b->items[image].image];
    const CompGeom &g = which ? im.out[comp] : im.in[comp];
    {
        const size_t at = size_t(b->items[image].image) * CSH_MAX_COMPS + size_t(comp);
        const int si = (which && b->enc.last_run_ac_lists && at < b->enc.nzset_of.size()) ? b->enc.nzset_of[at] : -1;
        if (si >= 0 && size_t(si) < b->enc.nzset_ac_lists.size() && b->enc.nzset_ac_lists[size_t(si)]) {
            if (hipSetDevice(b->device) != hipSuccess) { csh_set_error("hipSetDevice failed"); return -1; }
            launch_nz_to_tiles(b->stream, b->enc.d_nzsets.p, b->enc.d_nzlists.p, b->enc.d_nz_pool.p, b->enc.d_nz_chunk_off.p, b->enc.d_nz_chunk_cnt.p, uint32_t(si),
                               (b->enc.nzsets[size_t(si)].nunits + 255u) / 256u, b->d_coef.p);
        }
    }
    std::vector<int16_t> tiles(size_t(g.ntiles) * CSH_TILE_I16);
    if (csh_copy_wait(tiles.data(), b->d_coef.p + size_t(g.tile_base) * CSH_TILE_I16, tiles.size() * 2, hipMemcpyDeviceToHost, b->stream) != hipSuccess) { csh_set_error("D2H failed"); return -1; }
    for (int blk = 0; blk < bw * bh; blk++)
        for (int k = 0; k < 64; k++) dst[size_t(blk) * 64 + k] = tiles[size_t(blk >> 6) * CSH_TILE_I16 + (blk & 63) * CSH_BLK_STRIDE + coef_off(k)];
    return 0;
}
```

### include/caesium_hip.h

```cpp
#ifndef CAESIUM_HIP_H
#define CAESIUM_HIP_H
#include <stdbool.h>
#include <stddef.h>
#include <stdint.h>
#ifdef __cplusplus
extern "C" {
#endif

enum { CS_TYPE_JPEG = 0, CS_TYPE_PNG = 1, CS_TYPE_GIF = 2, CS_TYPE_WEBP = 3, CS_TYPE_TIFF = 4, CS_TYPE_UNKN = 5 };

enum {
    CS_OK = 0,
    CS_ERR_NO_DEVICE = 10001,
    CS_ERR_UNKNOWN_TYPE = 10200,
    CS_ERR_UNSUPPORTED = 10201,
    CS_ERR_BAD_JPEG = 20100,
    CS_ERR_JPEG_FEATURE = 20101,
    CS_ERR_POOL_OVERFLOW = 20200,
    CS_ERR_BAD_PNG = 30100,
    CS_ERR_BAD_WEBP = 40100,
    CS_ERR_BAD_GIF = 50100,
    CS_ERR_SAME_FORMAT = 10407,
    CS_ERR_TOO_BIG = 10500
};

typedef struct {
    bool keep_metadata;
    uint32_t jpeg_quality;
    uint32_t jpeg_chroma_subsampling;
    bool jpeg_progressive;
    bool jpeg_optimize;
    bool jpeg_preserve_icc;
    uint32_t png_quality;
    uint32_t png_optimization_level;
    bool png_force_zopfli;
    bool png_optimize;
    uint32_t gif_quality;
    uint32_t webp_quality;
    bool webp_lossless;
    uint32_t tiff_compression;
    uint32_t tiff_deflate_level;
    uint32_t width;
    uint32_t height;
} CCSParameters;

typedef struct {
    bool success;
    uint32_t code;
    const char *error_message;
} CCSResult;

typedef struct {
    uint8_t *data;
    size_t length;
} CByteArray;

void cs_default_parameters(CCSParameters *p);

CCSResult cs_compress_in_memory(const uint8_t *in, size_t n, const CCSParameters *p, CByteArray *out);
CCSResult cs_compress_to_size_in_memory(const uint8_t *in, size_t n, CCSParameters *p, size_t max_output_size,
                                        bool return_smallest, CByteArray *out);
CCSResult cs_convert_in_memory(const uint8_t *in, size_t n, const CCSParameters *p, uint32_t format, CByteArray *out);
int cs_batch_convert(const CByteArray *inputs, size_t count, const CCSParameters *p, uint32_t format, int device, CByteArray *outputs, CCSResult *results);

int cs_batch_compress(const CByteArray *inputs, size_t count, const CCSParameters *p, int device,
                      CByteArray *outputs, CCSResult *results);
int cs_batch_compress_to_size(const CByteArray *inputs, size_t count, CCSParameters *p, size_t max_output_size, bool return_smallest,
                              int device, CByteArray *outputs, CCSResult *results);

size_t cs_batch_extent(const CByteArray *inputs, size_t count);

void cs_free_bytes(CByteArray *b);
void cs_free_result(CCSResult *r);

typedef struct csh_batch csh_batch;

enum { CSH_NPHASES = 8, CSH_NKERNELS = 36 };
typedef struct {
    float total_ms;
    float phase_ms[CSH_NPHASES];
    float kernel_ms[CSH_NKERNELS];
    uint64_t in_bytes, out_bytes;
    uint64_t pixels;
    uint64_t coef_bytes;
    uint32_t n_images, n_failed;
    uint32_t n_seq_decoded;
    uint32_t n_par_fallback;
    uint32_t n_par_short;
    uint32_t n_prog_decoded;
    uint32_t n_refine_chains;
    uint32_t n_search_extra;
    uint32_t n_fused_lists;
    uint32_t n_list_refine;
    uint32_t n_ac_in_lists;
    uint32_t n_list_runs;
    uint32_t n_ref_packed;
} csh_timing;

int csh_device_count(void);
const char *csh_last_error(void);
void csh_warmup(int device);
void csh_release_cached_memory(void);
const char *csh_kernel_name(int slot);
const char *csh_kernel_name_webp(int slot);
int csh_batch_create(const CByteArray *inputs, size_t count, const CCSParameters *p, int device, csh_batch **out);
int csh_batch_create_webp(const CByteArray *inputs, size_t count, const CCSParameters *p, int device, csh_batch **out);
int csh_batch_create_pixels(const CByteArray *inputs, size_t count, const CCSParameters *p, int device, csh_batch **out);
int csh_batch_pixels(csh_batch *b, size_t image, const uint8_t **device_pixels, uint32_t *width, uint32_t *height, uint32_t *channels, const char **message);
struct csp_pixels_s;
int csh_batch_create_from_pixels(const struct csp_pixels_s *sources, size_t count, const CCSParameters *p, int device, csh_batch **out);
int csh_batch_run(csh_batch *b, csh_timing *t);
int csh_batch_fetch(csh_batch *b, CByteArray *outputs, CCSResult *results);
void csh_batch_destroy(csh_batch *b);

int csh_batch_retain_dct(csh_batch *b, int on);
int csh_batch_set_quality(csh_batch *b, const uint32_t *quality);
int csh_batch_rerun_encode(csh_batch *b, csh_timing *t);

int csh_batch_geometry(csh_batch *b, size_t image, int comp, int which, int *bw, int *bh, int *real_bw, int *real_bh);
int csh_batch_read_coefs(csh_batch *b, size_t image, int comp, int which, int16_t *dst);

typedef struct csp_batch csp_batch;
enum { CSP_NKERNELS = 16 };
typedef struct {
    float total_ms;
    float kernel_ms[CSP_NKERNELS];
    uint64_t in_bytes, out_bytes;
    uint64_t pixels, raw_bytes;
    uint32_t n_images, n_failed, n_trials;
} csp_timing;
const char *csp_kernel_name(int slot);
int csp_batch_create(const CByteArray *inputs, size_t count, const CCSParameters *p, int device, csp_batch **out);
int csp_batch_create_webp(const CByteArray *inputs, size_t count, const CCSParameters *p, int device, csp_batch **out);
typedef struct csp_pixels_s { const uint8_t *device_pixels; uint32_t width, height, channels; } csp_pixels;
int csp_batch_create_pixels(const csp_pixels *sources, size_t count, const CCSParameters *p, int device, csp_batch **out);
int csp_png_to_jpeg(const CByteArray *inputs, size_t count, const CCSParameters *p, int device, CByteArray *outputs, CCSResult *results);
int csp_png_to_lossless_webp(const CByteArray *inputs, size_t count, const CCSParameters *p, int device, CByteArray *outputs, CCSResult *results);
int csp_batch_run(csp_batch *b, csp_timing *t);
int csp_batch_fetch(csp_batch *b, CByteArray *outputs, CCSResult *results);
void csp_batch_destroy(csp_batch *b);
int csp_batch_geometry(csp_batch *b, size_t image, uint32_t *width, uint32_t *height, uint32_t *rowbytes);
int csp_batch_read_rows(csp_batch *b, size_t image, uint8_t *dst);
int csp_batch_read_stream(csp_batch *b, size_t image, int strategy, uint8_t *dst);
int csp_batch_read_scores(csp_batch *b, size_t image, uint64_t *dst, int *have);
int csp_batch_trials(csp_batch *b, size_t image, int *strategies, uint64_t *zlib_bytes, int *ntrials, int *winner);
int csp_batch_chunk_bits(csp_batch *b, size_t image, int trial, uint64_t *dst, size_t cap, size_t *nchunks);

int csl_encode_pixels(const struct csp_pixels_s *sources, size_t count, int device, CByteArray *outputs, CCSResult *results);
int csl_attach_alpha(CByteArray *lossy, const CByteArray *alpha_vp8l, uint32_t width, uint32_t height);

typedef struct cswd_batch cswd_batch;
int cswd_batch_create(const CByteArray *inputs, size_t count, int device, cswd_batch **out);
int cswd_batch_run(cswd_batch *b);
int cswd_batch_pixels(cswd_batch *b, size_t image, const uint8_t **device_pixels, uint32_t *width, uint32_t *height, uint32_t *channels, const char **message);
int cswd_batch_read_pixels(cswd_batch *b, size_t image, uint8_t *dst );
int cswd_batch_alpha(cswd_batch *b, size_t image, const uint8_t **device_rgba, const uint8_t **device_alpha);
int cswd_batch_read_rgba(cswd_batch *b, size_t image, uint8_t *dst );
void cswd_batch_destroy(cswd_batch *b);
int cswd_batch_frames(cswd_batch *b, size_t file, uint32_t *nframes, uint32_t *canvas_w, uint32_t *canvas_h);
int cswd_batch_read_canvas(cswd_batch *b, size_t file, uint32_t frame, uint8_t *dst_rgba);
int cswd_batch_encode_anim(cswd_batch *b, const CByteArray *sources, const size_t *files, size_t nfiles, const CCSParameters *p, int device, CByteArray *outputs, CCSResult *results);
typedef struct cswd_rgba cswd_rgba;
int cswd_rgba_join(const uint8_t *device_rgb, const uint8_t *device_alpha, uint32_t width, uint32_t height, int device, cswd_rgba **out, const uint8_t **device_rgba);
void cswd_rgba_destroy(cswd_rgba *r);
int csh_batch_create_webp_from_pixels(const struct csp_pixels_s *sources, size_t count, const CCSParameters *p, int device, csh_batch **out);
int csh_batch_create_from_pixels_rgb(const struct csp_pixels_s *sources, size_t count, const CCSParameters *p, int device, csh_batch **out);


typedef struct csg_batch csg_batch;
enum { CSG_NKERNELS = 8 };
typedef struct {
    float total_ms;
    float kernel_ms[CSG_NKERNELS];
    uint64_t in_bytes, out_bytes;
    uint32_t n_files, n_frames, n_failed;
    uint32_t n_passed_palette;
    uint32_t n_not_smaller;
    uint32_t chunk_pixels;
    uint32_t lossy_distance;
} csg_timing;
const char *csg_kernel_name(int slot);
int csg_batch_create(const CByteArray *inputs, size_t count, const CCSParameters *p, int device, csg_batch **out);
int csg_batch_create_lossy(const CByteArray *inputs, size_t count, const CCSParameters *p, int device, csg_batch **out);
int csg_batch_run(csg_batch *b, csg_timing *t);
int csg_batch_fetch(csg_batch *b, CByteArray *outputs, CCSResult *results);
void csg_batch_destroy(csg_batch *b);
int csg_batch_frames(csg_batch *b, size_t file, uint32_t *nframes, uint32_t *canvas_w, uint32_t *canvas_h);
int csg_batch_read_indices(csg_batch *b, size_t file, uint32_t frame, uint8_t *dst);
int csg_batch_read_canvas(csg_batch *b, size_t file, uint32_t frame, uint8_t *dst_rgba);
int csg_batch_read_near(csg_batch *b, size_t file, uint32_t frame, uint8_t *cand, uint8_t *count);

#ifdef __cplusplus
}
#endif
#endif
```

Baseline: 45930.

## Group sub-sequences per thread in speculative JPEG decode and seed relax list

Adds a grouped speculative Huffman decode kernel in which each thread walks G consecutive sub-sequences, carrying state between them, so only the group boundaries need hypothesis repair. The group size grows with the total number of sub-sequences. A scan plus seed kernel then builds the initial relax list from the group starts, and one non-walking relax pass replaces the old second dense pass. It also adds a boundary fix for decode ending exactly at the last real bit, and copies the full relax counters back to the host each round for statistics. In exchange it cuts the parallelism of the speculative pass, adds kernel launches, and makes each per-round readback larger.

```diff
diff --git a/caesium-clt_amd/binding.py b/caesium-clt_amd/binding.py
--- a/caesium-clt_amd/binding.py
+++ b/caesium-clt_amd/binding.py
@@ -25,7 +25,7 @@
 
 class Timing(C.Structure):
     _fields_ = [("total_ms", C.c_float), ("phase_ms", C.c_float * NPHASES), ("kernel_ms", C.c_float * NKERNELS), ("in_bytes", C.c_uint64), ("out_bytes", C.c_uint64),
-                ("pixels", C.c_uint64), ("coef_bytes", C.c_uint64), ("n_images", C.c_uint32), ("n_failed", C.c_uint32), ("n_seq_decoded", C.c_uint32), ("n_par_fallback", C.c_uint32), ("n_par_short", C.c_uint32), ("n_prog_decoded", C.c_uint32), ("n_refine_chains", C.c_uint32), ("n_search_extra", C.c_uint32), ("n_fused_lists", C.c_uint32), ("n_list_refine", C.c_uint32), ("n_ac_in_lists", C.c_uint32), ("n_list_runs", C.c_uint32), ("n_ref_packed", C.c_uint32)]
+                ("pixels", C.c_uint64), ("coef_bytes", C.c_uint64), ("n_images", C.c_uint32), ("n_failed", C.c_uint32), ("n_seq_decoded", C.c_uint32), ("n_par_fallback", C.c_uint32), ("n_par_short", C.c_uint32), ("n_prog_decoded", C.c_uint32), ("n_refine_chains", C.c_uint32), ("n_search_extra", C.c_uint32), ("n_fused_lists", C.c_uint32), ("n_list_refine", C.c_uint32), ("n_ac_in_lists", C.c_uint32), ("n_list_runs", C.c_uint32), ("n_ref_packed", C.c_uint32), ("n_dec_group", C.c_uint32), ("n_dec_seeds", C.c_uint32), ("n_dec_relaxed", C.c_uint32)]
 
 
 class PngTiming(C.Structure):
diff --git a/caesium-clt_amd/csrc/batch.hpp b/caesium-clt_amd/csrc/batch.hpp
--- a/caesium-clt_amd/csrc/batch.hpp
+++ b/caesium-clt_amd/csrc/batch.hpp
@@ -22,6 +22,9 @@
     size_t file_size = 0;
     std::vector<uint8_t> meta_out;
 };
+
+constexpr uint32_t kDecSpecLanes = 256;
+static inline uint32_t dec_group_for(uint32_t total_sub) { return total_sub >= (1u << 20) ? 8u : total_sub >= (1u << 19) ? 4u : total_sub >= (1u << 16) ? 2u : 1u; }
 
 struct DecodePlan {
     PinnedBytes bits_pool;
@@ -39,6 +42,12 @@
     std::vector<RefineUnit> refine_units;
     uint32_t refine_hist = 0, refine_pos = 0, refine_max_blocks = 0;
     uint32_t total_sub = 0, max_sub = 0, max_par_blocks = 0, dc_total = 0;
+    uint32_t group = 1, spec_lanes = 256;
+    bool clear_front = false;
+    std::vector<uint32_t> h_relax_cnt;
+    uint32_t last_run_seeds = 0, last_run_relaxed = 0;
+    DevBuf<uint32_t> d_seed_cnt;
+    DevBuf<uint64_t> d_seed_off;
 
     DevBuf<uint8_t> d_bits, d_clean;
     DevBuf<ParScan> d_pscans;
@@ -287,6 +296,9 @@
     uint32_t list_run = CSH_LIST_RUN;
     bool ac_runs_slot = false;
     bool ac_tiles = false;
+    uint32_t dec_group = 0;
+    bool dec_clear_front = false;
+    uint32_t dec_lanes = 0;
     static PlanSwitches read();
 };
 
diff --git a/caesium-clt_amd/csrc/batch_plan.cpp b/caesium-clt_amd/csrc/batch_plan.cpp
--- a/caesium-clt_amd/csrc/batch_plan.cpp
+++ b/caesium-clt_amd/csrc/batch_plan.cpp
@@ -226,6 +226,9 @@
     s.fused_420 = !getenv("CSH_NO_FUSED_420");
     if (const char *lr = getenv("CSH_LIST_RUN")) { if (*lr) s.list_run = uint32_t(std::min(32, std::max(1, atoi(lr)))); }
     s.ac_runs_slot = is("CSH_AC_RUNS", "slot");
+    for (uint32_t g : {1u, 2u, 4u, 8u}) if (is("CSH_DEC_GROUP", std::to_string(g).c_str())) s.dec_group = g;
+    s.dec_clear_front = is("CSH_DEC_CLEAR", "front");
+    s.dec_lanes = is("CSH_DEC_LANES", "192") ? 192u : is("CSH_DEC_LANES", "256") ? 256u : 0u;
     return s;
 }
 
@@ -1117,6 +1120,10 @@
         b->pix.d_rweights.upload(b->pix.rweights, st) || b->pix.d_rgb.alloc(b->pix.rgb_bytes + 64) || b->pix.d_rtmp.alloc((resize_is_fused(b->pix.max_row_in) ? 0 : b->pix.tmp_floats) + 16) || b->dec.d_need_seq_init.upload(b->dec.need_seq_init, st))
         return CS_ERR_NO_DEVICE;
     size_t nchunks = b->dec.bits_pool.size() / 64 + 1, nst = size_t(b->dec.total_sub) + b->dec.pscans.size() + 1;
+    b->dec.group = sw.dec_group ? sw.dec_group : dec_group_for(b->dec.total_sub);
+    b->dec.spec_lanes = sw.dec_lanes ? sw.dec_lanes : kDecSpecLanes;
+    b->dec.clear_front = sw.dec_clear_front;
+    if (b->dec.d_seed_cnt.alloc(b->dec.pscans.size() + 1) || b->dec.d_seed_off.alloc(b->dec.pscans.size() + 2)) return CS_ERR_NO_DEVICE;
     if (b->dec.d_clean.alloc(b->dec.bits_pool.size() + 64) || b->dec.d_unstuff_cnt.alloc(nchunks + 1) || b->dec.d_unstuff_off.alloc(nchunks + 2) ||
         b->dec.d_pstate.alloc(nst) || b->dec.d_relax_list[0].alloc(nst) || b->dec.d_relax_list[1].alloc(nst) || b->dec.d_relax_cnt.alloc(512) || b->dec.d_scan_pending.alloc(b->dec.pscans.size() + 1) || b->dec.d_cut_block.alloc(b->dec.pscans.size() + 1) || b->dec.d_claim.alloc(size_t(b->dec.total_sub) + 1) || b->dec.d_hyp.alloc((size_t(b->dec.total_sub) + 1) * 10) ||
         b->dec.d_nblk.alloc(size_t(b->dec.total_sub) + 1) || b->dec.d_blk_off.alloc(size_t(b->dec.total_sub) + 2) || b->dec.d_need_seq.alloc(b->nimg + 1) ||
diff --git a/caesium-clt_amd/csrc/batch_run.cpp b/caesium-clt_amd/csrc/batch_run.cpp
--- a/caesium-clt_amd/csrc/batch_run.cpp
+++ b/caesium-clt_amd/csrc/batch_run.cpp
@@ -72,7 +72,7 @@
         if (b->enc.d_raw.n != raw_chunks * 16) {
             if (b->enc.d_raw.alloc(raw_chunks * 16) || b->enc.d_chunk_ff.alloc(raw_chunks + 1) || b->out.d_out.alloc(b->out.out_cap + 64))
                 return -1;
-            const uint64_t longest = std::max({uint64_t(size_t(b->enc.nslots)), uint64_t(b->enc.swork.size()), uint64_t(b->dec.dc_total), uint64_t(b->dec.total_sub), uint64_t(b->dec.bits_pool.size() / 64), uint64_t(nimg)});
+            const uint64_t longest = std::max({uint64_t(size_t(b->enc.nslots)), uint64_t(b->enc.swork.size()), uint64_t(b->dec.dc_total), uint64_t(b->dec.total_sub), uint64_t(b->dec.pscans.size()), uint64_t(b->dec.bits_pool.size() / 64), uint64_t(nimg)});
             size_t tmp = exclusive_scan_tmp_bytes(longest + 1);
             if (b->enc.d_scan_tmp.alloc(tmp)) return -1;
         }
@@ -93,7 +93,7 @@
     }
 
     int decode() {
-        const bool zero_in_spec = !b->dec.pscans.empty() && b->dec.max_sub != 0;
+        const bool spec = !b->dec.pscans.empty() && b->dec.max_sub != 0, zero_in_spec = spec && !b->dec.clear_front;
         if (!zero_in_spec) CSH_CHECK(hipMemsetAsync(b->d_coef.p, 0, size_t(b->ntiles_in) * CSH_TILE_I16 * sizeof(int16_t), st));
         if (b->out.d_status.zero(st) || b->out.d_overflow.zero(st)) return -1;
         CSH_CHECK(hipMemcpyAsync(b->dec.d_need_seq.p, b->dec.d_need_seq_init.p, size_t(nimg) * sizeof(uint32_t), hipMemcpyDeviceToDevice, st));
@@ -115,35 +115,61 @@
             CSH_CHECK(hipMemsetAsync(b->dec.d_cut_block.p, 0xFF, b->dec.d_cut_block.n * sizeof(uint32_t), st));
             const uint64_t zero_all = uint64_t(b->ntiles_in) * CSH_TILE_I16 * sizeof(int16_t), zero_half = (zero_all / 2) & ~uint64_t(15);
             const uint64_t eob_all = (uint64_t(b->enc.d_eobrun.n) * sizeof(uint16_t)) & ~uint64_t(15), eob_half = (eob_all / 2) & ~uint64_t(15);
-            if (zero_in_spec) { da.zero_ptr = reinterpret_cast<uint8_t *>(b->d_coef.p); da.zero_bytes = zero_half; da.zero2_ptr = reinterpret_cast<uint8_t *>(b->enc.d_eobrun.p); da.zero2_bytes = eob_half; }
-            launch_dec_dense(st, 0, nps, b->dec.max_sub, da);
-            da.zero_bytes = 0; da.zero2_bytes = 0;
-            MARK(KS_DEC_SPEC);
-            if (nps) CSH_CHECK(hipMemsetAsync(b->dec.d_relax_cnt.p, 0, b->dec.d_relax_cnt.n * sizeof(uint32_t), st));
-            if (nps && b->dec.d_claim.zero(st)) return -1;
-            if (zero_in_spec) {
-                da.zero_ptr = reinterpret_cast<uint8_t *>(b->d_coef.p) + zero_half; da.zero_bytes = zero_all - zero_half;
-                da.zero2_ptr = reinterpret_cast<uint8_t *>(b->enc.d_eobrun.p) + eob_half; da.zero2_bytes = eob_all - eob_half;
-                if (uint64_t(b->enc.d_eobrun.n) * sizeof(uint16_t) > eob_all) CSH_CHECK(hipMemsetAsync(reinterpret_cast<uint8_t *>(b->enc.d_eobrun.p) + eob_all, 0, uint64_t(b->enc.d_eobrun.n) * sizeof(uint16_t) - eob_all, st));
-                eobrun_cleared = b->enc.d_eobrun.n != 0;
+            da.live_cnt = b->dec.d_relax_cnt.p + b->dec.d_relax_cnt.n - 1; da.seed_cnt = b->dec.d_seed_cnt.p;
+            const uint32_t G = spec ? b->dec.group : 1u;
+            const int seam = G > 1 ? 1 : 0;
+            const uint64_t eob_tail = uint64_t(b->enc.d_eobrun.n) * sizeof(uint16_t) - eob_all;
+            if (G > 1) {
+                if (zero_in_spec) {
+                    da.zero_ptr = reinterpret_cast<uint8_t *>(b->d_coef.p); da.zero_bytes = zero_all; da.zero2_ptr = reinterpret_cast<uint8_t *>(b->enc.d_eobrun.p); da.zero2_bytes = eob_all;
+                    if (eob_tail) CSH_CHECK(hipMemsetAsync(reinterpret_cast<uint8_t *>(b->enc.d_eobrun.p) + eob_all, 0, eob_tail, st));
+                    eobrun_cleared = b->enc.d_eobrun.n != 0;
+                }
+                launch_dec_spec_group(st, nps, b->dec.max_sub, G, b->dec.spec_lanes, da);
+                da.zero_bytes = 0; da.zero2_bytes = 0;
+                MARK(KS_DEC_SPEC);
+                CSH_CHECK(hipMemsetAsync(b->dec.d_relax_cnt.p, 0, b->dec.d_relax_cnt.n * sizeof(uint32_t), st));
+                if (b->dec.d_claim.zero(st)) return -1;
+                launch_exclusive_scan(st, b->dec.d_seed_cnt.p, b->dec.d_seed_off.p, uint64_t(nps), b->enc.d_scan_tmp.p, b->enc.d_scan_tmp.n);
+                launch_dec_seed(st, b->dec.d_seed_off.p, nps, b->dec.max_sub, G, b->dec.d_relax_list[0].p, b->dec.d_relax_cnt.p);
+                launch_dec_relax_list(st, b->dec.d_clean.p, b->dec.d_pscans.p, b->dec.total_sub, da.huffs, da.compact, b->dec.d_pstate.p, b->dec.d_nblk.p, b->dec.d_relax_list[0].p,
+                                      b->dec.d_relax_cnt.p, b->dec.d_relax_list[1].p, b->dec.d_relax_cnt.p + 1, b->dec.d_pstate.n, b->dec.d_claim.p, 0x80000000u, false);
+                MARK(KS_DEC_RELAX0);
+            } else {
+                if (zero_in_spec) { da.zero_ptr = reinterpret_cast<uint8_t *>(b->d_coef.p); da.zero_bytes = zero_half; da.zero2_ptr = reinterpret_cast<uint8_t *>(b->enc.d_eobrun.p); da.zero2_bytes = eob_half; }
+                launch_dec_dense(st, 0, nps, b->dec.max_sub, da);
+                da.zero_bytes = 0; da.zero2_bytes = 0;
+                MARK(KS_DEC_SPEC);
+                if (nps) CSH_CHECK(hipMemsetAsync(b->dec.d_relax_cnt.p, 0, b->dec.d_relax_cnt.n * sizeof(uint32_t), st));
+                if (nps && b->dec.d_claim.zero(st)) return -1;
+                if (zero_in_spec) {
+                    da.zero_ptr = reinterpret_cast<uint8_t *>(b->d_coef.p) + zero_half; da.zero_bytes = zero_all - zero_half;
+                    da.zero2_ptr = reinterpret_cast<uint8_t *>(b->enc.d_eobrun.p) + eob_half; da.zero2_bytes = eob_all - eob_half;
+                    if (eob_tail) CSH_CHECK(hipMemsetAsync(reinterpret_cast<uint8_t *>(b->enc.d_eobrun.p) + eob_all, 0, eob_tail, st));
+                    eobrun_cleared = b->enc.d_eobrun.n != 0;
+                }
+                launch_dec_dense(st, 1, nps, b->dec.max_sub, da);
+                da.zero_bytes = 0; da.zero2_bytes = 0;
+                MARK(KS_DEC_RELAX0);
             }
-            launch_dec_dense(st, 1, nps, b->dec.max_sub, da);
-            da.zero_bytes = 0; da.zero2_bytes = 0;
-            MARK(KS_DEC_RELAX0);
-            const int kMaxRounds = int(b->dec.d_relax_cnt.n) - 2;
+            const int kMaxRounds = int(b->dec.d_relax_cnt.n) - 2 - seam;
+            std::vector<uint32_t> &cnt = b->dec.h_relax_cnt;
+            cnt.assign(b->dec.d_relax_cnt.n, 0u);
             int R = 0;
             for (int group = 12; nps && R < kMaxRounds; group = 8) {
                 for (int g = 0; g < group && R < kMaxRounds; g++, R++)
-                    launch_dec_relax_list(st, b->dec.d_clean.p, b->dec.d_pscans.p, b->dec.total_sub, da.huffs, da.compact, b->dec.d_pstate.p, b->dec.d_nblk.p, b->dec.d_relax_list[R & 1].p,
-                                          b->dec.d_relax_cnt.p + R, b->dec.d_relax_list[(R & 1) ^ 1].p, b->dec.d_relax_cnt.p + R + 1, b->dec.d_pstate.n, b->dec.d_claim.p, uint32_t(R + 1));
-                uint32_t left = 0;
-                CSH_CHECK(hipMemcpyAsync(&left, b->dec.d_relax_cnt.p + R, sizeof left, hipMemcpyDeviceToHost, st));
+                    launch_dec_relax_list(st, b->dec.d_clean.p, b->dec.d_pscans.p, b->dec.total_sub, da.huffs, da.compact, b->dec.d_pstate.p, b->dec.d_nblk.p, b->dec.d_relax_list[(R + seam) & 1].p,
+                                          b->dec.d_relax_cnt.p + R + seam, b->dec.d_relax_list[((R + seam) & 1) ^ 1].p, b->dec.d_relax_cnt.p + R + seam + 1, b->dec.d_pstate.n, b->dec.d_claim.p, uint32_t(R + 1));
+                CSH_CHECK(hipMemcpyAsync(cnt.data(), b->dec.d_relax_cnt.p, cnt.size() * sizeof(uint32_t), hipMemcpyDeviceToHost, st));
                 CSH_CHECK(hipStreamSynchronize(st));
-                if (!left) break;
+                if (!cnt[size_t(R + seam)]) break;
             }
+            b->dec.last_run_seeds = cnt[0];
+            b->dec.last_run_relaxed = cnt.back();
+            for (int r = 0; r < R + seam; r++) b->dec.last_run_relaxed += cnt[size_t(r)];
             if (nps) {
                 if (b->dec.d_scan_pending.zero(st)) return -1;
-                launch_dec_mark_pending(st, b->dec.d_pscans.p, b->dec.total_sub, b->dec.d_relax_list[R & 1].p, b->dec.d_relax_cnt.p + R, b->dec.d_scan_pending.p);
+                launch_dec_mark_pending(st, b->dec.d_pscans.p, b->dec.total_sub, b->dec.d_relax_list[(R + seam) & 1].p, b->dec.d_relax_cnt.p + R + seam, b->dec.d_scan_pending.p);
                 da.hyp = b->dec.d_hyp.p; da.scan_pending = b->dec.d_scan_pending.p;
                 launch_dec_dense(st, 3, nps, b->dec.max_sub, da);
                 launch_dec_chain(st, b->dec.d_pscans.p, nps, b->dec.d_pstate.p, b->dec.d_nblk.p, b->dec.d_hyp.p, b->dec.d_scan_pending.p, b->dec.d_need_seq.p);
@@ -422,6 +448,7 @@
 int run_once(csh_batch *b, csh_timing *t, bool requant_only) {
     Run r(b, t);
     b->enc.last_run_list_runs = 0;
+    b->dec.last_run_seeds = 0; b->dec.last_run_relaxed = 0;
     b->enc.last_run_fused = 0; b->enc.last_run_refine = 0; b->enc.last_run_ref_packed = 0; b->enc.last_run_ac_lists = 0;
     if (r.pools() || r.marks.start()) return -1;
     const bool from_pixels = requant_only && b->tr.dering;
diff --git a/caesium-clt_amd/csrc/k_decode_par.hip b/caesium-clt_amd/csrc/k_decode_par.hip
--- a/caesium-clt_amd/csrc/k_decode_par.hip
+++ b/caesium-clt_amd/csrc/k_decode_par.hip
@@ -291,8 +291,9 @@
         }
     };
     while (pos < stop_bit) step();
+    const bool at_end = stop_bit >= cx.real_bits;
     if (WRITE && !dead)
-        while (pos > cx.real_bits && (k != k_first || m != 0) && __umul24(mcu, uint32_t(cx.nb_mcu)) < cx.total_blocks) step();
+        while ((pos > cx.real_bits || (at_end && pos == cx.real_bits)) && (k != k_first || m != 0) && __umul24(mcu, uint32_t(cx.nb_mcu)) < cx.total_blocks) step();
     if (WRITE && KIND == CSH_PS_SEQ && cur_oct >= 0) flush(true);
     st.pos = pos; st.k = k; st.m = m;
     return WRITE ? ((cut_mcu == 0xFFFFFFFFu || dead) ? 0xFFFFFFFFu : (cut_mcu + 1u) * uint32_t(cx.nb_mcu)) : nblk;
@@ -426,6 +427,7 @@
     CSH_PHASE_LOOP(2) {
         if (phase == 0) {
             if (MODE == 1 && t < nsub && t * CSH_SUBSEQ_BYTES >= ps.clean_len) a.nblk[ps.sub_base + t] = 0;
+            if (MODE == 1 && t == 0) atomicAdd(a.live_cnt, min(nsub, (ps.clean_len + CSH_SUBSEQ_BYTES - 1) / CSH_SUBSEQ_BYTES));
             if (!wg_live) continue;
             const uint32_t *src = reinterpret_cast<const uint32_t *>(&static_cast<const SET *>(a.huffs)[ps.huff_set]);
             uint32_t *dst = reinterpret_cast<uint32_t *>(&lhs);
@@ -486,6 +488,95 @@
     clear_share();
 }
 
+template <class SET, int LANES>
+__global__ void __launch_bounds__(LANES) k_dec_spec_group(DenseArgs a, uint32_t G) {
+    CSH_SHARED uint32_t lrows[LANES * CSH_LROW_STRIDE];
+    CSH_SHARED SET lhs;
+    CSH_PERSIST(uint64_t, carry, 1);
+    auto clear_region = [&](uint8_t *ptr, uint64_t bytes) __attribute__((always_inline)) {
+        if (!bytes) return;
+        const uint64_t nwg = uint64_t(gridDim.x) * gridDim.y, wg = uint64_t(blockIdx.y) * gridDim.x + blockIdx.x;
+        const uint64_t share = ((bytes / 16 + nwg - 1) / nwg) * 16, z0 = wg * share, z1 = z0 + share < bytes ? z0 + share : bytes;
+        for (uint64_t off = z0 + uint64_t(threadIdx.x) * 16; off < z1; off += LANES * 16) {
+#ifdef CSH_EMUL
+            memset(ptr + off, 0, 16);
+#else
+            __builtin_nontemporal_store(0ull, reinterpret_cast<unsigned long long *>(ptr + off));
+            __builtin_nontemporal_store(0ull, reinterpret_cast<unsigned long long *>(ptr + off + 8));
+#endif
+        }
+    };
+    const ParScan &ps = a.pss[blockIdx.y];
+    const uint32_t tid = threadIdx.x;
+    const uint32_t nsub = (ps.bits_len + CSH_SUBSEQ_BYTES - 1) / CSH_SUBSEQ_BYTES;
+    const uint32_t live_sub = par_decoded(ps.kind) ? min(nsub, (ps.clean_len + CSH_SUBSEQ_BYTES - 1) / CSH_SUBSEQ_BYTES) : 0u;
+    if (blockIdx.x == 0 && tid == 0) a.seed_cnt[blockIdx.y] = (live_sub + G - 1) / G;
+    if (!par_decoded(ps.kind)) { clear_region(a.zero_ptr, a.zero_bytes); clear_region(a.zero2_ptr, a.zero2_bytes); return; }
+    const uint32_t g0 = blockIdx.x * LANES, wave0 = tid & ~63u, lane = tid & 63u;
+    const bool wg_live = g0 * G < live_sub;
+    PReader g; g.base = a.clean + ps.bits_off; g.len = ps.clean_len;
+    const size_t base = ps.sub_base + ps.par_index;
+    CSH_PHASE_LOOP_MIXED(2 * int(G), 0xFFFFFFFEu) {
+        const uint32_t j = uint32_t(phase) >> 1;
+        if (!(phase & 1)) {
+            if (phase == 0) {
+                for (uint32_t jj = 0; jj < G; jj++) {
+                    const uint32_t t = (g0 + tid) * G + jj;
+                    if (t < nsub && t >= live_sub) a.nblk[ps.sub_base + t] = 0;
+                }
+                if (wg_live) {
+                    const uint32_t *src = reinterpret_cast<const uint32_t *>(&static_cast<const SET *>(a.huffs)[ps.huff_set]);
+                    uint32_t *dst = reinterpret_cast<uint32_t *>(&lhs);
+                    for (uint32_t i = tid; i < sizeof(SET) / 4; i += LANES) dst[i] = src[i];
+                }
+            }
+            if (!wg_live) continue;
+            for (uint32_t idx = lane; idx < 64 * 9; idx += 64) {
+                const uint32_t row = wave0 + idx / 9, q = idx % 9, t = (g0 + row) * G + j;
+                if (t >= live_sub) continue;
+                uint32_t *dst = lrows + row * CSH_LROW_STRIDE + q * 4;
+                const uint32_t b = t * CSH_SUBSEQ_BYTES + q * 16, nw = q == 8 ? CSH_LROW_WORDS - 32 : 4;
+                if (b + 16 <= g.len) {
+                    uint32_t w[4];
+#ifdef CSH_EMUL
+                    memcpy(w, g.base + b, 16);
+#else
+                    const uint4 v = *reinterpret_cast<const uint4 *>(g.base + b);
+                    w[0] = v.x; w[1] = v.y; w[2] = v.z; w[3] = v.w;
+#endif
+                    for (uint32_t i = 0; i < nw; i++) dst[i] = (w[i] >> 24) | ((w[i] >> 8) & 0xFF00u) | ((w[i] << 8) & 0xFF0000u) | (w[i] << 24);
+                } else
+                    for (uint32_t i = 0; i < nw; i++) dst[i] = g.word(b / 4 + i);
+            }
+            continue;
+        }
+        if (!wg_live) continue;
+        const uint32_t t = (g0 + tid) * G + j;
+        if (t >= nsub) continue;
+        PState st;
+        if (j == 0) {
+            st.pos = t * CSH_SUBSEQ_BYTES * 8; st.m = 0; st.k = ps.kind == CSH_PS_AC_FIRST ? ps.Ss : 0;
+            if (t == 0) a.state[base] = pack_state(st);
+        } else st = unpack_state(carry[0]);
+        if (t >= live_sub) { a.state[base + t + 1] = 0; continue; }
+        RowReader rd; rd.row = lrows + tid * CSH_LROW_STRIDE;
+        const ParCtx cx = make_ctx(ps, nullptr);
+        const uint32_t n = CSH_SPAN(false, ps.kind, rd, t * (CSH_SUBSEQ_BYTES / 4), reinterpret_cast<const uint8_t *>(&lhs), uint32_t(sizeof(SET::root)), cx, st,
+                                    (t + 1) * CSH_SUBSEQ_BYTES * 8, 0, nullptr, nullptr, nullptr);
+        carry[0] = pack_state(st);
+        a.state[base + t + 1] = carry[0];
+        if (j) a.nblk[ps.sub_base + t] = n;
+    }
+    clear_region(a.zero_ptr, a.zero_bytes);
+    clear_region(a.zero2_ptr, a.zero2_bytes);
+}
+__global__ void __launch_bounds__(256) k_dec_seed(const uint64_t *seed_off, int nps, uint32_t G, uint64_t *list, uint32_t *cnt) {
+    const uint32_t si = blockIdx.y, i = blockIdx.x * blockDim.x + threadIdx.x;
+    const uint64_t o = seed_off[si];
+    if (i < uint32_t(seed_off[si + 1] - o)) list[o + i] = (uint64_t(si) << 32) | (i * G);
+    if (blockIdx.x == 0 && si == 0 && threadIdx.x == 0) *cnt = uint32_t(seed_off[nps]);
+}
+
 __global__ void __launch_bounds__(256) k_dc_scatter(const ParScan *pss, const ImgDesc *imgs, const uint64_t *dc_off, int16_t *coef, const uint32_t *need_seq,
                                                      const uint32_t *cut_block) {
     const ParScan &ps = pss[blockIdx.y];
@@ -541,12 +632,26 @@
     else CSH_DENSE(3);
 #undef CSH_DENSE
 }
+void launch_dec_spec_group(hipStream_t st, int nps, uint32_t max_sub, uint32_t group, uint32_t lanes, const DenseArgs &a) {
+    if (!nps || !max_sub) return;
+    const uint32_t ngroups = (max_sub + group - 1) / group;
+#define CSH_SPEC(L) do { const dim3 grid((ngroups + L - 1) / L, nps);                                                                        \
+                         if (a.compact) CSH_LAUNCH_PHASED((k_dec_spec_group<ParHuffSet4, L>), 2 * int(group), grid, dim3(L), st, a, group); \
+                         else CSH_LAUNCH_PHASED((k_dec_spec_group<ParHuffSet, L>), 2 * int(group), grid, dim3(L), st, a, group); } while (0)
+    if (lanes == 192) CSH_SPEC(192);
+    else CSH_SPEC(256);
+#undef CSH_SPEC
+}
+void launch_dec_seed(hipStream_t st, const uint64_t *seed_off, int nps, uint32_t max_sub, uint32_t group, uint64_t *list, uint32_t *cnt) {
+    if (!nps || !max_sub) return;
+    CSH_LAUNCH(k_dec_seed, dim3(((max_sub + group - 1) / group + 255) / 256, nps), dim3(256), st, seed_off, nps, group, list, cnt);
+}
 #ifdef CSH_EMUL
 int csh_emul_jacobi = 0;
 #endif
 void launch_dec_relax_list(hipStream_t st, const uint8_t *clean, const ParScan *ps, uint32_t total_sub, const void *huffs, int compact, uint64_t *state, uint32_t *nblk,
-                           const uint64_t *list_in, const uint32_t *cnt_in, uint64_t *list_out, uint32_t *cnt_out, size_t nstate, uint32_t *claim, uint32_t epoch) {
-    const uint32_t walk_below = epoch > 10 ? 0xFFFFFFFFu : total_sub / 1024 + 1;
+                           const uint64_t *list_in, const uint32_t *cnt_in, uint64_t *list_out, uint32_t *cnt_out, size_t nstate, uint32_t *claim, uint32_t epoch, bool walk) {
+    const uint32_t walk_below = !walk ? 0u : epoch > 10 ? 0xFFFFFFFFu : total_sub / 1024 + 1;
     if (!total_sub) return;
     const uint64_t *state_rd = state;
 #ifdef CSH_EMUL
diff --git a/caesium-clt_amd/csrc/kernels.h b/caesium-clt_amd/csrc/kernels.h
--- a/caesium-clt_amd/csrc/kernels.h
+++ b/caesium-clt_amd/csrc/kernels.h
@@ -51,10 +51,14 @@
     uint32_t *cut_block;
     uint8_t *zero_ptr; uint64_t zero_bytes;
     uint8_t *zero2_ptr; uint64_t zero2_bytes;
+    uint32_t *live_cnt;
+    uint32_t *seed_cnt;
 };
 void launch_dec_dense(hipStream_t st, int mode , int nps, uint32_t max_sub, const DenseArgs &a);
+void launch_dec_spec_group(hipStream_t st, int nps, uint32_t max_sub, uint32_t group, uint32_t lanes, const DenseArgs &a);
+void launch_dec_seed(hipStream_t st, const uint64_t *seed_off, int nps, uint32_t max_sub, uint32_t group, uint64_t *list, uint32_t *cnt);
 void launch_dec_relax_list(hipStream_t st, const uint8_t *clean, const ParScan *ps, uint32_t total_sub, const void *huffs, int compact, uint64_t *state, uint32_t *nblk,
-                           const uint64_t *list_in, const uint32_t *cnt_in, uint64_t *list_out, uint32_t *cnt_out, size_t nstate, uint32_t *claim, uint32_t epoch);
+                           const uint64_t *list_in, const uint32_t *cnt_in, uint64_t *list_out, uint32_t *cnt_out, size_t nstate, uint32_t *claim, uint32_t epoch, bool walk = true);
 void launch_refine_chains(hipStream_t st, const uint8_t *clean, const ParScan *pss, const ParHuffSet *huffs, const DecScan *scans, const ProgChain *chains,
                           const int *chain_scans, int nchains, const RefineUnit *units, int nunits, uint32_t max_blocks, const ImgDesc *imgs, int16_t *coef,
                           uint32_t *need_seq, uint64_t *hist, uint32_t *posv, uint32_t *prog);
diff --git a/caesium-clt_amd/csrc/pipeline.cpp b/caesium-clt_amd/csrc/pipeline.cpp
--- a/caesium-clt_amd/csrc/pipeline.cpp
+++ b/caesium-clt_amd/csrc/pipeline.cpp
@@ -252,6 +252,7 @@
         t->n_ac_in_lists = b->enc.last_run_ac_lists;
         t->n_list_runs = b->enc.last_run_list_runs;
         t->n_ref_packed = b->enc.last_run_ref_packed;
+        t->n_dec_group = b->dec.group; t->n_dec_seeds = b->dec.last_run_seeds; t->n_dec_relaxed = b->dec.last_run_relaxed;
         for (const Item &it : b->items) if (it.image < 0) t->n_failed++;
         for (int i = 0; i < b->nimg; i++) { t->out_bytes += b->out.h_img_size[i]; t->pixels += uint64_t(b->imgs[i].width) * b->imgs[i].height; }
         t->in_bytes = b->dec.bits_pool.size();
diff --git a/include/caesium_hip.h b/include/caesium_hip.h
--- a/include/caesium_hip.h
+++ b/include/caesium_hip.h
@@ -95,6 +95,9 @@
     uint32_t n_ac_in_lists;
     uint32_t n_list_runs;
     uint32_t n_ref_packed;
+    uint32_t n_dec_group;
+    uint32_t n_dec_seeds;
+    uint32_t n_dec_relaxed;
 } csh_timing;
 
 int csh_device_count(void);
```

New measurement: 48800, median of 6. 1.06x the previous value.
